# abstract-liu/LORB_SLAM

Measured on AMD Instinct MI355X. Metric: ORB matches/sec + local-BA iterations/sec (50 KF, 10k pts) at 1/2/4/8 MI355X, higher is better.
Workload: dtype f64+u8; 1 GPU; c4_local_mapping_step_chained; windows_per_gpu=1, kf=50, fixed_kf=5, points=10679, observations=75130, new_kf_keypoints=2000, match=2000x~10679 bf crossCheck, parallelism=independent windows x1

## Files before the change

lorb_slam_amd/csrc/lorb_ba.hip:

```cpp
#ifndef LORB_NO_CONTRACT
#pragma clang fp contract(fast)
#endif
#include "lorb_ba_math.h"
#include "lorb_internal.h"
#include "lorb_ba_dev.h"
#include "lorb_ba_plan.h"

#include <algorithm>
#include <cmath>
#include <type_traits>

namespace {

using namespace lorb::ba;
using lorb::residual;
using lorb::residual_jac;
using lorb::residual_jac_s;
using lorb::residual_s;

__device__ __forceinline__ void init_run(const BaDev& d, int W, int ctot, int n_pt, int nf, const LMOpt& o, const int i,
                                         const int stride) {
  if (i < W) {
    WinState s;
    s.radius = o.init_radius; s.decrease_factor = 2.0; s.cost = 0.0; s.x_norm = 0.0; s.gmax = 0.0;
    s.initial_cost = 0.0; s.iter = 0; s.n_success = 0; s.n_invalid = 0;
    s.done = d.win[i].n_obs_all == 0 ? 1 : 0;
    s.relin = 1; s.cur = 0; s.last_successful = 1; s.term = 0; s.chol_fail = 0; s.pad = 0;
    d.st[i] = s;
    if (d.sharded) d.wfail_part[i] = 0.0;
  }
  if (i < ctot) {
    double x[6];
#pragma unroll
    for (int k = 0; k < 6; ++k) { x[k] = d.x_init_pose[6 * i + k]; d.x_pose[0][6 * i + k] = x[k]; }
    d.rot_lin[i] = lorb::rot_jet(x);
  }
  if (i < nf) {
    double x[6];
#pragma unroll
    for (int k = 0; k < 6; ++k) x[k] = d.fixed_pose[6 * i + k];
    d.rot_fix[i] = lorb::rot_jet(x);
    d.rotv_fix[i] = lorb::rot_val(x);
  }
  for (int k = i; k < 3 * n_pt; k += stride) d.x_pt[0][k] = d.x_init_pt[k];
}
__global__ __launch_bounds__(256) void k_ba_init(BaDev d, int W, int ctot, int n_pt, int nf, LMOpt o) {
  init_run(d, W, ctot, n_pt, nf, o, blockIdx.x * blockDim.x + threadIdx.x, gridDim.x * blockDim.x);
}


constexpr int kGW = kGB / 64;
static_assert(kGW >= 1 && kGW <= 16 && kGB % 64 == 0, "point groups of 64..1024 observations, whole waves");
template <bool M1>
__device__ __forceinline__ void block_red3(double& a, double& b, double& c, double (*red)[kGW]) {
  a = wave_sum(a); b = M1 ? wave_max(b) : wave_sum(b); c = wave_sum(c);
  if (kGW == 1) return;
  __syncthreads();
  if ((threadIdx.x & 63) == 0) {
    const int w = threadIdx.x >> 6;
    red[0][w] = a; red[1][w] = b; red[2][w] = c;
  }
  __syncthreads();
  a = red[0][0]; b = red[1][0]; c = red[2][0];
#pragma unroll
  for (int k = 1; k < kGW; ++k) { a += red[0][k]; b = M1 ? fmax(b, red[1][k]) : b + red[1][k]; c += red[2][k]; }
}

__device__ __forceinline__ bool prep_point(const double (&Eu)[6], const double (&bu)[3], const double (&sp)[3],
                                           double rad, const LMOpt& o, double (&Ei)[6], double (&b)[3]) {
  double E[6];
#pragma unroll
  for (int k = 0; k < 3; ++k) b[k] = bu[k] * sp[k];
  E[0] = Eu[0] * sp[0] * sp[0]; E[1] = Eu[1] * sp[0] * sp[1]; E[2] = Eu[2] * sp[0] * sp[2];
  E[3] = Eu[3] * sp[1] * sp[1]; E[4] = Eu[4] * sp[1] * sp[2]; E[5] = Eu[5] * sp[2] * sp[2];
  E[0] += fmin(fmax(E[0], o.min_diag), o.max_diag) / rad;
  E[3] += fmin(fmax(E[3], o.min_diag), o.max_diag) / rad;
  E[5] += fmin(fmax(E[5], o.min_diag), o.max_diag) / rad;
  if (!inv3(E, Ei)) {
#pragma unroll
    for (int k = 0; k < 6; ++k) Ei[k] = 0.0;
    return false;
  }
  return true;
}
__device__ __forceinline__ void prep_fail(const BaDev& d, int win) {
  if (d.sharded) d.wfail_part[win] = 1.0;
  else d.st[win].chol_fail = 1;
}

template <int PH>
__global__ __launch_bounds__(64) void k_ba_win_reduce(BaDev d) {
  const int w = blockIdx.x;
  if (d.st[w].done) return;
  const BaWin& W = d.win[w];
  const int lane = threadIdx.x;
  double a = 0.0, b = 0.0, c = 0.0;
  if (PH == 0) group_partials<0, 1, 2, true>(d.part, W.pblk_base, W.n_pblk, lane, a, c, b);
  else group_partials<3, 4, 5, false>(d.part, W.pblk_base, W.n_pblk, lane, a, b, c);
  a = wave_sum(a); b = wave_sum(b);
  c = PH == 0 ? wave_max(c) : wave_sum(c);
  if (lane == 0) {
    if (PH == 0) { d.wlin_part[2 * w] = a; d.wlin_part[2 * w + 1] = b; d.wmax_part[w] = c; }
    else { d.wstep_part[3 * w] = a; d.wstep_part[3 * w + 1] = b; d.wstep_part[3 * w + 2] = c; }
  }
}

template <bool SH>
__device__ __forceinline__ void lm_begin_run(const BaDev& d, const LMOpt& o, const int w) {
  const WinState* Sp = d.st + w;
  const WinState S = *Sp;
  const BaWin W = d.win[w];
  if (S.done) return;
  (void)lm_head<SH>(d, o, w, threadIdx.x, S, W);
}
template <bool SH>
__global__ __launch_bounds__(64) void k_ba_lm_begin(BaDev d, LMOpt o) {
  lm_begin_run<SH>(d, o, blockIdx.x);
}

__device__ __forceinline__ void lm_record(const BaDev& d, int w, const WinState& S, int outcome, double mcc,
                                          double ncost, double step_norm) {
  if (S.iter < 1 || S.iter > LORB_LM_TRACE_CAP) return;
  lorb_lm_iteration r;
  r.iteration = S.iter; r.outcome = outcome;
  r.cost = S.cost; r.model_cost_change = mcc; r.new_cost = ncost; r.radius = S.radius; r.step_norm = step_norm;
  d.trace[(size_t)w * LORB_LM_TRACE_CAP + S.iter - 1] = r;
}

__device__ int lm_decide(BaDev d, const LMOpt& o, int w, WinState S, bool valid, double mccs,
                         double ncost, double sn2) {
  const double model_cost_change = -mccs;
  valid = valid && isfinite(model_cost_change) && isfinite(sn2) && model_cost_change > 0.0;
  if (!valid) {
    lm_record(d, w, S, LORB_LM_STEP_INVALID, model_cost_change, ncost, sqrt(sn2));
    if (++S.n_invalid >= o.max_invalid) {
      S.done = 1; S.term = LORB_TERM_FAILURE;
    } else {
      S.radius = S.radius / S.decrease_factor;
      S.decrease_factor *= 2.0;
      S.last_successful = 0;
      if (S.iter >= o.max_iter) { S.done = 1; S.term = LORB_TERM_NO_CONVERGENCE; }
    }
    d.st[w] = S;
    return 0;
  }
  S.n_invalid = 0;
  const double new_cost = isfinite(ncost) ? ncost : 1.7976931348623157e308;
  const double step_norm = sqrt(sn2);
  if (step_norm <= o.ptol * (S.x_norm + o.ptol)) {
    lm_record(d, w, S, LORB_LM_STEP_PARAM_TOL, model_cost_change, new_cost, step_norm);
    S.done = 1; S.term = LORB_TERM_PARAMETER_TOL; d.st[w] = S; return 0;
  }
  const double cost_change = S.cost - new_cost;
  if (fabs(cost_change) <= o.ftol * S.cost) {
    lm_record(d, w, S, LORB_LM_STEP_FUNC_TOL, model_cost_change, new_cost, step_norm);
    S.done = 1; S.term = LORB_TERM_FUNCTION_TOL; d.st[w] = S; return 0;
  }
  const double rel = cost_change / model_cost_change;
  lm_record(d, w, S, rel > o.min_rel ? LORB_LM_STEP_ACCEPTED : LORB_LM_STEP_REJECTED, model_cost_change, new_cost,
            step_norm);
  if (rel > o.min_rel) {
    S.cur ^= 1;
    S.relin = 1;
    S.cost = new_cost;
    S.n_success++;
    const double tt = 2.0 * rel - 1.0;
    S.radius = S.radius / fmax(1.0 / 3.0, 1.0 - tt * tt * tt);
    S.radius = fmin(o.max_radius, S.radius);
    S.decrease_factor = 2.0;
  } else {
    S.last_successful = 0;
    S.radius = S.radius / S.decrease_factor;
    S.decrease_factor *= 2.0;
  }
  if (S.iter >= o.max_iter) { S.done = 1; S.term = LORB_TERM_NO_CONVERGENCE; }
  d.st[w] = S;
  return rel > o.min_rel;
}

template <bool SH>
__device__ __forceinline__ void lm_end_run(const BaDev& d, const LMOpt& o, int w, int lane) {
  const WinState* Sp = d.st + w;
  WinState S = *Sp;
  const BaWin W = d.win[w];
  if (S.done) return;
  bool valid = !S.chol_fail;
  double mccs = 0.0, ncost = 0.0, sn2 = 0.0;
  double xc[6] = {0, 0, 0, 0, 0, 0};
  if (valid) {
    const int cur = S.cur;
    const int c0 = W.pose_base + lane;
    const bool has0 = lane < W.n_poses;
    double x0[6], xn0[6];
    bool act0 = false;
    if (has0) {
      act0 = d.cam_active[c0];
#pragma unroll
      for (int k = 0; k < 6; ++k) { x0[k] = d.x_pose[cur][6 * c0 + k]; xn0[k] = d.x_pose[cur ^ 1][6 * c0 + k]; }
    }
    if (!SH) group_partials<3, 4, 5, false>(d.part, W.pblk_base, W.n_pblk, lane, mccs, ncost, sn2);
    if (has0) {
#pragma unroll
      for (int k = 0; k < 6; ++k) {
        if (act0) sn2 += (x0[k] - xn0[k]) * (x0[k] - xn0[k]);
        xc[k] = xn0[k];
      }
    }
    for (int c = c0 + 64; c < W.pose_base + W.n_poses; c += 64) {
      const bool active = d.cam_active[c];
      for (int k = 0; k < 6; ++k) {
        const double x = d.x_pose[cur][6 * c + k];
        const double xn = d.x_pose[cur ^ 1][6 * c + k];
        if (active) sn2 += (x - xn) * (x - xn);
      }
    }
    mccs = wave_sum(mccs); ncost = wave_sum(ncost); sn2 = wave_sum(sn2);
    if (SH) { mccs += d.wstep[3 * w]; ncost += d.wstep[3 * w + 1]; sn2 += d.wstep[3 * w + 2]; }
  }
  S.chol_fail = 0;
  if (SH && lane == 0) d.wfail_part[w] = 0.0;
  int acc = 0;
  if (lane == 0) acc = lm_decide(d, o, w, S, valid, mccs, ncost, sn2);
  acc = __builtin_amdgcn_readfirstlane(acc);
  if (acc) {
    if (lane < W.n_poses) d.rot_lin[W.pose_base + lane] = lorb::rot_jet(xc);
    for (int c = W.pose_base + lane + 64; c < W.pose_base + W.n_poses; c += 64)
      d.rot_lin[c] = lorb::rot_jet(d.x_pose[S.cur ^ 1] + 6 * c);
  }
}
template <bool SH>
__global__ __launch_bounds__(64) void k_ba_lm_end(BaDev d, LMOpt o) {
  lm_end_run<SH>(d, o, blockIdx.x, threadIdx.x);
}


__device__ __forceinline__ void pm_slot_inv(int q, int bwc, int& a, int& dd) {
  const int T = (bwc + 1) * (bwc + 2) / 2;
  if (q < T) {
    a = (int)((sqrt(8.0 * q + 1.0) - 1.0) * 0.5);
    while ((a + 1) * (a + 2) / 2 <= q) ++a;
    while (a * (a + 1) / 2 > q) --a;
    dd = q - a * (a + 1) / 2;
  } else {
    const int r = q - T;
    a = bwc + 1 + r / (bwc + 1);
    dd = r - (r / (bwc + 1)) * (bwc + 1);
  }
}

constexpr int kLsThreads = kGB;
constexpr int kLsWaves = kLsThreads / 64;

template <int NW, bool M1>
__device__ __forceinline__ void block_red3w(double& a, double& b, double& c, double (*red)[NW]) {
  a = wave_sum(a); b = M1 ? wave_max(b) : wave_sum(b); c = wave_sum(c);
  __syncthreads();
  if ((threadIdx.x & 63) == 0) {
    const int w = threadIdx.x >> 6;
    red[0][w] = a; red[1][w] = b; red[2][w] = c;
  }
  __syncthreads();
  a = red[0][0]; b = red[1][0]; c = red[2][0];
#pragma unroll
  for (int k = 1; k < NW; ++k) { a += red[0][k]; b = M1 ? fmax(b, red[1][k]) : b + red[1][k]; c += red[2][k]; }
}

__device__ __forceinline__ void pm_lin(const BaDev& d, const BaWin& W, int cur, int p, int c, int fx, double2 uv,
                                       double (&r)[2], double (&Jp)[6], double (&Jc)[12]) {
  double X[3];
#pragma unroll
  for (int k = 0; k < 3; ++k) X[k] = d.x_pt[cur][3 * p + k];
  if (c >= 0) {
    double tr[3];
#pragma unroll
    for (int k = 0; k < 3; ++k) tr[k] = d.x_pose[cur][6 * c + 3 + k];
    residual_jac_s(d.rot_lin[c], tr, X, W.fx, W.fy, W.cx, W.cy, uv.x, uv.y, r, Jp, Jc);
  } else {
    double tr[3];
#pragma unroll
    for (int k = 0; k < 3; ++k) tr[k] = d.fixed_pose[6 * fx + 3 + k];
    residual_jac_s(d.rot_fix[fx], tr, X, W.fx, W.fy, W.cx, W.cy, uv.x, uv.y, r, Jp, Jc);
  }
}

struct LsSup {
  double* gsp;
  int cmin;
};
template <bool SUP>
__device__ __forceinline__ void ls_group(const BaDev& d, const LMOpt& o, const unsigned bid, const LsSup& su) {
  __shared__ double s_jc[kGB][12];
  __shared__ double s_qj[kGB][12];
  __shared__ double s_rg[kGB][4];
  __shared__ unsigned long long s_mask[2][kGB];
  __shared__ int s_po[kGB];
  __shared__ int s_mm[2][kLsWaves];
  __shared__ double red3[3][kLsWaves];
#ifdef LORB_LS_STAMPS
#define LS_STAMP(k) do { if (threadIdx.x == 0) d.dbg[8 * bid + (k)] = __builtin_amdgcn_s_memtime(); } while (0)
#else
#define LS_STAMP(k) do {} while (0)
#endif
  LS_STAMP(0);
#ifdef LORB_LS_STAMPS
  const unsigned long long ls_rt0 = __builtin_amdgcn_s_memrealtime();
  if (threadIdx.x == 0)
    d.dbg[8 * bid + 6] = ((unsigned long long)__builtin_amdgcn_s_getreg((31 << 11) | 4) << 8) |
                                (__builtin_amdgcn_s_getreg((31 << 11) | 20) & 255);
#endif
  const PBlk g = d.pblk[bid];
  const int t = threadIdx.x, lane = t & 63, wv = t >> 6;
  const bool has = t < g.no;
  const int of = g.o0 + min(t, max(g.no - 1, 0));
  const int p_ = has ? d.obs_pt[of] : 0, c_ = has ? d.obs_cam[of] : -1;
  const int fx_ = has ? d.obs_fix[of] : 0;
  const double2 uv = has ? d.obs_uv[of] : make_double2(0.0, 0.0);
  int po0 = 0, po1 = 0;
  double Xp[2][3] = {{0, 0, 0}, {0, 0, 0}}, spp[3] = {0, 0, 0};
  if (t < g.cnt) {
    const int p = g.p0 + t;
    po0 = d.pt_obs_off[p]; po1 = d.pt_obs_off[p + 1];
#pragma unroll
    for (int k = 0; k < 3; ++k) { Xp[0][k] = d.x_pt[0][3 * p + k]; Xp[1][k] = d.x_pt[1][3 * p + k]; spp[k] = d.scale_pt[3 * p + k]; }
  }
  const WinState& S = d.st[g.win];
  if (S.done) return;
  const BaWin& W = d.win[g.win];
  const int cur = S.cur;
  const double rad = S.radius;
  if (t < kGB) { s_mask[0][t] = 0ull; s_mask[1][t] = 0ull; }
  double r[2] = {0, 0}, Jp[6] = {0, 0, 0, 0, 0, 0}, Jc[12];
#pragma unroll
  for (int k = 0; k < 12; ++k) Jc[k] = 0.0;
  double cost = 0.0;
  if (has) {
    pm_lin(d, W, cur, p_, c_, fx_, uv, r, Jp, Jc);
    cost = 0.5 * (r[0] * r[0] + r[1] * r[1]);
    double* v = s_qj[t];
    v[0] = Jp[0] * Jp[0] + Jp[3] * Jp[3]; v[1] = Jp[0] * Jp[1] + Jp[3] * Jp[4];
    v[2] = Jp[0] * Jp[2] + Jp[3] * Jp[5]; v[3] = Jp[1] * Jp[1] + Jp[4] * Jp[4];
    v[4] = Jp[1] * Jp[2] + Jp[4] * Jp[5]; v[5] = Jp[2] * Jp[2] + Jp[5] * Jp[5];
    v[6] = Jp[0] * r[0] + Jp[3] * r[1]; v[7] = Jp[1] * r[0] + Jp[4] * r[1];
    v[8] = Jp[2] * r[0] + Jp[5] * r[1];
  }
  {
    int mn = has && c_ >= 0 ? c_ : 0x7fffffff, mx = has && c_ >= 0 ? c_ : -1;
#pragma unroll
    for (int s = 32; s > 0; s >>= 1) { mn = min(mn, __shfl_xor(mn, s, 64)); mx = max(mx, __shfl_xor(mx, s, 64)); }
    if (lane == 0) { s_mm[0][wv] = mn; s_mm[1][wv] = mx; }
  }
  __syncthreads();
  LS_STAMP(1);
  int cmin = s_mm[0][0], cmax = s_mm[1][0];
#pragma unroll
  for (int k = 1; k < kLsWaves; ++k) { cmin = min(cmin, s_mm[0][k]); cmax = max(cmax, s_mm[1][k]); }
  const int span = cmax >= 0 ? cmax - cmin + 1 : 0;
  double gm = 0.0, xn2 = 0.0;
  if (t < g.cnt) {
    const int p = g.p0 + t;
    double E[6] = {0, 0, 0, 0, 0, 0}, b[3] = {0, 0, 0};
    for (int e = po0 - g.o0; e < po1 - g.o0; ++e) {
      const double* v = s_qj[e];
#pragma unroll
      for (int k = 0; k < 6; ++k) E[k] += v[k];
#pragma unroll
      for (int k = 0; k < 3; ++k) b[k] += v[6 + k];
    }
#pragma unroll
    for (int k = 0; k < 3; ++k) d.etb[3 * p + k] = b[k];
    double sp[3];
    if (S.iter == 0) {
      sp[0] = 1.0 / (1.0 + sqrt(E[0]));
      sp[1] = 1.0 / (1.0 + sqrt(E[3]));
      sp[2] = 1.0 / (1.0 + sqrt(E[5]));
#pragma unroll
      for (int k = 0; k < 3; ++k) d.scale_pt[3 * p + k] = sp[k];
    } else {
#pragma unroll
      for (int k = 0; k < 3; ++k) sp[k] = spp[k];
    }
    if (po1 > po0) {
#pragma unroll
      for (int k = 0; k < 3; ++k) {
        const double X = cur ? Xp[1][k] : Xp[0][k];
        gm = fmax(gm, fabs(X - (X + -b[k])));
        xn2 += X * X;
      }
    }
    double Ei[6], bs[3];
    if (!prep_point(E, b, sp, rad, o, Ei, bs)) prep_fail(d, g.win);
#pragma unroll
    for (int k = 0; k < 6; ++k) { d.pinv[6 * p + k] = Ei[k]; s_jc[t][k] = Ei[k]; }
#pragma unroll
    for (int k = 0; k < 3; ++k) { s_jc[t][6 + k] = bs[k]; s_jc[t][9 + k] = sp[k]; }
    s_po[t] = po0 - g.o0;
  }
  const int lp = p_ - g.p0;
  const int a_ = c_ - cmin;
  if (has && c_ >= 0) atomicOr(&s_mask[a_ >> 6][lp], 1ull << (a_ & 63));
  __syncthreads();
  LS_STAMP(2);
  double Q[6], Js[6], g0 = 0.0, g1 = 0.0;
  int slot = -1;
  if (has && c_ >= 0) {
    const double* pt = s_jc[lp];
#pragma unroll
    for (int k = 0; k < 6; ++k) Js[k] = Jp[k] * pt[9 + k % 3];
#pragma unroll
    for (int rr = 0; rr < 2; ++rr)
#pragma unroll
      for (int j = 0; j < 3; ++j)
        Q[3 * rr + j] = Js[3 * rr] * s3(pt, 0, j) + Js[3 * rr + 1] * s3(pt, 1, j) + Js[3 * rr + 2] * s3(pt, 2, j);
    g0 = Q[0] * pt[6] + Q[1] * pt[7] + Q[2] * pt[8];
    g1 = Q[3] * pt[6] + Q[4] * pt[7] + Q[5] * pt[8];
    const unsigned long long m0 = s_mask[0][lp];
    slot = s_po[lp] + (a_ < 64 ? __popcll(m0 & ((1ull << a_) - 1ull))
                               : __popcll(m0) + __popcll(s_mask[1][lp] & ((1ull << (a_ - 64)) - 1ull)));
  }
  __syncthreads();
  if (slot >= 0) {
#pragma unroll
    for (int k = 0; k < 12; ++k) s_jc[slot][k] = Jc[k];
#pragma unroll
    for (int k = 0; k < 6; ++k) { s_qj[slot][k] = Q[k]; s_qj[slot][6 + k] = Js[k]; }
    s_rg[slot][0] = r[0]; s_rg[slot][1] = r[1]; s_rg[slot][2] = g0; s_rg[slot][3] = g1;
  }
  __syncthreads();
  LS_STAMP(3);
  const int bwc = W.bwc, nsl = pm_nslots(span, bwc);
  double* gp = SUP ? su.gsp : d.gpart + W.part_base + (size_t)(bid - W.sg_base) * W.part_stride;
  const int aoff = SUP ? cmin - su.cmin : 0;
  if (!SUP && t == 0) d.gspan[bid] = make_int2(span > 0 ? cmin - W.pose_base : 0, span);
  const bool split = nsl <= 64;
  int lr = 0;
  if (split) while (lr < 6 && (nsl << (lr + 1)) <= 64) ++lr;
  const int nrounds = split ? 1 : (nsl + 64 * kLsWaves - 1) / (64 * kLsWaves);
  for (int rd = 0; rd < nrounds; ++rd) {
    const int q = split ? lane >> lr : 64 * (kLsWaves * rd + wv) + lane;
    const int rr = split ? lane & ((1 << lr) - 1) : 0;
    const bool act = q < nsl;
    int a = 0, dd = 0;
    if (act) pm_slot_inv(q, bwc, a, dd);
    const int b = a - dd;
    const bool dg = dd == 0;
    double acc[36], ex[18];
#pragma unroll
    for (int k = 0; k < 36; ++k) acc[k] = 0.0;
#pragma unroll
    for (int k = 0; k < 18; ++k) ex[k] = 0.0;
    const int k0 = split ? (wv << lr) + rr : 0, kst = split ? kLsWaves << lr : 1;
    auto point_loop = [&](auto wide_tag) {
      constexpr bool kWide = decltype(wide_tag)::value;
      const int wa = kWide ? a >> 6 : 0, wb = kWide ? b >> 6 : 0;
      const unsigned long long ba = act ? 1ull << (a & 63) : 0ull, bb = 1ull << (b & 63);
      unsigned long long m = s_mask[0][k0], mh = kWide ? s_mask[1][k0] : 0ull;
      int po = s_po[k0];
      for (int k = k0; k < g.cnt; k += kst) {
        const unsigned long long mc = m, mch = mh;
        const int pc = po;
        if (k + kst < g.cnt) {
          m = s_mask[0][k + kst]; po = s_po[k + kst];
          if (kWide) mh = s_mask[1][k + kst];
        }
        const unsigned long long ma = kWide && wa ? mch : mc, mb = kWide && wb ? mch : mc;
        if ((ma & ba) && (mb & bb)) {
          const int lo = kWide ? __popcll(mc) : 0;
          const int eh = pc + (kWide && wa ? lo : 0) + __popcll(ma & (ba - 1ull));
          const int el = pc + (kWide && wb ? lo : 0) + __popcll(mb & (bb - 1ull));
          const double* Qh = s_qj[eh];
          const double* Jl = s_qj[el] + 6;
          const double* Ch = s_jc[eh];
          const double* Cl = s_jc[el];
          double k00 = -(Qh[0] * Jl[0] + Qh[1] * Jl[1] + Qh[2] * Jl[2]);
          double k01 = -(Qh[0] * Jl[3] + Qh[1] * Jl[4] + Qh[2] * Jl[5]);
          double k10 = -(Qh[3] * Jl[0] + Qh[4] * Jl[1] + Qh[5] * Jl[2]);
          double k11 = -(Qh[3] * Jl[3] + Qh[4] * Jl[4] + Qh[5] * Jl[5]);
          if (dg) { k00 += 1.0; k11 += 1.0; }
          double cl[12], ch[12];
#pragma unroll
          for (int j = 0; j < 12; ++j) { cl[j] = Cl[j]; ch[j] = Ch[j]; }
#pragma unroll
          for (int i = 0; i < 6; ++i) {
            const double z0 = ch[i] * k00 + ch[6 + i] * k10, z1 = ch[i] * k01 + ch[6 + i] * k11;
#pragma unroll
            for (int j = 0; j < 6; ++j) acc[6 * i + j] = fma(z0, cl[j], fma(z1, cl[6 + j], acc[6 * i + j]));
          }
          if (dg) {
            const double* rg = s_rg[eh];
            const double g0r = rg[0], g1r = rg[1], g2r = rg[2], g3r = rg[3];
#pragma unroll
            for (int i = 0; i < 6; ++i) {
              ex[i] = fma(ch[i], ch[i], fma(ch[6 + i], ch[6 + i], ex[i]));
              ex[6 + i] = fma(ch[i], g0r, fma(ch[6 + i], g1r, ex[6 + i]));
              ex[12 + i] = fma(ch[i], g2r, fma(ch[6 + i], g3r, ex[12 + i]));
            }
          }
        }
      }
    };
    if (k0 < g.cnt) {
      if (span > 64) point_loop(std::true_type{});
      else point_loop(std::false_type{});
    }
    for (int m = 1; m < (1 << lr); m <<= 1) {
#pragma unroll
      for (int k = 0; k < 36; ++k) acc[k] += __shfl_xor(acc[k], m, 64);
#pragma unroll
      for (int k = 0; k < 18; ++k) ex[k] += __shfl_xor(ex[k], m, 64);
    }
    const bool own = act && rr == 0;
    if (split) {
      static_assert(64 * 36 <= kGB * 12 && 64 * 18 <= kGB * 12, "reduction buffers");
      __syncthreads();
#pragma unroll
      for (int w = 0; w < kLsWaves; ++w) {
        if (wv == w && own) {
          double* bl = &s_jc[0][0] + 36 * q;
          double* bx = &s_qj[0][0] + 18 * q;
#pragma unroll
          for (int k = 0; k < 36; ++k) { if (w > 0) acc[k] += bl[k]; if (w + 1 < kLsWaves) bl[k] = acc[k]; }
          if (dg) {
#pragma unroll
            for (int k = 0; k < 18; ++k) { if (w > 0) ex[k] += bx[k]; if (w + 1 < kLsWaves) bx[k] = ex[k]; }
          }
        }
        if (w + 1 < kLsWaves) __syncthreads();
      }
    }
    if (own && (!split || wv == kLsWaves - 1)) {
      if (SUP) {
        double* out = gp + 36 * pm_slot(a + aoff, dd, bwc);
#pragma unroll
        for (int k = 0; k < 36; ++k) out[k] = out[k] + acc[k];
        if (dg) {
          double* gc = gp + W.part_cam + 18 * (a + aoff);
#pragma unroll
          for (int k = 0; k < 18; ++k) gc[k] = gc[k] + ex[k];
        }
      } else {
        double* out = gp + 36 * q;
#pragma unroll
        for (int k = 0; k < 36; ++k) out[k] = acc[k];
        if (dg) {
          double* gc = gp + W.part_cam + 18 * a;
#pragma unroll
          for (int k = 0; k < 18; ++k) gc[k] = ex[k];
        }
      }
    }
  }
  LS_STAMP(4);
  block_red3w<kLsWaves, true>(cost, gm, xn2, red3);
  if (t == 0) { double* P = d.part + 8 * bid; P[0] = cost; P[1] = gm; P[2] = xn2; }
  LS_STAMP(5);
#ifdef LORB_LS_STAMPS
  if (t == 0) d.dbg[8 * bid + 7] = (ls_rt0 << 20) | ((__builtin_amdgcn_s_memrealtime() - ls_rt0) & 0xfffff);
#endif
#undef LS_STAMP
}
__device__ __forceinline__ void ls_run(const BaDev& d, const LMOpt& o, const unsigned bid) {
  if ((int)bid >= d.live[0]) return;
  ls_group<false>(d, o, bid, LsSup{nullptr, 0});
}
__global__ __launch_bounds__(kLsThreads) void k_ba_ls(BaDev d, LMOpt o) { ls_run(d, o, blockIdx.x); }

__device__ __forceinline__ void ls_run_sup(const BaDev& d, const LMOpt& o, const unsigned sid) {
  __shared__ int s_r[2][kLsWaves];
  if ((int)sid >= d.live[2]) return;
  const int4 sg = d.sgrp[sid];
  const WinState& S = d.st[sg.x];
  if (S.done) return;
  const BaWin& W = d.win[sg.x];
  const PBlk gf = d.pblk[sg.y], gl = d.pblk[sg.y + sg.z - 1];
  const int t = threadIdx.x, lane = t & 63, wv = t >> 6;
  int mn = 0x7fffffff, mx = -1;
  for (int e = gf.o0 + t; e < gl.o0 + gl.no; e += kLsThreads) {
    const int c = d.obs_cam[e];
    if (c >= 0) { mn = min(mn, c); mx = max(mx, c); }
  }
#pragma unroll
  for (int k = 32; k > 0; k >>= 1) { mn = min(mn, __shfl_xor(mn, k, 64)); mx = max(mx, __shfl_xor(mx, k, 64)); }
  if (lane == 0) { s_r[0][wv] = mn; s_r[1][wv] = mx; }
  __syncthreads();
  int cmin = s_r[0][0], cmax = s_r[1][0];
#pragma unroll
  for (int k = 1; k < kLsWaves; ++k) { cmin = min(cmin, s_r[0][k]); cmax = max(cmax, s_r[1][k]); }
  const int span = cmax >= 0 ? cmax - cmin + 1 : 0;
  double* gsp = d.gpart + W.part_base + (size_t)(sid - W.sg_base) * W.part_stride;
  const int nb = 36 * pm_nslots(span, W.bwc), nc = 18 * span;
  for (int i = t; i < nb + nc; i += kLsThreads) gsp[i < nb ? i : W.part_cam + (i - nb)] = 0.0;
  if (t == 0) d.gspan[sid] = make_int2(span > 0 ? cmin - W.pose_base : 0, span);
  __syncthreads();
  for (int k = 0; k < sg.z; ++k) ls_group<true>(d, o, sg.y + k, LsSup{gsp, cmin});
}
__global__ __launch_bounds__(kLsThreads) __attribute__((amdgpu_waves_per_eu(2))) void k_ba_ls_sup(BaDev d, LMOpt o) {
  ls_run_sup(d, o, blockIdx.x);
}

template <int MODE, int RT>
__device__ __forceinline__ void red_run(const BaDev& d, const LMOpt& o, const unsigned bid) {
  constexpr int kRt = RT, kRw = kRt / 64;
  constexpr int kRc = 1024 / kRt;
  __shared__ int s_cand[kRt * kRc];
  __shared__ int s_a[kRt * kRc];
  __shared__ int s_wc[kRc][kRw];
  __shared__ double s_acc[1024];
  __shared__ double s_tot[54];
  if ((int)bid >= d.live[1]) return;
  const BlockPair bp = d.bp[bid];
  const bool diag = bp.ch == bp.cl;
  if (MODE == 0 && !diag) return;
  const WinState& S = d.st[bp.win];
  const BaWin& W = d.win[bp.win];
  const int t = threadIdx.x, lane = t & 63, wv = t >> 6;
  const int fi = t < 36 ? t / 6 : (t < 42 ? t - 36 : 0), fj = t < 36 ? t % 6 : 0;
  double sci = 1.0, scj = 1.0, udg = 0.0;
  if (MODE != 0) {
    sci = d.scale_pose[6 * bp.ch + fi];
    scj = d.scale_pose[6 * bp.cl + fj];
    if (MODE == 1 && diag) udg = d.U[21 * bp.ch + u21(fi, fi)];
  }
  if (S.done) return;
  const int h = bp.ch - W.pose_base, l = bp.cl - W.pose_base, dd = h - l;
  const int e0 = MODE == 0 ? 36 : 0, ne = MODE == 0 ? 12 : (diag ? 54 : 36);
  const int NS = 1024 / ne;
  const int nsub = kRt / ne, e = t % ne, sub = t / ne;
  constexpr int kSp = RT >= 1024 ? 1 : RT >= 512 ? 3 : 5;
  double acc[kSp];
#pragma unroll
  for (int q = 0; q < kSp; ++q) acc[q] = 0.0;
  const int g0 = W.sg_base, ng = W.n_sg;
  for (int c0 = 0; c0 < ng; c0 += kRt * kRc) {
    int2 gs[kRc];
#pragma unroll
    for (int u = 0; u < kRc; ++u) {
      const int gi = c0 + kRt * u + t;
      gs[u] = gi < ng ? d.gspan[g0 + gi] : make_int2(0, 0);
    }
    unsigned long long bal[kRc];
#pragma unroll
    for (int u = 0; u < kRc; ++u) {
      const bool cand = gs[u].y > 0 && gs[u].x <= l && h < gs[u].x + gs[u].y;
      bal[u] = __ballot(cand);
      if (lane == 0) s_wc[u][wv] = __popcll(bal[u]);
    }
    __syncthreads();
    int pre = 0, nc = 0;
#pragma unroll
    for (int u = 0; u < kRc; ++u)
#pragma unroll
      for (int k = 0; k < kRw; ++k) nc += s_wc[u][k];
#pragma unroll
    for (int u = 0; u < kRc; ++u) {
      int pu = pre;
#pragma unroll
      for (int k = 0; k < kRw; ++k) pu += k < wv ? s_wc[u][k] : 0;
      if ((bal[u] >> lane) & 1ull) {
        const int j = pu + __popcll(bal[u] & ((1ull << lane) - 1ull));
        s_cand[j] = c0 + kRt * u + t;
        s_a[j] = h - gs[u].x;
      }
#pragma unroll
      for (int k = 0; k < kRw; ++k) pre += s_wc[u][k];
    }
    __syncthreads();
    if (sub < nsub) {
      const int ee = e0 + e;
      auto at = [&](int j) -> const double* {
        const double* gp = d.gpart + W.part_base + (size_t)s_cand[j] * W.part_stride;
        const int a = s_a[j];
        return ee < 36 ? gp + 36 * pm_slot(a, dd, W.bwc) + ee : gp + W.part_cam + 18 * a + (ee - 36);
      };
      constexpr int kRu = RT >= 1024 ? 8 : RT >= 512 ? 4 : 2;
      for (int b0 = 0;; b0 += kRu) {
        double v[kSp][kRu];
        bool more = false;
#pragma unroll
        for (int q = 0; q < kSp; ++q) {
          const int s0 = sub + q * nsub;
#pragma unroll
          for (int u = 0; u < kRu; ++u) {
            const int j = s0 + (b0 + u) * NS;
            v[q][u] = s0 < NS && j < nc ? *at(j) : 0.0;
          }
          more |= s0 < NS && s0 + (b0 + kRu) * NS < nc;
        }
#pragma unroll
        for (int q = 0; q < kSp; ++q)
#pragma unroll
          for (int u = 0; u < kRu; ++u) acc[q] += v[q][u];
        if (!more) break;
      }
    }
    __syncthreads();
  }
  if (sub < nsub) {
#pragma unroll
    for (int q = 0; q < kSp; ++q) {
      const int s0 = sub + q * nsub;
      if (s0 < NS) s_acc[e + s0 * ne] = acc[q];
    }
  }
  __syncthreads();
  if (t < ne) {
    double v4[4] = {0.0, 0.0, 0.0, 0.0};
#pragma unroll 4
    for (int s = 0; s < NS; ++s) v4[s & 3] += s_acc[t + s * ne];
    s_tot[t] = (v4[0] + v4[1]) + (v4[2] + v4[3]);
  }
  __syncthreads();
  const int c = bp.ch;
  if (MODE == 0) {
    if (t < 6) d.U_part[21 * c + u21(t, t)] = s_tot[t];
    else if (t < 12) d.V_part[6 * c + t - 6] = s_tot[t];
    return;
  }
  double* A = d.env_part + W.env_base;
  if (t < 36) {
    const int i = fi, j = fj;
    if (!diag || j <= i) {
      double v = s_tot[t] * sci * scj;
      if (MODE == 1 && diag && i == j && d.rank0) {
        const double u = udg * sci * sci;
        v += fmin(fmax(u, o.min_diag), o.max_diag) / S.radius;
      }
      band(A, W.bw, 6 * h + i, 6 * l + j) = v;
    }
  } else if (diag && t < 42) {
    const int i = fi;
    d.rhs_part[W.row_base + 6 * h + i] = (s_tot[42 + i] - s_tot[48 + i]) * sci;
    if (MODE == 2) { d.U_part[21 * c + u21(i, i)] = s_tot[36 + i]; d.V_part[6 * c + i] = s_tot[42 + i]; }
  }
}
template <int MODE, int RT>
__global__ __launch_bounds__(RT) void k_ba_red(BaDev d, LMOpt o) { red_run<MODE, RT>(d, o, blockIdx.x); }

__device__ __forceinline__ void bs2_run(const BaDev& d, const unsigned bid) {
  __shared__ double sh[kGB][3], sst[kGB][3], sxn[kGB][3], ssp[kGB][3];
  __shared__ double red3[3][kGW];
  if ((int)bid >= d.live[0]) return;
  const PBlk g = d.pblk[bid];
  const int t = threadIdx.x;
  const bool has = t < g.no;
  const int of = g.o0 + min(t, max(g.no - 1, 0));
  const int p_ = has ? d.obs_pt[of] : 0, c_ = has ? d.obs_cam[of] : -1;
  const int fx_ = has ? d.obs_fix[of] : 0;
  const double2 uv = has ? d.obs_uv[of] : make_double2(0.0, 0.0);
  double b[3] = {0, 0, 0}, sp[3] = {0, 0, 0}, Xa[3] = {0, 0, 0}, Xb[3] = {0, 0, 0};
  double Ei[6] = {0, 0, 0, 0, 0, 0};
  int po0 = 0, po1 = 0;
  if (t < g.cnt) {
    const int p = g.p0 + t;
    po0 = d.pt_obs_off[p]; po1 = d.pt_obs_off[p + 1];
#pragma unroll
    for (int k = 0; k < 3; ++k) {
      sp[k] = d.scale_pt[3 * p + k];
      b[k] = d.etb[3 * p + k] * sp[k];
      Xa[k] = d.x_pt[0][3 * p + k];
      Xb[k] = d.x_pt[1][3 * p + k];
    }
#pragma unroll
    for (int k = 0; k < 6; ++k) Ei[k] = d.pinv[6 * p + k];
  }
  const WinState& S = d.st[g.win];
  if (S.done || S.chol_fail) return;
  const BaWin& W = d.win[g.win];
  const int cur = S.cur;
  if (t < g.cnt) {
#pragma unroll
    for (int k = 0; k < 3; ++k) ssp[t][k] = sp[k];
  }
  double ys[6] = {0, 0, 0, 0, 0, 0}, tc[3] = {0, 0, 0};
  lorb::RotVal Rc{};
  if (has && c_ >= 0) {
    const double* y = d.ycam + W.row_base + 6 * (c_ - W.pose_base);
#pragma unroll
    for (int i = 0; i < 6; ++i) ys[i] = y[i] * d.scale_pose[6 * c_ + i];
    Rc = d.rot_cand[c_];
#pragma unroll
    for (int k = 0; k < 3; ++k) tc[k] = d.x_pose[cur ^ 1][6 * c_ + 3 + k];
  }
  double r[2] = {0, 0}, Jp[6] = {0, 0, 0, 0, 0, 0}, Jc[12];
#pragma unroll
  for (int k = 0; k < 12; ++k) Jc[k] = 0.0;
  if (has) pm_lin(d, W, cur, p_, c_, fx_, uv, r, Jp, Jc);
  const int lp = p_ - g.p0;
  __syncthreads();
  double ya0 = 0.0, ya1 = 0.0;
  if (has) {
    if (c_ >= 0) {
#pragma unroll
      for (int i = 0; i < 6; ++i) {
        ya0 += Jc[i] * ys[i];
        ya1 += Jc[6 + i] * ys[i];
      }
#pragma unroll
      for (int j = 0; j < 3; ++j) sh[t][j] = (Jp[j] * ssp[lp][j]) * ya0 + (Jp[3 + j] * ssp[lp][j]) * ya1;
    } else {
      sh[t][0] = sh[t][1] = sh[t][2] = 0.0;
    }
  }
  __syncthreads();
  double sn2 = 0.0;
  if (t < g.cnt) {
    const int p = g.p0 + t;
    for (int e = po0 - g.o0; e < po1 - g.o0; ++e) {
#pragma unroll
      for (int j = 0; j < 3; ++j) b[j] -= sh[e][j];
    }
    double X[3], step[3];
#pragma unroll
    for (int k = 0; k < 3; ++k) X[k] = cur ? Xb[k] : Xa[k];
#pragma unroll
    for (int j = 0; j < 3; ++j)
      step[j] = -(s3(Ei, j, 0) * b[0] + s3(Ei, j, 1) * b[1] + s3(Ei, j, 2) * b[2]);
#pragma unroll
    for (int j = 0; j < 3; ++j) {
      const double xn = X[j] + step[j] * sp[j];
      d.x_pt[cur ^ 1][3 * p + j] = xn;
      sxn[t][j] = xn;
      sst[t][j] = step[j] * sp[j];
      if (po1 > po0) sn2 += (X[j] - xn) * (X[j] - xn);
    }
  }
  __syncthreads();
  double mcc = 0.0, ncost = 0.0;
  if (has) {
    const double Xn[3] = {sxn[lp][0], sxn[lp][1], sxn[lp][2]};
    double m0 = 0.0, m1 = 0.0;
#pragma unroll
    for (int j = 0; j < 3; ++j) {
      m0 += Jp[j] * sst[lp][j];
      m1 += Jp[3 + j] * sst[lp][j];
    }
    double rn[2];
    if (c_ >= 0) {
      m0 -= ya0;
      m1 -= ya1;
      residual_s(Rc, tc, Xn, W.fx, W.fy, W.cx, W.cy, uv.x, uv.y, rn);
    } else {
      double tr[3];
#pragma unroll
      for (int k = 0; k < 3; ++k) tr[k] = d.fixed_pose[6 * fx_ + 3 + k];
      residual_s(d.rotv_fix[fx_], tr, Xn, W.fx, W.fy, W.cx, W.cy, uv.x, uv.y, rn);
    }
    mcc = m0 * (r[0] + m0 / 2.0) + m1 * (r[1] + m1 / 2.0);
    ncost = 0.5 * (rn[0] * rn[0] + rn[1] * rn[1]);
  }
  block_red3<false>(mcc, ncost, sn2, red3);
  if (t == 0) {
    double* P = d.part + 8 * bid;
    P[3] = mcc; P[4] = ncost; P[5] = sn2;
  }
}
__global__ __launch_bounds__(kGB) void k_ba_bs2(BaDev d) { bs2_run(d, blockIdx.x); }

__global__ __launch_bounds__(256) void k_ba_init_g(BaGrp g, GrpGrid G, GrpInit a, LMOpt o) {
  unsigned lb;
  const int k = grp_member(G, g.n, blockIdx.x, lb);
  init_run(g.d[k], a.W[k], a.ctot[k], a.n_pt[k], a.nf[k], o, (int)(lb * 256 + threadIdx.x),
           (G.pre[k + 1] - G.pre[k]) * 256);
}
__global__ __launch_bounds__(kLsThreads) void k_ba_ls_g(BaGrp g, GrpGrid G, LMOpt o) {
  unsigned lb;
  const int k = grp_member(G, g.n, blockIdx.x, lb);
  ls_run(g.d[k], o, lb);
}
template <int MODE, int RT>
__global__ __launch_bounds__(RT) void k_ba_red_g(BaGrp g, GrpGrid G, LMOpt o) {
  unsigned lb;
  const int k = grp_member(G, g.n, blockIdx.x, lb);
  red_run<MODE, RT>(g.d[k], o, lb);
}
__global__ __launch_bounds__(64) void k_ba_lm_begin_g(BaGrp g, GrpGrid G, LMOpt o) {
  unsigned lb;
  const int k = grp_member(G, g.n, blockIdx.x, lb);
  lm_begin_run<false>(g.d[k], o, (int)lb);
}
__global__ __launch_bounds__(kGB) void k_ba_bs2_g(BaGrp g, GrpGrid G) {
  unsigned lb;
  const int k = grp_member(G, g.n, blockIdx.x, lb);
  bs2_run(g.d[k], lb);
}
__global__ __launch_bounds__(64) void k_ba_lm_end_g(BaGrp g, GrpGrid G, LMOpt o) {
  unsigned lb;
  const int k = grp_member(G, g.n, blockIdx.x, lb);
  lm_end_run<false>(g.d[k], o, (int)lb, threadIdx.x);
}

constexpr int kPoW = 4, kPoThreads = 64 * kPoW;
constexpr int kPoRegRes = 2 * kPoThreads;
constexpr int kPoArgF = 16;
struct PoOff { int n; int off[kPoArgF + 1]; };
template <class Load>
__device__ __forceinline__ void po_run(int nres, double fx, double fyv, double cx, double cy,
                                       const float* pose_init, const LMOpt& o, Load load,
                                       double* __restrict__ pose_out, lorb_ba_summary* __restrict__ sum) {
  __shared__ double s_nv[2][kPoW][28];
  __shared__ double s_cv[2][kPoW];
  const int t = threadIdx.x, lane = t & 63, wv = t >> 6;
  const int r0 = 0, r1 = nres;
  double xs[6], xn[6], sc[6], JtJ[21], Jtr[6];
#pragma unroll
  for (int k = 0; k < 6; ++k) { xs[k] = (double)pose_init[k]; xn[k] = xs[k]; sc[k] = 1.0; }
  if (r1 == r0) {
    if (t < 6) pose_out[t] = xs[t];
    if (t == 0) { lorb_ba_summary z = {}; *sum = z; }
    return;
  }
  double radius = o.init_radius, df = 2.0;
  int iter = 0, n_success = 0, n_invalid = 0, term = LORB_TERM_NO_CONVERGENCE, last_successful = 1;
  double initial_cost = 0.0, cost = 0.0, gmax = 0.0, xnorm = 0.0;
  bool relin = true;
  int buf = 0;
  constexpr int kPoC = kPoRegRes / kPoThreads;
  double cX[kPoC][3], cuv[kPoC][2];
#pragma unroll
  for (int q = 0; q < kPoC; ++q) {
    load(min(r0 + t + kPoThreads * q, r1 - 1), cX[q], cuv[q]);
  }
  for (;;) {
    if (relin) {
      double v[32];
#pragma unroll
      for (int k = 0; k < 28; ++k) v[k] = 0.0;
      const lorb::RotJet R = lorb::rot_jet(xs);
      auto acc = [&](const double (&X)[3], double u, double w) {
        double rr[2], Jp[6], Jc[12];
        residual_jac_s(R, xs + 3, X, fx, fyv, cx, cy, u, w, rr, Jp, Jc);
        int q = 0;
#pragma unroll
        for (int a = 0; a < 6; ++a) {
          v[21 + a] = fma(Jc[a], rr[0], fma(Jc[6 + a], rr[1], v[21 + a]));
#pragma unroll
          for (int b = a; b < 6; ++b) { v[q] = fma(Jc[a], Jc[b], fma(Jc[6 + a], Jc[6 + b], v[q])); ++q; }
        }
        v[27] += 0.5 * (rr[0] * rr[0] + rr[1] * rr[1]);
      };
// ... 161 lines not shown
                                                             double* __restrict__ pose_out,
                                                             lorb_ba_summary* __restrict__ sums) {
  const int f = blockIdx.x;
  const int r0 = aoff.n ? aoff.off[f] : res_off[f], r1 = aoff.n ? aoff.off[f + 1] : res_off[f + 1];
  const float* P = pts3d + 3 * (size_t)r0;
  const float* U = obs2d + 2 * (size_t)r0;
  po_run(r1 - r0, intr[4 * f], intr[4 * f + 1], intr[4 * f + 2], intr[4 * f + 3], pose_init + 6 * f, o,
         [&](int r, double (&X)[3], double (&uv)[2]) {
#pragma unroll
           for (int k = 0; k < 3; ++k) X[k] = P[3 * r + k];
           uv[0] = U[2 * r]; uv[1] = U[2 * r + 1];
         },
         pose_out + 6 * f, sums + f);
}

struct TailSlots {
  int nk;
  const int* code;
  bool keep;
  const uint8_t* slot_state;
  const float *slot_pos, *pt_pos, *x, *y;
  float* list;
  int* copy_to;
  int* assign_out;
};
__device__ __forceinline__ void tail_run(const TailSlots& s, bool solve, double fx, double fyv, double cx, double cy,
                                         const float* pose_init, const LMOpt& o, int* __restrict__ n_res,
                                         double* __restrict__ pose_out, lorb_ba_summary* __restrict__ sum) {
  __shared__ int s_slot[kPoRegRes];
  __shared__ int wsum[kPoW];
  const int t = threadIdx.x;
  int nres = 0;
  for (int c0 = 0; c0 < s.nk; c0 += kPoThreads) {
    const int j = c0 + t;
    int cd = LORB_ASSIGN_NULL;
    bool has = false;
    if (j < s.nk) {
      cd = s.code[j];
      has = cd >= 0 || (s.keep && cd == LORB_ASSIGN_UNCHANGED && s.slot_state && s.slot_state[j] != LORB_SLOT_EMPTY);
      if (s.copy_to) s.copy_to[j] = cd;
      if (s.assign_out) s.assign_out[j] = cd;
    }
    int tot;
    const int r = nres + lorb::block_excl_scan<kPoThreads>(has ? 1 : 0, wsum, &tot);
    if (has) {
      if (r < kPoRegRes) {
        s_slot[r] = j;
      } else {
        const float* X = cd >= 0 ? s.pt_pos + 3 * (size_t)cd : s.slot_pos + 3 * (size_t)j;
        float* L = s.list + 5 * (size_t)r;
        L[0] = X[0]; L[1] = X[1]; L[2] = X[2]; L[3] = s.x[j]; L[4] = s.y[j];
      }
    }
    nres += tot;
  }
  __syncthreads();
  if (t == 0) *n_res = nres;
  po_run(solve ? nres : 0, fx, fyv, cx, cy, pose_init, o,
         [&](int r, double (&X)[3], double (&uv)[2]) {
           if (r < kPoRegRes) {
             const int j = s_slot[r], cd = s.code[j];
             const float* Xp = cd >= 0 ? s.pt_pos + 3 * (size_t)cd : s.slot_pos + 3 * (size_t)j;
#pragma unroll
             for (int k = 0; k < 3; ++k) X[k] = Xp[k];
             uv[0] = s.x[j]; uv[1] = s.y[j];
           } else {
             const float* L = s.list + 5 * (size_t)r;
#pragma unroll
             for (int k = 0; k < 3; ++k) X[k] = L[k];
             uv[0] = L[3]; uv[1] = L[4];
           }
         },
         pose_out, sum);
}

__global__ __launch_bounds__(kPoThreads) void k_track_tail(lorb::TrackTail a, LMOpt o) {
  const int nm1 = *a.nm1;
  const bool retry = nm1 <= a.min_matches;
  const int nm2 = retry ? *a.nm2 : -1;
  const int pass = !retry ? 1 : (nm2 > a.min_matches ? 2 : 0);
  if (threadIdx.x == 0) { a.rec->pass = pass; a.rec->nmatches_first = nm1; a.rec->nmatches_retry = nm2; }
  const TailSlots s = {a.nk, retry ? a.assign2 : a.assign, !retry, a.slot_state, a.slot_pos, a.last_pos, a.x, a.y,
                       a.list, retry ? a.assign : nullptr, a.assign_out};
  tail_run(s, pass != 0, a.fx, a.fy_eff, a.cx, a.cy, a.pose_init, o, &a.rec->n_residuals, a.rec->pose, &a.rec->summary);
}

__global__ __launch_bounds__(kPoThreads) void k_local_tail(lorb::LocalTail a, LMOpt o) {
  __shared__ int wcnt[kPoW];
  const int nm = *a.nm;
  int c = 0;
  for (int m = threadIdx.x; m < a.np; m += kPoThreads) c += a.in_view[m] != 0;
  int n_in_view;
  lorb::block_excl_scan<kPoThreads>(c, wcnt, &n_in_view);
  const bool ok = nm > a.min_matches;
  if (threadIdx.x == 0) { a.rec->ok = ok; a.rec->nmatches = nm; a.rec->n_in_view = n_in_view; }
  const TailSlots s = {a.nk, a.assign, true, a.slot_state, a.slot_pos, a.pt_pos, a.x, a.y, a.list, nullptr, a.assign_out};
  tail_run(s, ok, a.fx, a.fy_eff, a.cx, a.cy, a.pose_init, o, &a.rec->n_residuals, a.rec->pose, &a.rec->summary);
}

LMOpt to_dev_opt(const lorb_lm_options* o) {
  LMOpt d;
  d.max_iter = o->max_num_iterations; d.max_invalid = o->max_num_consecutive_invalid_steps;
  d.jacobi = o->jacobi_scaling; d.ftol = o->function_tolerance; d.gtol = o->gradient_tolerance;
  d.ptol = o->parameter_tolerance; d.init_radius = o->initial_trust_region_radius;
  d.max_radius = o->max_trust_region_radius; d.min_radius = o->min_trust_region_radius;
  d.min_rel = o->min_relative_decrease; d.min_diag = o->min_lm_diagonal; d.max_diag = o->max_lm_diagonal;
  return d;
}
bool same_opt(const LMOpt& a, const LMOpt& b) {
  return a.max_iter == b.max_iter && a.max_invalid == b.max_invalid && a.jacobi == b.jacobi && a.ftol == b.ftol &&
         a.gtol == b.gtol && a.ptol == b.ptol && a.init_radius == b.init_radius && a.max_radius == b.max_radius &&
         a.min_radius == b.min_radius && a.min_rel == b.min_rel && a.min_diag == b.min_diag && a.max_diag == b.max_diag;
}

bool no_graph() { static const bool v = env_flag("LORB_NO_GRAPH"); return v; }
bool no_fuse() { static const bool v = env_flag("LORB_NO_FUSE"); return v; }

int chol_kind_of(const lorb_ba_plan* P) {
  static const bool force_old = [] { const char* e = getenv("LORB_CHOL"); return e && e[0] == 'o'; }();
  static const bool no_2s = [] { const char* e = getenv("LORB_CHOL"); return e && e[0] == 'w'; }();
  if (!P->Ctot) return -1;
  const bool chol_w = !force_old && P->max_bw <= 48 && sizeof(double) * (size_t)P->max_env_w <= (size_t)kLdsBudget;
  const bool chol_2s = chol_w && !no_2s && P->min_n16 >= 128 && P->min_bw >= 15;
  return chol_2s ? 2 : chol_w ? 1 : 0;
}

size_t x2_count(const lorb_ba_plan* P) {
  return P->devb ? P->x2_off + (size_t)P->env_total : (size_t)P->env_total + P->n_total + P->W;
}

int red_threads(const lorb_ba_plan* P) {
  const double W = std::max(P->W, 1), cams = std::max((double)P->Ctot / W, 1.0);
  const double cand = (double)P->n_pblk / W * ((P->max_bw + 1) / 6.0) / cams;
  if (P->grid_bp <= 256 || cand >= 128.0) return 1024;
  return P->grid_bp <= 1024 ? 512 : 256;
}
template <int MODE>
void launch_red(const lorb_ba_plan* P, hipStream_t s, const BaDev& d, const LMOpt& o) {
  const int rt = red_threads(P);
  if (rt == 1024) hipLaunchKernelGGL((k_ba_red<MODE, 1024>), dim3(P->grid_bp), dim3(1024), 0, s, d, o);
  else if (rt == 512) hipLaunchKernelGGL((k_ba_red<MODE, 512>), dim3(P->grid_bp), dim3(512), 0, s, d, o);
  else hipLaunchKernelGGL((k_ba_red<MODE, 256>), dim3(P->grid_bp), dim3(256), 0, s, d, o);
}

void launch_ls(const lorb_ba_plan* P, hipStream_t s, const BaDev& d, const LMOpt& o) {
  lorb::KernelTimer kt(P->ctx, LORB_K_BA_LINEARIZE);
  if (P->has_super) {
    if (P->grid_sg) hipLaunchKernelGGL(k_ba_ls_sup, dim3(P->grid_sg), dim3(kLsThreads), 0, s, d, o);
  } else if (P->grid_pblk) {
    hipLaunchKernelGGL(k_ba_ls, dim3(P->grid_pblk), dim3(kLsThreads), 0, s, d, o);
  }
}

lorb_ba_plan::GraphKey graph_key(const lorb_ba_plan* P) {
  lorb_ba_plan::GraphKey k;
  k.kind = chol_kind_of(P);
  k.lds = k.kind >= 1 ? P->max_env_w : P->max_env + 1000000 * P->max_bw;
  k.memset_env = sizeof(double) * (size_t)P->max_env > (size_t)kLdsBudget;
  k.env_total = k.memset_env ? P->env_total : 0;
  k.grid_pblk = P->grid_pblk; k.grid_bp = P->grid_bp; k.pt_launch = P->pt_launch;
  k.x2_n = P->comm ? (int)x2_count(P) : 0;
  k.red_wide = red_threads(P);
  k.sup = P->has_super ? 1 : 0;
  k.grid_sg = P->grid_sg;
  return k;
}

int enqueue_linearize(lorb_ba_plan* P, const LMOpt& o) {
  hipStream_t s = P->ctx->stream;
  const BaDev& d = P->dev;
  launch_ls(P, s, d, o);
  if (P->grid_bp) {
    lorb::KernelTimer kt(P->ctx, LORB_K_BA_SCHUR);
    launch_red<0>(P, s, d, o);
  }
  if (P->comm) {
    hipLaunchKernelGGL(k_ba_win_reduce<0>, dim3(P->W), dim3(64), 0, s, d);
    {
      lorb::KernelTimer kt(P->ctx, LORB_K_ALLREDUCE);
      LORB_TRY(lorb::comm_allreduce(P->comm, d.U_part, d.U, (size_t)P->Ctot * 27 + 2 * P->W, LORB_OP_SUM));
      LORB_TRY(lorb::comm_allreduce(P->comm, d.wmax_part, d.wmax, (size_t)P->W, LORB_OP_MAX));
    }
    hipLaunchKernelGGL(k_ba_lm_begin<true>, dim3(P->W), dim3(64), 0, s, d, o);
  } else {
    hipLaunchKernelGGL(k_ba_lm_begin<false>, dim3(P->W), dim3(64), 0, s, d, o);
  }
  return LORB_OK;
}

int enqueue_iteration(lorb_ba_plan* P, const LMOpt& o, bool first) {
  lorb_ctx* ctx = P->ctx;
  hipStream_t s = ctx->stream;
  const BaDev& d = P->dev;
  const bool fused = !first && chol_kind_of(P) == 2 && !no_fuse();
  if (fused) {
    launch_ls(P, s, d, o);
  } else {
    LORB_TRY(enqueue_linearize(P, o));
  }
  const bool chol_in_lds = sizeof(double) * (size_t)P->max_env <= (size_t)kLdsBudget;
  if (P->env_total && !chol_in_lds && !P->comm) LORB_HIP(ctx, hipMemsetAsync(d.env, 0, sizeof(double) * P->env_total, s));
  if (P->grid_bp) {
    lorb::KernelTimer kt(ctx, LORB_K_BA_SCHUR);
    if (fused) launch_red<2>(P, s, d, o);
    else launch_red<1>(P, s, d, o);
  }
  if (P->comm && fused) {
    hipLaunchKernelGGL(k_ba_win_reduce<0>, dim3(P->W), dim3(64), 0, s, d);
    lorb::KernelTimer kt(ctx, LORB_K_ALLREDUCE);
    LORB_TRY(lorb::comm_allreduce(P->comm, d.U_part, d.U, P->fx_n, LORB_OP_SUM));
    LORB_TRY(lorb::comm_allreduce(P->comm, d.wmax_part, d.wmax, (size_t)P->W, LORB_OP_MAX));
  } else if (P->comm) {
    lorb::KernelTimer kt(ctx, LORB_K_ALLREDUCE);
    LORB_TRY(lorb::comm_allreduce(P->comm, P->x2_send, P->x2_recv, x2_count(P), LORB_OP_SUM));
  }
  const int kind = chol_kind_of(P);
  P->chol_kind = kind;
  if (kind >= 0) {
    lorb::KernelTimer kt(ctx, LORB_K_BA_CHOLESKY);
    launch_chol(kind, CholShape{P->W, P->max_env, P->max_env_w, P->max_bw}, s, d, o, fused);
  }
  if (P->grid_pblk) hipLaunchKernelGGL(k_ba_bs2, dim3(P->grid_pblk), dim3(kGB), 0, s, d);
  if (P->comm) {
    hipLaunchKernelGGL(k_ba_win_reduce<1>, dim3(P->W), dim3(64), 0, s, d);
    {
      lorb::KernelTimer kt(ctx, LORB_K_ALLREDUCE);
      LORB_TRY(lorb::comm_allreduce(P->comm, d.wstep_part, d.wstep, 3 * (size_t)P->W, LORB_OP_SUM));
    }
    hipLaunchKernelGGL(k_ba_lm_end<true>, dim3(P->W), dim3(64), 0, s, d, o);
  } else {
    hipLaunchKernelGGL(k_ba_lm_end<false>, dim3(P->W), dim3(64), 0, s, d, o);
  }
  LORB_CHECK_LAUNCH(ctx);
  return LORB_OK;
}

int enqueue_solve(lorb_ba_plan* P, const LMOpt& o) {
  lorb_ctx* ctx = P->ctx;
  {
    const int n = std::max(std::max(std::max(P->W, P->Ctot), P->NF), std::min(3 * P->pt_launch, 256 * 1024));
    hipLaunchKernelGGL(k_ba_init, dim3(lorb::ceil_div(std::max(n, 1), 256)), dim3(256), 0, ctx->stream, P->dev, P->W,
                       P->Ctot, P->pt_launch, P->NF, o);
  }
  LORB_CHECK_LAUNCH(ctx);
  if (o.max_iter <= 0) return enqueue_linearize(P, o);
  for (int it = 0; it < o.max_iter; ++it) LORB_TRY(enqueue_iteration(P, o, it == 0));
  return LORB_OK;
}

int plan_solve(lorb_ba_plan* P, const lorb_lm_options* opt) {
  lorb_ctx* ctx = P->ctx;
  LMOpt o = to_dev_opt(opt);
  const bool timing = ctx->ktime || no_graph() || (P->comm && !P->comm->rccl);
  if (timing) return enqueue_solve(P, o);
  const lorb_ba_plan::GraphKey key = graph_key(P);
  const bool same = key == P->gkey && same_opt(P->graph_opt, o);
  return P->cache.replay_or_capture(ctx, same, [&] { return enqueue_solve(P, o); },
                                    [&] { P->gkey = key; P->graph_opt = o; });
}

int plan_read(lorb_ba_plan* P, double* const* pose_out, double* const* point_out,
              lorb_ba_summary* sums) {
  lorb_ctx* ctx = P->ctx;
  std::vector<WinState> st(P->W);
  std::vector<std::vector<double>> hp(P->W);
  LORB_HIP(ctx, hipMemcpyAsync(st.data(), P->d_state, sizeof(WinState) * P->W, hipMemcpyDeviceToHost, ctx->stream));
  LORB_HIP(ctx, hipStreamSynchronize(ctx->stream));
  for (int w = 0; w < P->W; ++w) {
    const BaWin& bw = P->hwin[w];
    const int cur = st[w].cur;
    if (pose_out && pose_out[w] && bw.n_poses) {
      hp[w].resize(6 * (size_t)bw.n_poses);
      LORB_HIP(ctx, hipMemcpyAsync(hp[w].data(), P->dev.x_pose[cur] + 6 * bw.pose_base, sizeof(double) * 6 * bw.n_poses, hipMemcpyDeviceToHost, ctx->stream));
    }
    if (point_out && point_out[w] && bw.n_points)
      LORB_HIP(ctx, hipMemcpyAsync(point_out[w], P->dev.x_pt[cur] + 3 * bw.point_base, sizeof(double) * 3 * bw.n_points, hipMemcpyDeviceToHost, ctx->stream));
    if (sums) {
      lorb_ba_summary s{};
      s.iterations = st[w].iter; s.successful_steps = st[w].n_success; s.termination = st[w].term;
      s.initial_cost = st[w].initial_cost; s.final_cost = st[w].cost;
      if (bw.n_obs_all == 0) { s.iterations = 0; s.termination = LORB_TERM_FUNCTION_TOL; }
      sums[w] = s;
    }
  }
  LORB_HIP(ctx, hipStreamSynchronize(ctx->stream));
  for (int w = 0; w < P->W; ++w) {
    if (hp[w].empty()) continue;
    const std::vector<int>& map = P->cam_map[w];
    for (int c = 0; c < P->hwin[w].n_poses; ++c)
      for (int q = 0; q < 6; ++q)
        pose_out[w][6 * (size_t)c + q] = hp[w][6 * (size_t)(map.empty() ? c : map[c]) + q];
  }
  return LORB_OK;
}

}

struct lorb_ba_group {
  lorb_ctx* ctx = nullptr;
  std::vector<lorb_ba_plan*> plans;
  GraphCache cache{"group graph"};
  LMOpt graph_opt{};
  std::vector<unsigned> gens;
  std::vector<lorb_ba_plan::GraphKey> keys;
  int n_fused = 0;
};

namespace {

bool group_fused(const lorb_ba_group* G) {
  if (no_fuse() || G->plans.size() > (size_t)kGrpMax) return false;
  for (const lorb_ba_plan* P : G->plans)
    if (P->W == 0 || P->comm || P->has_super || chol_kind_of(P) != 2) return false;
  return true;
}

template <typename F>
GrpGrid grp_grid(const lorb_ba_group* G, F f) {
  GrpGrid g{};
  for (size_t k = 0; k < G->plans.size(); ++k) g.pre[k + 1] = g.pre[k] + f(G->plans[k]);
  for (size_t k = G->plans.size() + 1; k <= (size_t)kGrpMax; ++k) g.pre[k] = g.pre[G->plans.size()];
  return g;
}

template <int MODE>
void launch_red_g(const lorb_ba_group* G, hipStream_t s, const BaGrp& bg, const LMOpt& o) {
  const GrpGrid gg = grp_grid(G, [](const lorb_ba_plan* P) { return P->grid_bp; });
  const int n = (int)G->plans.size(), nb = gg.pre[n];
  if (nb == 0) return;
  bool wide = nb <= 256;
  for (const lorb_ba_plan* P : G->plans) wide = wide || (red_threads(P) == 1024 && P->grid_bp > 256);
  const int rt = wide ? 1024 : nb <= 1024 ? 512 : 256;
  if (rt == 1024) hipLaunchKernelGGL((k_ba_red_g<MODE, 1024>), dim3(nb), dim3(1024), 0, s, bg, gg, o);
  else if (rt == 512) hipLaunchKernelGGL((k_ba_red_g<MODE, 512>), dim3(nb), dim3(512), 0, s, bg, gg, o);
  else hipLaunchKernelGGL((k_ba_red_g<MODE, 256>), dim3(nb), dim3(256), 0, s, bg, gg, o);
}

int enqueue_group_solve(lorb_ba_group* G, const LMOpt& o) {
  lorb_ctx* ctx = G->ctx;
  hipStream_t s = ctx->stream;
  const int n = (int)G->plans.size();
  BaGrp bg{};
  bg.n = n;
  for (int k = 0; k < n; ++k) bg.d[k] = G->plans[k]->dev;
  {
    GrpInit a{};
    for (int k = 0; k < n; ++k) {
      const lorb_ba_plan* P = G->plans[k];
      a.W[k] = P->W; a.ctot[k] = P->Ctot; a.n_pt[k] = P->pt_launch; a.nf[k] = P->NF;
    }
    const GrpGrid gg = grp_grid(G, [](const lorb_ba_plan* P) {
      const int m = std::max(std::max(std::max(P->W, P->Ctot), P->NF), std::min(3 * P->pt_launch, 256 * 1024));
      return lorb::ceil_div(std::max(m, 1), 256);
    });
    hipLaunchKernelGGL(k_ba_init_g, dim3(gg.pre[n]), dim3(256), 0, s, bg, gg, a, o);
  }
  const GrpGrid g_pb = grp_grid(G, [](const lorb_ba_plan* P) { return P->grid_pblk; });
  const GrpGrid g_w = grp_grid(G, [](const lorb_ba_plan* P) { return P->W; });
  size_t lds = 0;
  for (const lorb_ba_plan* P : G->plans) lds = std::max(lds, sizeof(double) * (size_t)P->max_env_w);
  auto linearise = [&]() {
    lorb::KernelTimer kt(ctx, LORB_K_BA_LINEARIZE);
    if (g_pb.pre[n]) hipLaunchKernelGGL(k_ba_ls_g, dim3(g_pb.pre[n]), dim3(kLsThreads), 0, s, bg, g_pb, o);
  };
  if (o.max_iter <= 0) {
    linearise();
    launch_red_g<0>(G, s, bg, o);
    hipLaunchKernelGGL(k_ba_lm_begin_g, dim3(g_w.pre[n]), dim3(64), 0, s, bg, g_w, o);
    LORB_CHECK_LAUNCH(ctx);
    return LORB_OK;
  }
  for (int it = 0; it < o.max_iter; ++it) {
    const bool first = it == 0;
    linearise();
    if (first) {
      {
        lorb::KernelTimer kt(ctx, LORB_K_BA_SCHUR);
        launch_red_g<0>(G, s, bg, o);
      }
      hipLaunchKernelGGL(k_ba_lm_begin_g, dim3(g_w.pre[n]), dim3(64), 0, s, bg, g_w, o);
    }
    for (const lorb_ba_plan* P : G->plans)
      if (P->env_total && sizeof(double) * (size_t)P->max_env > (size_t)kLdsBudget)
        LORB_HIP(ctx, hipMemsetAsync(P->dev.env, 0, sizeof(double) * P->env_total, s));
    {
      lorb::KernelTimer kt(ctx, LORB_K_BA_SCHUR);
      if (first) launch_red_g<1>(G, s, bg, o);
      else launch_red_g<2>(G, s, bg, o);
    }
    {
      lorb::KernelTimer kt(ctx, LORB_K_BA_CHOLESKY);
      launch_chol_2s_g(s, bg, g_w, o, !first, lds);
    }
    if (g_pb.pre[n]) hipLaunchKernelGGL(k_ba_bs2_g, dim3(g_pb.pre[n]), dim3(kGB), 0, s, bg, g_pb);
    hipLaunchKernelGGL(k_ba_lm_end_g, dim3(g_w.pre[n]), dim3(64), 0, s, bg, g_w, o);
  }
  for (lorb_ba_plan* P : G->plans) P->chol_kind = 2;
  LORB_CHECK_LAUNCH(ctx);
  return LORB_OK;
}

int group_solve(lorb_ba_group* G, const lorb_lm_options* opt) {
  lorb_ctx* ctx = G->ctx;
  if (!group_fused(G)) {
    for (lorb_ba_plan* P : G->plans)
      if (P->W > 0) LORB_TRY(plan_solve(P, opt));
    return LORB_OK;
  }
  const LMOpt o = to_dev_opt(opt);
  if (no_graph() || ctx->ktime) {
    LORB_TRY(enqueue_group_solve(G, o));
    G->n_fused++;
    return LORB_OK;
  }
  bool same = same_opt(G->graph_opt, o) && G->gens.size() == G->plans.size();
  for (size_t k = 0; k < G->plans.size() && same; ++k)
    same = G->gens[k] == G->plans[k]->gen && G->keys[k] == graph_key(G->plans[k]);
  LORB_TRY(G->cache.replay_or_capture(ctx, same, [&] { return enqueue_group_solve(G, o); }, [&] {
    G->graph_opt = o;
    G->gens.clear(); G->keys.clear();
    for (const lorb_ba_plan* P : G->plans) { G->gens.push_back(P->gen); G->keys.push_back(graph_key(P)); }
  }));
  G->n_fused++;
  return LORB_OK;
}

}

namespace lorb {
int launch_local_tail(lorb_ctx* ctx, const LocalTail& t, const lorb_lm_options* opt) {
  hipLaunchKernelGGL(k_local_tail, dim3(1), dim3(kPoThreads), 0, ctx->stream, t, to_dev_opt(opt));
  LORB_CHECK_LAUNCH(ctx);
  return LORB_OK;
}
int launch_track_tail(lorb_ctx* ctx, const TrackTail& t, const lorb_lm_options* opt) {
  hipLaunchKernelGGL(k_track_tail, dim3(1), dim3(kPoThreads), 0, ctx->stream, t, to_dev_opt(opt));
  LORB_CHECK_LAUNCH(ctx);
  return LORB_OK;
}
}

extern "C" {

int lorb_ba_plan_solve(lorb_ba_plan* plan, const lorb_lm_options* opt) {
  if (!plan || !opt) return LORB_E_INVALID;
  if (plan->W == 0) return LORB_OK;
  return plan_solve(plan, opt);
}

int lorb_ba_plan_read(lorb_ba_plan* plan, double* const* pose_out, double* const* point_out,
                      lorb_ba_summary* summaries) {
  if (!plan) return LORB_E_INVALID;
  if (plan->W == 0) return LORB_OK;
  return plan_read(plan, pose_out, point_out, summaries);
}

int lorb_ba_plan_trace(lorb_ba_plan* plan, int32_t window, lorb_lm_iteration* out, int32_t cap, int32_t* n_out) {
  if (!plan || !n_out || cap < 0 || (cap > 0 && !out)) return LORB_E_INVALID;
  *n_out = 0;
  if (window < 0 || window >= std::max(plan->W, 0)) return plan->W == 0 ? LORB_OK : LORB_E_INVALID;
  lorb_ctx* ctx = plan->ctx;
  WinState st;
  LORB_HIP(ctx, hipMemcpyAsync(&st, plan->d_state + window, sizeof(WinState), hipMemcpyDeviceToHost, ctx->stream));
  LORB_HIP(ctx, hipStreamSynchronize(ctx->stream));
  const int n = std::min(std::min(st.iter, (int)LORB_LM_TRACE_CAP), (int)cap);
  if (n > 0) {
    LORB_HIP(ctx, hipMemcpyAsync(out, plan->dev.trace + (size_t)window * LORB_LM_TRACE_CAP, sizeof(lorb_lm_iteration) * n,
                                 hipMemcpyDeviceToHost, ctx->stream));
    LORB_HIP(ctx, hipStreamSynchronize(ctx->stream));
  }
  *n_out = std::max(n, 0);
  return LORB_OK;
}

int lorb_ba_plan_debug_stamps(lorb_ba_plan* plan, unsigned long long* out8) {
  if (!plan || !out8) return LORB_E_INVALID;
  const size_t nst = dbg_words(1, (size_t)std::max(plan->n_pblk, plan->W));
  LORB_HIP(plan->ctx, hipMemcpyAsync(out8, plan->dev.dbg, nst * sizeof(unsigned long long), hipMemcpyDeviceToHost, plan->ctx->stream));
  LORB_HIP(plan->ctx, hipStreamSynchronize(plan->ctx->stream));
  return LORB_OK;
}

int lorb_ba_plan_info(lorb_ba_plan* plan, int32_t* info, int32_t n) {
  if (!plan || !info || n < 0) return LORB_E_INVALID;
  int bw = 0;
  for (const BaWin& w : plan->hwin) bw = std::max(bw, w.bw);
  int reordered = 0;
  for (const auto& m : plan->cam_map)
    for (size_t c = 0; c < m.size(); ++c) reordered |= m[c] != (int)c;
  int runs = 0;
  for (const BaWin& w : plan->hwin) runs += w.n_sg;
  const int32_t v[11] = {bw, plan->chol_kind, plan->n_bp, plan->n_pblk, plan->K, plan->Ptot, plan->Ctot, reordered,
                         1, red_threads(plan), plan->has_super ? runs : 0};
  for (int i = 0; i < n && i < 11; ++i) info[i] = v[i];
  return LORB_OK;
}

int lorb_ba_group_create(lorb_ctx* ctx, int32_t n_plans, lorb_ba_plan* const* plans, lorb_ba_group** out) {
  if (!ctx || !out || n_plans < 1 || !plans) return LORB_E_INVALID;
  *out = nullptr;
  for (int k = 0; k < n_plans; ++k) {
    if (!plans[k]) return lorb::set_error(ctx, LORB_E_INVALID, "lorb_ba_group_create: plan %d is null", k);
    if (plans[k]->ctx != ctx)
      return lorb::set_error(ctx, LORB_E_INVALID, "lorb_ba_group_create: plan %d belongs to another context", k);
    for (int j = 0; j < k; ++j)
      if (plans[j] == plans[k]) return lorb::set_error(ctx, LORB_E_INVALID, "lorb_ba_group_create: plan %d appears twice", k);
  }
  lorb_ba_group* G = new (std::nothrow) lorb_ba_group();
  if (!G) return LORB_E_NOMEM;
  G->ctx = ctx;
  G->plans.assign(plans, plans + n_plans);
  *out = G;
  return LORB_OK;
}

int lorb_ba_group_solve(lorb_ba_group* group, const lorb_lm_options* opt) {
  if (!group || !opt) return LORB_E_INVALID;
  return group_solve(group, opt);
}

int lorb_ba_group_info(lorb_ba_group* group, int32_t* info, int32_t n) {
  if (!group || !info || n < 0) return LORB_E_INVALID;
  const int32_t v[3] = {(int32_t)group->plans.size(), group->n_fused, group->cache.captures};
  for (int i = 0; i < n && i < 3; ++i) info[i] = v[i];
  return LORB_OK;
}

int lorb_ba_group_destroy(lorb_ba_group* group) {
  if (!group) return LORB_OK;
  (void)hipStreamSynchronize(group->ctx->stream);
  delete group;
  return LORB_OK;
}

int lorb_ba_local(lorb_ctx* ctx, int32_t n_windows, const lorb_ba_window* windows,
                  const lorb_lm_options* opt, double* const* pose_out, double* const* point_out,
                  lorb_ba_summary* summaries) {
  if (!ctx || !opt) return LORB_E_INVALID;
  lorb_ba_plan* P = nullptr;
  LORB_TRY(lorb_ba_plan_create(ctx, n_windows, windows, &P));
  int rc = lorb_ba_plan_solve(P, opt);
  if (rc == LORB_OK) rc = lorb_ba_plan_read(P, pose_out, point_out, summaries);
  lorb_ba_plan_destroy(P);
  return rc;
}

int lorb_ba_pose_only(lorb_ctx* ctx, const lorb_pose_problem_batch* prob,
                      const lorb_lm_options* opt, double* pose_out, float* Tcw_out,
                      lorb_ba_summary* summaries) {
  if (!ctx || !prob || !opt || !pose_out) return LORB_E_INVALID;
  const int nf = prob->n_frames;
  if (nf <= 0) return LORB_OK;
  const int nr = prob->res_off[nf];
  int max_res = 0;
  for (int f = 0; f < nf; ++f) max_res = std::max(max_res, prob->res_off[f + 1] - prob->res_off[f]);
  lorb::InPack in(ctx);
  const int i_roff = in.add_t(prob->res_off, (size_t)nf + 1), i_intr = in.add_t(prob->intr, (size_t)nf * 4),
            i_pinit = in.add_t(prob->pose_init, (size_t)nf * 6), i_pts = in.add_t(prob->pts3d, (size_t)nr * 3),
            i_obs = in.add_t(prob->obs2d, (size_t)nr * 2);
  LORB_TRY(in.commit(max_res <= kPoRegRes));
  lorb::OutPack out(ctx);
  const int o_pose = out.add(sizeof(double) * 6 * nf), o_sum = out.add(sizeof(lorb_ba_summary) * nf);
  LORB_TRY(out.alloc(true));
  PoOff aoff{};
  if (nf <= kPoArgF) {
    aoff.n = nf;
    for (int f = 0; f <= nf; ++f) aoff.off[f] = prob->res_off[f];
  }
  hipLaunchKernelGGL(k_ba_pose_only, dim3(nf), dim3(kPoThreads), 0, ctx->stream, aoff, in.dev<int32_t>(i_roff), in.dev<float>(i_intr),
                     in.dev<float>(i_pinit), in.dev<float>(i_pts), in.dev<float>(i_obs), to_dev_opt(opt),
                     out.dev<double>(o_pose), out.dev<lorb_ba_summary>(o_sum));
  LORB_CHECK_LAUNCH(ctx);
  LORB_TRY(out.fetch());
  memcpy(pose_out, out.host<double>(o_pose), sizeof(double) * 6 * nf);
  if (summaries) memcpy(summaries, out.host<lorb_ba_summary>(o_sum), sizeof(lorb_ba_summary) * nf);
  if (Tcw_out)
    for (int f = 0; f < nf; ++f) {
      const float R[3] = {(float)pose_out[6 * f], (float)pose_out[6 * f + 1], (float)pose_out[6 * f + 2]};
      const float T[3] = {(float)pose_out[6 * f + 3], (float)pose_out[6 * f + 4], (float)pose_out[6 * f + 5]};
      lorb_pose_to_Tcw(R, T, Tcw_out + 16 * f);
    }
  return LORB_OK;
}

int lorb_ba_pose_only_dev(lorb_ctx* ctx, const lorb_pose_problem_batch* d_prob, const lorb_lm_options* opt,
                          double* d_pose_out, lorb_ba_summary* d_summaries) {
  if (!ctx || !d_prob || !opt) return LORB_E_INVALID;
  const int nf = d_prob->n_frames;
  if (nf <= 0) return LORB_OK;
  if (!d_prob->res_off || !d_prob->intr || !d_prob->pose_init || !d_pose_out || !d_summaries)
    return lorb::set_error(ctx, LORB_E_INVALID, "null array");
  PoOff aoff{};
  hipLaunchKernelGGL(k_ba_pose_only, dim3(nf), dim3(kPoThreads), 0, ctx->stream, aoff, d_prob->res_off, d_prob->intr,
                     d_prob->pose_init, d_prob->pts3d, d_prob->obs2d, to_dev_opt(opt), d_pose_out, d_summaries);
  LORB_CHECK_LAUNCH(ctx);
  return LORB_OK;
}

void lorb_pose_to_Tcw(const float rvec[3], const float tvec[3], float T[16]) {
#pragma clang fp contract(off)
  double rx = rvec[0], ry = rvec[1], rz = rvec[2];
  const double theta = std::sqrt(rx * rx + ry * ry + rz * rz);
  double R[9];
  if (theta < 2.220446049250313e-16) {
    for (int k = 0; k < 9; ++k) R[k] = (k % 4 == 0) ? 1.0 : 0.0;
  } else {
    const double c = std::cos(theta), s = std::sin(theta), c1 = 1. - c;
    const double it = theta ? 1. / theta : 0.;
    rx *= it; ry *= it; rz *= it;
    const double rrt[9] = {rx * rx, rx * ry, rx * rz, rx * ry, ry * ry, ry * rz, rx * rz, ry * rz, rz * rz};
    const double rxm[9] = {0, -rz, ry, rz, 0, -rx, -ry, rx, 0};
    const double I[9] = {1, 0, 0, 0, 1, 0, 0, 0, 1};
    for (int k = 0; k < 9; ++k) R[k] = c * I[k] + c1 * rrt[k] + s * rxm[k];
  }
  for (int r = 0; r < 3; ++r) {
    for (int c = 0; c < 3; ++c) T[4 * r + c] = (float)R[3 * r + c];
    T[4 * r + 3] = tvec[r];
  }
  T[12] = 0.f; T[13] = 0.f; T[14] = 0.f; T[15] = 1.f;
}

}
```

lorb_slam_amd/csrc/lorb_ba_build.hip:

```cpp
#ifndef LORB_NO_CONTRACT
#pragma clang fp contract(fast)
#endif
#include "lorb_ba_math.h"
#include "lorb_internal.h"
#include "lorb_ba_dev.h"
#include "lorb_ba_plan.h"

#include <algorithm>
#include <chrono>
#include <cmath>
#include <map>

struct lorb_ba_devbuild {
  int K_cap = 0, P_cap = 0, C = 0, F = 0, Wd = 0;
  int* key_out = nullptr; int* val_out = nullptr;
  int* scr = nullptr; size_t scr_bytes = 0;
  int* pt_cnt = nullptr;
  int* hdr = nullptr;
  int* cov = nullptr;
  int* cam_cnt = nullptr;
  unsigned long long* bits = nullptr;
  int* perm = nullptr;
  int pblk_cap = 0, part_cap = 0, gspan_cap = 0, sgrp_cap = 0;
  size_t gpart_cap = 0;
// ... 303 lines not shown
  for (int w = 0; w < nw; ++w) {
    const lorb_ba_window& in = win[w];
    if (in.n_poses < 0 || in.n_points < 0 || in.n_obs < 0 || in.n_fixed < 0)
      return lorb::set_error(ctx, LORB_E_INVALID, "window %d: negative sizes", w);
    BaWin bw{};
    bw.pose_base = pose_base; bw.n_poses = in.n_poses;
    bw.point_base = point_base; bw.n_points = in.n_points;
    bw.fx = in.fx; bw.fy = in.fy; bw.cx = in.cx; bw.cy = in.cy;
    bw.obs_base = (int)obs_cam.size(); bw.n_obs = in.n_obs;
    bw.n_obs_all = comm ? g_obs[w] : in.n_obs;
    std::vector<int> cnt(in.n_points + 1, 0);
    for (int k = 0; k < in.n_obs; ++k) {
      const int p = in.obs_point[k], f = in.obs_frame[k];
      if (p < 0 || p >= in.n_points) return lorb::set_error(ctx, LORB_E_INVALID, "window %d obs %d: bad point %d", w, k, p);
      if (f >= in.n_poses || f < -in.n_fixed) return lorb::set_error(ctx, LORB_E_INVALID, "window %d obs %d: bad frame %d", w, k, f);
      cnt[p + 1]++;
    }
    for (int p = 0; p < in.n_points; ++p) cnt[p + 1] += cnt[p];
    std::vector<int> order(in.n_obs), fill(in.n_points, 0);
    for (int k = 0; k < in.n_obs; ++k) { const int p = in.obs_point[k]; order[cnt[p] + fill[p]++] = k; }
    const int ob0 = (int)obs_cam.size();
    for (int p = 0; p < in.n_points; ++p) pt_obs_off.push_back(ob0 + cnt[p + 1]);
    for (int e = 0; e < in.n_obs; ++e) {
      const int k = order[e], f = in.obs_frame[k];
      obs_cam.push_back(f >= 0 ? pose_base + f : -1);
      obs_pt.push_back(point_base + in.obs_point[k]);
      obs_fix.push_back(f >= 0 ? -1 : fix_base + (-1 - f));
      obs_uv.push_back(make_double2(in.obs_uv[2 * k], in.obs_uv[2 * k + 1]));
    }
    for (int i = 0; i < 6 * in.n_fixed; ++i) fixed.push_back(in.fixed_pose[i]);
    for (int i = 0; i < 6 * in.n_poses; ++i) xpose.push_back(in.pose_init[i]);
    for (int i = 0; i < 3 * in.n_points; ++i) xpt.push_back(in.point_init[i]);
    {
      std::vector<int> n_cam(in.n_poses, 0);
      for (int e = 0; e < in.n_obs; ++e) { const int c = obs_cam[ob0 + e]; if (c >= 0) n_cam[c - pose_base]++; }
      for (int c = 0; c < in.n_poses; ++c) cam_active.push_back(comm ? (g_cam_obs[w][c] > 0) : n_cam[c] > 0);
    }
    std::map<std::pair<int, int>, int> bmap;
    for (int c = 0; c < in.n_poses; ++c) bmap[{c, c}];
    std::vector<int> fc(in.n_poses);
    for (int c = 0; c < in.n_poses; ++c) fc[c] = c;
    for (int p = 0; p < in.n_points; ++p) {
      const int e0 = ob0 + cnt[p], e1 = ob0 + cnt[p + 1];
      for (int a = e0; a < e1; ++a) {
        const int ca = obs_cam[a];
        if (ca < 0) continue;
        for (int b = e0; b < e1; ++b) {
          const int cb = obs_cam[b];
          if (cb < 0 || cb > ca) continue;
          if (cb == ca && a != b)
            return lorb::set_error(ctx, LORB_E_INVALID, "window %d: a point observed twice by one camera", w);
          bmap[{ca - pose_base, cb - pose_base}]++;
          fc[ca - pose_base] = std::min(fc[ca - pose_base], cb - pose_base);
        }
      }
    }
    for (auto& kv : bmap) {
      bps.push_back(BlockPair{w, pose_base + kv.first.first, pose_base + kv.first.second, n_pairs, kv.second});
      n_pairs += kv.second;
    }
    const int n = 6 * in.n_poses;
    if (comm)
      for (int c = 0; c < in.n_poses; ++c) fc[c] = std::min(fc[c], g_fc[w][c]);
    const int bwid = band_of(fc);
    bw.env_base = env_base; bw.env_size = n * (bwid + 1); bw.n = n; bw.row_base = row_base; bw.bw = bwid;
    P->max_env = std::max(P->max_env, bw.env_size + 2 * n);
    P->max_bw = std::max(P->max_bw, bwid);
    if (n > 0) P->min_bw = std::min(P->min_bw, bwid);
    {
      const int n16 = (n + 15) & ~15;
      P->max_env_w = std::max(P->max_env_w, chol_lds_words(n16, bwid));
      if (n16 > 0) P->min_n16 = std::min(P->min_n16, n16);
    }
    env_base += bw.env_size; row_base += n;
    bw.pblk_base = (int)pblk.size();
    int span_max = 0;
    for (int p = 0; p < in.n_points;) {
      PBlk g{w, point_base + p, 0, ob0 + cnt[p], 0};
      int gmin = INT32_MAX, gmax = -1;
      while (p < in.n_points && g.cnt < kGB) {
        const int k = cnt[p + 1] - cnt[p];
        int pmin = INT32_MAX, pmax = -1;
        for (int e = ob0 + cnt[p]; e < ob0 + cnt[p + 1]; ++e)
          if (obs_cam[e] >= 0) { pmin = std::min(pmin, obs_cam[e]); pmax = std::max(pmax, obs_cam[e]); }
        if (k > kGB)
          return lorb::set_error(ctx, LORB_E_UNSUPPORTED, "window %d: point %d has %d observations (a point group holds %d)",
                                 w, p, k, kGB);
        if (pmax - pmin >= kPmSpan)
          return lorb::set_error(ctx, LORB_E_UNSUPPORTED, "window %d: point %d is seen by cameras %d apart (at most %d)",
                                 w, p, pmax - pmin, kPmSpan - 1);
        const int nmin = std::min(gmin, pmin), nmax = std::max(gmax, pmax);
        if (g.cnt > 0 && (g.no + k > kGB || (nmax >= 0 && nmax - nmin >= kPmSpan))) break;
        g.cnt++; g.no += k; ++p;
        gmin = nmin; gmax = nmax;
      }
      if (gmax >= 0) span_max = std::max(span_max, gmax - gmin + 1);
      pblk.push_back(g);
      gcam.push_back(make_int2(gmin, gmax));
    }
    bw.n_pblk = (int)pblk.size() - bw.pblk_base;
    {
      const int F = sg_factor(bw.n_pblk);
      bw.sg_base = (int)sgrp.size();
      if (F > 1) span_max = 0;
      for (int g = 0; g < bw.n_pblk; g += F) {
        const int ng = std::min(F, bw.n_pblk - g);
        sgrp.push_back(make_int4(w, bw.pblk_base + g, ng, 0));
        int umin = INT32_MAX, umax = -1;
        for (int k = 0; k < ng; ++k) {
          const int2 c = gcam[bw.pblk_base + g + k];
          if (c.y >= 0) { umin = std::min(umin, c.x); umax = std::max(umax, c.y); }
        }
        if (F > 1 && umax >= 0) span_max = std::max(span_max, umax - umin + 1);
      }
      bw.n_sg = (int)sgrp.size() - bw.sg_base;
      P->has_super = P->has_super || F > 1;
    }
    pm_layout(bw, span_max, part_total);
    P->hwin.push_back(bw);
    pose_base += in.n_poses; point_base += in.n_points; fix_base += in.n_fixed;
  }
  P->Ctot = pose_base; P->Ptot = point_base; P->K = (int)obs_cam.size(); P->NF = fix_base;
  LORB_TRY(part_budget_check(ctx, part_total));
  P->n_pblk = (int)pblk.size(); P->n_bp = (int)bps.size(); P->n_pairs = n_pairs;
  P->env_total = env_base; P->n_total = row_base;
  P->grid_pblk = P->n_pblk; P->grid_bp = P->n_bp; P->pt_launch = P->Ptot;
  P->grid_sg = (int)sgrp.size();
  BaDev& d = P->dev;
  LORB_TRY(dupload(P, P->hwin, &d.win));
  LORB_TRY(dupload(P, std::vector<int>{P->n_pblk, P->n_bp, (int)sgrp.size()}, &P->live)); d.live = P->live;
  LORB_TRY(dupload(P, sgrp.empty() ? std::vector<int4>{make_int4(0, 0, 0, 0)} : sgrp, &d.sgrp));
  LORB_TRY(dupload(P, pblk, &d.pblk));
  LORB_TRY(dupload(P, obs_pt, &d.obs_pt));
  LORB_TRY(dupload(P, bps, &d.bp));
  LORB_TRY(dupload(P, pt_obs_off, &d.pt_obs_off));
  LORB_TRY(dupload(P, obs_cam, &d.obs_cam));
  LORB_TRY(dupload(P, obs_fix, &d.obs_fix));
  LORB_TRY(dupload(P, obs_uv, &d.obs_uv));
  LORB_TRY(dupload(P, fixed, &d.fixed_pose));
  LORB_TRY(dupload(P, xpose, &d.x_init_pose));
  LORB_TRY(dupload(P, xpt, &d.x_init_pt));
  LORB_TRY(dupload(P, xpose, &d.x_pose[0]));
  LORB_TRY(dupload(P, xpose, &d.x_pose[1]));
  LORB_TRY(dupload(P, xpt, &d.x_pt[0]));
  LORB_TRY(dupload(P, xpt, &d.x_pt[1]));
  const size_t C = P->Ctot, Pn = P->Ptot;
  LORB_TRY(dalloc(P, C * 6, &d.scale_pose)); LORB_TRY(dalloc(P, Pn * 3, &d.scale_pt));
  LORB_TRY(dalloc(P, Pn * 3, &d.etb)); LORB_TRY(dalloc(P, Pn * 6, &d.pinv));
  LORB_TRY(dupload(P, cam_active, &d.cam_active));
  double *sol, *solp;
  LORB_TRY(alloc_exchange(P, C, (size_t)nw, (size_t)P->env_total + P->n_total + nw, &sol, &solp));
  d.env = sol; d.rhs = sol + P->env_total; d.wfail = sol + P->env_total + P->n_total;
  d.env_part = solp; d.rhs_part = solp + P->env_total; d.wfail_part = solp + P->env_total + P->n_total;
  LORB_TRY(dalloc(P, (size_t)P->Ctot, &d.rot_lin));
  LORB_TRY(dalloc(P, (size_t)P->Ctot, &d.rot_cand));
  LORB_TRY(dalloc(P, (size_t)std::max(P->NF, 1), &d.rot_fix));
  LORB_TRY(dalloc(P, (size_t)std::max(P->NF, 1), &d.rotv_fix));
  if (P->env_total) LORB_HIP(ctx, hipMemsetAsync(d.env, 0, sizeof(double) * P->env_total, ctx->stream));
  LORB_TRY(dalloc(P, (size_t)P->n_total, &d.ycam)); LORB_TRY(dalloc(P, (size_t)P->n_pblk * 8, &d.part));
  LORB_TRY(dalloc(P, dbg_words((size_t)nw, (size_t)std::max(P->n_pblk, nw)), &d.dbg));
  LORB_TRY(dalloc(P, ((size_t)P->n_total / 16 + nw + 1) * 1024, &d.kco));
  LORB_TRY(dalloc(P, (size_t)nw, &P->d_state)); d.st = P->d_state;
  LORB_TRY(dalloc(P, (size_t)nw * LORB_LM_TRACE_CAP, &d.trace));
  LORB_TRY(dalloc(P, (size_t)std::max(part_total, 1ll), &d.gpart));
  LORB_TRY(dalloc(P, (size_t)std::max(P->grid_sg, 1), &d.gspan));
  LORB_HIP(ctx, hipStreamSynchronize(ctx->stream));
  return LORB_OK;
}


__global__ __launch_bounds__(256) void k_db_keys(lorb_ba_window_dev w, int C, int F, int Wd,
                                                 int* __restrict__ pt_cnt, int* __restrict__ hdr,
                                                 unsigned long long* __restrict__ bits) {
  const int k = blockIdx.x * 256 + threadIdx.x;
  const int n_obs_in = *w.d_n_obs, n_pt_in = *w.d_n_points;
  const int n_obs = min(n_obs_in, w.max_obs), n_pt = min(n_pt_in, w.max_points);
  if (k == 0) {
    hdr[3] = n_pt;
    if (n_obs_in > w.max_obs || n_pt_in > w.max_points || n_obs_in < 0 || n_pt_in < 0) atomicOr(&hdr[2], 8);
  }
  if (k >= n_obs) return;
  const int q = w.d_obs_point[k], f = w.d_obs_frame[k];
  if (f >= -F && f < C) {
    if (q < 0 || q >= n_pt) {
      atomicOr(&hdr[2], 1);
    } else {
      atomicAdd(&pt_cnt[q], 1);
      if (f >= 0) {
        const unsigned long long m = 1ull << (q & 63);
        if (atomicOr(&bits[(size_t)f * Wd + (q >> 6)], m) & m) atomicOr(&hdr[2], 4);
      }
    }
  } else if (f >= C) {
    atomicOr(&hdr[2], 2);
  }
}

constexpr int kDbWords = 4;
constexpr int kDbFuseLds = 64 * 1024;
template <bool FUSE>
__global__ __launch_bounds__(256) void k_db_sorted(lorb_ba_window_dev w, int C, int F, int Wd, int* __restrict__ pt_off,
                                                   int* __restrict__ hdr, unsigned long long* __restrict__ bits,
                                                   int* __restrict__ cov, int* __restrict__ cam_cnt) {
  extern __shared__ unsigned long long s_bits[];
  int* s_cov = reinterpret_cast<int*>(s_bits + C * kDbWords);
  int* s_cam = s_cov + C * C;
  __shared__ int s_cnt, s_err;
  const int t = threadIdx.x, lane = t & 63;
  const int i = blockIdx.x * 256 + t;
  const int n_obs_in = *w.d_n_obs, n_pt_in = *w.d_n_points;
  const int n_obs = max(min(n_obs_in, w.max_obs), 0), n_pt = max(min(n_pt_in, w.max_points), 0);
  const int* __restrict__ op = w.d_obs_point;
  const int* __restrict__ of = w.d_obs_frame;
  for (int k = t; k < C * kDbWords; k += 256) s_bits[k] = 0ull;
  if (FUSE)
    for (int k = t; k < C * C + C; k += 256) s_cov[k] = 0;
  if (t == 0) { s_cnt = 0; s_err = 0; }
  const int i0 = blockIdx.x * 256;
  const int w0 = i0 < n_obs ? max(op[i0], 0) >> 6 : 0;
  int err = 0, cnt = 0;
  if (i == 0) {
    hdr[3] = n_pt;
    hdr[0] = n_obs;
    if (n_obs_in > w.max_obs || n_pt_in > w.max_points || n_obs_in < 0 || n_pt_in < 0) err |= 8;
  }
  const int prev = (i > 0 && i <= n_obs) ? op[i - 1] : -1;
  const int q = i < n_obs ? op[i] : n_pt;
  const int f = i < n_obs ? of[i] : -1;
  const bool bound = i <= n_obs && (i == n_obs || prev != q);
  const unsigned long long bal = __ballot(bound);
  __syncthreads();
  if (i < n_obs) {
    if (f < -F) err |= 16;
    else if (f >= C) err |= 2;
    else if (q < 0 || q >= n_pt) err |= 1;
    else if (f >= 0) {
      const unsigned long long m = 1ull << (q & 63);
      const int wl = (q >> 6) - w0;
      if (wl >= 0 && wl < kDbWords) atomicOr(&s_bits[f * kDbWords + wl], m);
      else __hip_atomic_fetch_or(&bits[(size_t)f * Wd + (q >> 6)], m, __ATOMIC_RELAXED, __HIP_MEMORY_SCOPE_AGENT);
    }
  }
  if (i <= n_obs) {
    if (prev > q) err |= 16;
    else if (prev != q) {
      const int p1 = min(q, n_pt);
      for (int p = max(prev + 1, 0); p <= p1; ++p) pt_off[p] = i;
      if (i < n_obs) {
        const unsigned long long above = lane < 63 ? bal & (~0ull << (lane + 1)) : 0ull;
        int e;
        if (above) {
          e = i - lane + __builtin_ctzll(above);
        } else {
          e = i - lane + 64;
          for (bool more = true; more;) {
            bool eq[8];
#pragma unroll
            for (int u = 0; u < 8; ++u) eq[u] = e + u < n_obs && op[e + u] == q;
            int run = 0;
#pragma unroll
            for (int u = 7; u >= 0; --u) run = eq[u] ? run + 1 : 0;
            e += run;
            more = run == 8;
          }
          e = min(max(e, i + 1), n_obs);
        }
        cnt = e - i;
        constexpr int kR = 16;
        int fr[kR];
#pragma unroll
        for (int k = 0; k < kR; ++k) fr[k] = k < cnt ? of[i + k] : -1 - k;
#pragma unroll
        for (int a = 1; a < kR; ++a)
#pragma unroll
          for (int b = 0; b < a; ++b)
            if (fr[a] >= 0 && fr[a] == fr[b]) err |= 4;
        for (int a = kR; a < cnt; ++a) {
          const int fa = of[i + a];
          if (fa < 0) continue;
          for (int b = 0; b < a; ++b)
            if (of[i + b] == fa) err |= 4;
        }
        if (FUSE && q >= 0 && q < n_pt) {
#pragma unroll
          for (int a = 0; a < kR; ++a) {
            if (fr[a] < 0 || fr[a] >= C) continue;
            atomicAdd(&s_cam[fr[a]], 1);
#pragma unroll
            for (int b = 0; b < a; ++b)
              if (fr[b] >= 0 && fr[b] < C && fr[b] != fr[a])
                atomicAdd(&s_cov[max(fr[a], fr[b]) * C + min(fr[a], fr[b])], 1);
          }
          for (int a = kR; a < cnt; ++a) {
            const int fa = of[i + a];
            if (fa < 0 || fa >= C) continue;
            atomicAdd(&s_cam[fa], 1);
            for (int b = 0; b < a; ++b) {
              const int fb = of[i + b];
              if (fb >= 0 && fb < C && fb != fa) atomicAdd(&s_cov[max(fa, fb) * C + min(fa, fb)], 1);
            }
          }
        }
      }
    }
  }
#pragma unroll
  for (int o = 32; o > 0; o >>= 1) cnt = max(cnt, __shfl_xor(cnt, o, 64));
  if (lane == 0 && cnt) atomicMax(&s_cnt, cnt);
  if (err) atomicOr(&s_err, err);
  __syncthreads();
  for (int k = t; k < C * kDbWords; k += 256) {
    const unsigned long long v = s_bits[k];
    const int wd = w0 + k % kDbWords;
    if (v && wd < Wd)
      __hip_atomic_fetch_or(&bits[(size_t)(k / kDbWords) * Wd + wd], v, __ATOMIC_RELAXED, __HIP_MEMORY_SCOPE_AGENT);
// ... 103 lines not shown
  int sgf = 1, nsg = 0;
  int4* sgrp = nullptr;
};
struct DbCams {
  int perm[kPmSpan], gcam[kPmSpan];
};
__device__ __forceinline__ void group_bounds(const int* __restrict__ off, int P, long long b0, long long b1, int lane,
                                             int& s0, int& s1) {
  const int half = lane >> 5, j = lane & 31;
  const long long bound = half ? b1 : b0;
  int lo = 0, hi = P;
  while (__ballot(hi > lo)) {
    const int n = hi - lo;
    bool pr = false;
    if (n > 0) {
      const int q = lo + (int)(((long long)n * (j + 1)) / 33);
      pr = (long long)off[q] + q >= bound;
    }
    const unsigned long long bal = __ballot(pr);
    const unsigned msk = half ? (unsigned)(bal >> 32) : (unsigned)bal;
    if (n > 0) {
      if (msk) {
        const int f = __builtin_ctz(msk);
        hi = lo + (int)(((long long)n * (f + 1)) / 33);
        if (f > 0) lo = lo + (int)(((long long)n * f) / 33) + 1;
      } else {
        lo = lo + (int)(((long long)n * 32) / 33) + 1;
      }
    }
  }
  s0 = __shfl(lo, 0, 64);
  s1 = __shfl(lo, 32, 64);
}
__global__ __launch_bounds__(256) void k_db_gather(lorb_ba_window_dev w, BaDev d, int K, const int* __restrict__ key,
                                                   const int* __restrict__ val, DbFused f, DbCams cams) {
  const int gt = blockIdx.x * 256 + threadIdx.x, gs = gridDim.x * 256;
  for (int i = gt; i < f.up_words; i += gs) f.up_dst[i] = f.up_src[i];
  const int* __restrict__ perm = cams.perm;
  const int* __restrict__ gcam = cams.gcam;
  {
    const int m = max(max(6 * f.C, 6 * f.F), 3 * f.P);
    for (int i = gt; i < m; i += gs) {
      if (i < 6 * f.C) {
        const int c = i / 6, q = i - 6 * c;
        d.x_init_pose[6 * perm[c] + q] = (double)w.d_pose_init[i];
        if (q == 0) const_cast<int*>(d.cam_active)[perm[c]] = gcam[c] > 0;
      }
      if (i < 6 * f.F) const_cast<double*>(d.fixed_pose)[i] = (double)w.d_fixed_pose[i];
      if (i < 3 * f.P) d.x_init_pt[i] = (double)w.d_point_init[i];
    }
  }
  for (int g = gt >> 6; g < f.G; g += gs >> 6) {
    int s0, s1;
    group_bounds(d.pt_obs_off, f.P, (long long)g * f.S, (long long)(g + 1) * f.S, threadIdx.x & 63, s0, s1);
    if ((threadIdx.x & 63) == 0) {
      PBlk b;
      b.win = 0; b.p0 = s0; b.cnt = s1 - s0; b.o0 = d.pt_obs_off[s0]; b.no = d.pt_obs_off[s1] - d.pt_obs_off[s0];
      const_cast<PBlk*>(d.pblk)[g] = b;
    }
  }
  for (int i = gt; i < f.nsg; i += gs) f.sgrp[i] = make_int4(0, i * f.sgf, min(f.sgf, f.G - i * f.sgf), 0);
  for (int i = gt; i < f.env_n; i += gs) d.env_part[i] = 0.0;
  for (int i = gt; i < f.bits_n; i += gs) f.bits[i] = 0ull;
  for (int i = gt; i < f.cov_n; i += gs) f.cov[i] = 0;
  if (gt == 0) { f.hdr[1] = 0; f.hdr[2] = 0; }
  for (int e = gt; e < K; e += gs) {
    const int k = f.sorted ? e : val[e];
    const int fr = w.d_obs_frame[k];
    const_cast<int*>(d.obs_pt)[e] = f.sorted ? w.d_obs_point[e] : key[e];
    const_cast<int*>(d.obs_cam)[e] = fr >= 0 ? perm[fr] : -1;
    const_cast<int*>(d.obs_fix)[e] = fr >= 0 ? -1 : -1 - fr;
    const_cast<double2*>(d.obs_uv)[e] = make_double2(w.d_obs_uv[2 * k], w.d_obs_uv[2 * k + 1]);
  }
}

__global__ __launch_bounds__(256) void k_db_result(BaDev d, int C, int P, const int* __restrict__ perm,
                                                   float* __restrict__ pose_out, float* __restrict__ pt_out,
                                                   float* __restrict__ ring, int R, int t0) {
  const int i = blockIdx.x * 256 + threadIdx.x;
  const int cur = d.st[0].cur;
  if ((pose_out || ring) && i < 6 * C) {
    const int c = i / 6, q = i - 6 * c;
    const float v = (float)d.x_pose[cur][6 * perm[c] + q];
    if (pose_out) pose_out[i] = v;
    if (ring) {
      const int r = (t0 + c) % R;
      ring[6 * (r < 0 ? r + R : r) + q] = v;
    }
  }
  if (pt_out)
    for (int k = i; k < 3 * P; k += gridDim.x * 256) pt_out[k] = (float)d.x_pt[cur][k];
}

__global__ __launch_bounds__(256) void k_db_result64(BaDev d, int C, int P, const int* __restrict__ perm,
                                                     double* __restrict__ out) {
  const int i = blockIdx.x * 256 + threadIdx.x;
  const WinState& st = d.st[0];
  const int cur = st.cur;
  if (i < 6 * C) {
    const int c = i / 6, q = i - 6 * c;
    out[i] = d.x_pose[cur][6 * perm[c] + q];
  }
  for (int k = i; k < 3 * P; k += gridDim.x * 256) out[6 * C + k] = d.x_pt[cur][k];
  if (i == 0) {
    double* s = out + 6 * C + 3 * P;
    s[0] = st.iter; s[1] = st.n_success; s[2] = st.term; s[3] = st.initial_cost; s[4] = st.cost;
  }
}

template <typename T, typename Cap>
int grow(lorb_ba_plan* P, T** ptr, Cap* cap, size_t need) {
  if (*ptr && (size_t)*cap >= need) return LORB_OK;
  if (*ptr) LORB_TRY(dfree(P, *ptr));
  const size_t n = std::max<size_t>(need + need / 4, 16);
  LORB_TRY(dalloc(P, n, ptr));
  *cap = (Cap)n;
  P->cache.invalidate();
  P->gen++;
  return LORB_OK;
}

int dev_alloc(lorb_ctx* ctx, const lorb_ba_window_dev* w, lorb_ba_plan* P) {
  lorb_ba_devbuild& b = *P->devb;
  b.K_cap = w->max_obs; b.P_cap = w->max_points; b.C = w->n_poses; b.F = w->n_fixed;
  b.Wd = (std::max(b.P_cap, 1) + 63) / 64;
  const size_t K = (size_t)std::max(b.K_cap, 1), Pn = (size_t)std::max(b.P_cap, 1), C = (size_t)std::max(b.C, 1);
  BaDev& d = P->dev;
  if (b.C > kPmSpan)
    return lorb::set_error(ctx, LORB_E_UNSUPPORTED, "device-built plans hold windows of <= %d cameras (%d)", kPmSpan, b.C);
  LORB_TRY(dalloc(P, K, &b.key_out)); LORB_TRY(dalloc(P, K, &b.val_out));
  {
    const size_t ints = ((Pn + 1 + 8 + C * C + C) + 1) & ~(size_t)1;
    b.scr_bytes = sizeof(int) * ints + sizeof(unsigned long long) * C * (size_t)b.Wd;
    unsigned char* m;
    LORB_TRY(dalloc(P, b.scr_bytes, &m));
    b.scr = reinterpret_cast<int*>(m);
    b.pt_cnt = b.scr; b.hdr = b.pt_cnt + Pn + 1; b.cov = b.hdr + 8; b.cam_cnt = b.cov + C * C;
    b.bits = reinterpret_cast<unsigned long long*>(b.scr + ints);
  }
  LORB_TRY(dalloc(P, K, &d.obs_pt)); LORB_TRY(dalloc(P, K, &d.obs_cam)); LORB_TRY(dalloc(P, K, &d.obs_fix));
  LORB_TRY(dalloc(P, K, &d.obs_uv)); LORB_TRY(dalloc(P, C, &d.cam_active));
  LORB_TRY(dalloc(P, Pn + 1, &d.pt_obs_off)); LORB_TRY(dalloc(P, (size_t)std::max(b.F, 1) * 6, &d.fixed_pose));
  LORB_TRY(dalloc(P, C * 6, &d.x_init_pose)); LORB_TRY(dalloc(P, Pn * 3, &d.x_init_pt));
  LORB_TRY(dalloc(P, C * 6, &d.x_pose[0])); LORB_TRY(dalloc(P, C * 6, &d.x_pose[1]));
  LORB_TRY(dalloc(P, Pn * 3, &d.x_pt[0])); LORB_TRY(dalloc(P, Pn * 3, &d.x_pt[1]));
  LORB_TRY(dalloc(P, C * 6, &d.scale_pose)); LORB_TRY(dalloc(P, Pn * 3, &d.scale_pt));
  LORB_TRY(dalloc(P, Pn * 3, &d.etb)); LORB_TRY(dalloc(P, Pn * 6, &d.pinv));
  const size_t n = 6 * C;
  P->x2_off = (n + 1 + 31) & ~(size_t)31;
  double *sol, *solp;
  LORB_TRY(alloc_exchange(P, C, 1, P->x2_off + n * n, &sol, &solp));
  d.rhs = sol; d.wfail = sol + n; d.env = sol + P->x2_off;
  d.rhs_part = solp; d.wfail_part = solp + n; d.env_part = solp + P->x2_off;
  LORB_TRY(dalloc(P, C, &d.rot_lin)); LORB_TRY(dalloc(P, C, &d.rot_cand));
  LORB_TRY(dalloc(P, (size_t)std::max(b.F, 1), &d.rot_fix)); LORB_TRY(dalloc(P, (size_t)std::max(b.F, 1), &d.rotv_fix));
  LORB_TRY(dalloc(P, n, &d.ycam));
  LORB_TRY(dalloc(P, dbg_words(1, K + Pn + 1), &d.dbg));
  LORB_TRY(dalloc(P, ((size_t)n / 16 + 2) * 1024, &d.kco));
  LORB_TRY(dalloc(P, (size_t)1, &P->d_state)); d.st = P->d_state;
  LORB_TRY(dalloc(P, (size_t)LORB_LM_TRACE_CAP, &d.trace));
  P->W = 1;
  P->hwin.assign(1, BaWin{});
  P->pt_launch = b.P_cap;
  return LORB_OK;
}

int up_alloc(lorb_ba_plan* P, int bp_need) {
  lorb_ba_devbuild& b = *P->devb;
  if (b.up_dev && b.up_bp_cap >= bp_need) return LORB_OK;
  lorb_ctx* ctx = P->ctx;
  const int cap = std::max(bp_need + bp_need / 4, 16);
  auto al = [](size_t x) { return (x + 255) & ~(size_t)255; };
  const size_t C = (size_t)std::max(b.C, 1);
  b.off_live = al(sizeof(BaWin));
  b.off_perm = b.off_live + 256;
  b.off_gcam = b.off_perm + al(4 * C);
  b.off_bp = b.off_gcam + al(4 * C);
  b.up_bytes = b.off_bp + sizeof(BlockPair) * (size_t)cap;
  if (b.up_dev) {
    LORB_TRY(dfree(P, b.up_dev));
    (void)hipHostFree(b.up_host);
    b.up_host = nullptr;
  }
  LORB_TRY(dalloc(P, b.up_bytes, &b.up_dev));
  LORB_HIP(ctx, hipHostMalloc(reinterpret_cast<void**>(&b.up_host), b.up_bytes));
  LORB_HIP(ctx, hipHostGetDevicePointer((void**)&b.up_host_dev, b.up_host, 0));
  b.up_bp_cap = cap;
  BaDev& d = P->dev;
  d.win = reinterpret_cast<const BaWin*>(b.up_dev);
  d.live = reinterpret_cast<const int*>(b.up_dev + b.off_live);
  b.perm = reinterpret_cast<int*>(b.up_dev + b.off_perm);
  d.bp = reinterpret_cast<const BlockPair*>(b.up_dev + b.off_bp);
  P->grid_bp = cap;
  P->cache.invalidate();
  P->gen++;
  return LORB_OK;
}

int db_phase1_issue(lorb_ctx* ctx, const lorb_ba_window_dev* w, lorb_ba_plan* P, bool sorted) {
  lorb_ba_devbuild& b = *P->devb;
  hipStream_t s = ctx->stream;
  BaDev& d = P->dev;
  const int C = b.C, F = b.F, Kc = w->max_obs;
  const size_t nrb = 8 + (size_t)C + (size_t)C * C;
  const int nb_obs = lorb::ceil_div(std::max(Kc, 1), 256), nb_pt = lorb::ceil_div(std::max(b.P_cap, 1), 256);
  if (b.pinned_n < nrb) {
    if (b.pinned) (void)hipHostFree(b.pinned);
    b.pinned = nullptr; b.pinned_n = 0;
    LORB_HIP(ctx, hipHostMalloc(reinterpret_cast<void**>(&b.pinned), sizeof(int) * nrb));
    b.pinned_n = nrb;
  }
  if (!b.rb_ev) LORB_HIP(ctx, hipEventCreateWithFlags(&b.rb_ev, hipEventDisableTiming));
  if (b.dirty) LORB_HIP(ctx, hipMemsetAsync(b.scr, 0, b.scr_bytes, s));
  b.dirty = true;
  const bool fuse = sorted && C > 0 && sizeof(int) * ((size_t)C * C + C) <= (size_t)kDbFuseLds;
  if (sorted) {
    const size_t lds = sizeof(unsigned long long) * kDbWords * std::max(C, 1) +
                       (fuse ? sizeof(int) * ((size_t)C * C + C) : 0);
    hipLaunchKernelGGL(fuse ? k_db_sorted<true> : k_db_sorted<false>, dim3(lorb::ceil_div(Kc + 1, 256)), dim3(256), lds, s,
                       *w, C, F, b.Wd, const_cast<int*>(d.pt_obs_off), b.hdr, b.bits, b.cov, b.cam_cnt);
  } else {
    hipLaunchKernelGGL(k_db_keys, dim3(nb_obs), dim3(256), 0, s, *w, C, F, b.Wd, b.pt_cnt, b.hdr, b.bits);
    hipLaunchKernelGGL(k_db_scan1, dim3(1), dim3(1024), 0, s, b.pt_cnt, const_cast<int*>(d.pt_obs_off), b.P_cap + 1,
                       w->d_n_points, b.hdr);
    if (Kc > 0) {
      hipLaunchKernelGGL(k_db_scatter, dim3(nb_obs), dim3(256), 0, s, *w, C, F, d.pt_obs_off, b.pt_cnt, b.val_out);
      hipLaunchKernelGGL(k_db_segsort, dim3(nb_pt), dim3(256), 0, s, *w, d.pt_obs_off, b.val_out, b.key_out);
    }
  }
  if (C > 0 && !fuse)
    hipLaunchKernelGGL(k_db_cov, dim3(lorb::ceil_div(C * (C + 1) / 2, 4)), dim3(256), 0, s, C, b.Wd, b.bits, b.cov,
                       b.cam_cnt);
  LORB_CHECK_LAUNCH(ctx);
  LORB_HIP(ctx, hipMemcpyAsync(b.pinned, b.hdr, sizeof(int) * nrb, hipMemcpyDeviceToHost, s));
  LORB_HIP(ctx, hipEventRecord(b.rb_ev, s));
  b.rb_sorted = sorted;
  b.rb_fuse = fuse;
  b.rb_pending = true;
  return LORB_OK;
}

int db_phase1_wait(lorb_ctx* ctx, const lorb_ba_window_dev* w, lorb_ba_plan* P) {
  lorb_ba_devbuild& b = *P->devb;
  for (;;) {
    b.rb_pending = false;
    LORB_HIP(ctx, lorb::spin_wait(b.rb_ev));
    if (!(b.rb_sorted && (b.pinned[2] & 16))) return LORB_OK;
    b.sorted_hint = false;
    LORB_TRY(db_phase1_issue(ctx, w, P, false));
  }
}

int dev_build_issue(lorb_ctx* ctx, const lorb_ba_window_dev* w, lorb_ba_plan* P, int* lerr_out) {
  lorb_ba_devbuild& b = *P->devb;
  const bool shape_ok = w->n_poses == b.C && w->n_fixed == b.F && w->max_obs <= b.K_cap && w->max_points <= b.P_cap;
  *lerr_out = shape_ok ? 0 : 32;
  if (!shape_ok && !P->comm)
    return lorb::set_error(ctx, LORB_E_INVALID, "window shape differs from the plan's (cameras %d/%d, fixed %d/%d)",
                           w->n_poses, b.C, w->n_fixed, b.F);
  if (!shape_ok) return LORB_OK;
  const int rc = db_phase1_issue(ctx, w, P, b.sorted_hint);
  if (rc != LORB_OK && P->comm) { *lerr_out |= 64; return LORB_OK; }
  return rc;
}

struct HostPhase {
  using Clock = std::chrono::steady_clock;
  lorb_ba_plan* P;
  const bool on;
  const Clock::time_point t0 = Clock::now();
  Clock::time_point last = t0;
  void mark(int k) {
    if (!on) return;
    const auto now = Clock::now();
    P->hp_sec[k] += std::chrono::duration<double, std::micro>(now - last).count();
    if (k == 5) { P->hp_us += std::chrono::duration<double, std::micro>(now - t0).count(); P->hp_n++; }
    last = now;
  }
};

struct DbBuild {
  int K, maxk, Pn, K_all;
  const int *cov, *cam_cnt;
  const int *gcov, *gcam;
  std::vector<int> g_int;
  std::vector<BlockPair> bps;
  int n_pairs = 0, bw = 0;
  int S, G, SF, NSG;
  long long part_total;
};

int db_land(lorb_ctx* ctx, const lorb_ba_window_dev* w, lorb_ba_plan* P, int lerr, int phase_rc, DbBuild& r) {
  lorb_ba_devbuild& b = *P->devb;
  const bool shape_ok = !(lerr & 32), fuse = b.rb_fuse;
  const int C = b.C;
  const size_t nrb = 8 + (size_t)C + (size_t)C * C;
  if (phase_rc != LORB_OK) {
    if (!P->comm) return phase_rc;
    lerr |= 64;
  }
  b.h_copy.resize(nrb);
  if (lerr) std::fill(b.h_copy.begin(), b.h_copy.end(), 0);
  else std::memcpy(b.h_copy.data(), b.pinned, sizeof(int) * nrb);
  int* H = b.h_copy.data();
  if (fuse)
    for (int i = 0; i < C; ++i)
      for (int j = i + 1; j < C; ++j) H[8 + (size_t)i * C + j] = H[8 + (size_t)j * C + i];
  r.K = r.K_all = H[0]; r.maxk = H[1]; r.Pn = H[3];
  r.cov = r.gcov = H + 8;
  r.cam_cnt = r.gcam = r.cov + (size_t)C * C;
  const int err = H[2], Pn = r.Pn;
  int gerr = err, gmaxk = r.maxk;
// ... 298 lines not shown
```

lorb_slam_amd/csrc/lorb_ba_chol.hip:

```cpp
#ifndef LORB_NO_CONTRACT
#pragma clang fp contract(fast)
#endif
#include "lorb_ba_math.h"
#include "lorb_internal.h"
#include "lorb_ba_dev.h"

namespace {

using namespace lorb::ba;

typedef double v4d __attribute__((ext_vector_type(4)));

__device__ __forceinline__ void wave_sync_lds() {
  __builtin_amdgcn_s_waitcnt(0xc07f);
  __builtin_amdgcn_wave_barrier();
}

constexpr int NB = 16;

__device__ __forceinline__ void chol_trail_tile(double* A, int bw, int kb, int ke, int rlast,
                                                int I, int J, int lane) {
  if (16 * (I - J) - 15 > bw) return;
  const int ci = lane & 15, ck = lane >> 4;
  const int i0 = ke + 16 * I, j0 = ke + 16 * J;
  v4d acc;
#pragma unroll
  for (int r = 0; r < 4; ++r) {
    const int i = i0 + ck + 4 * r, j = j0 + ci;
    const bool ok = i <= rlast && j <= i && i - j <= bw;
    const double v = band(A, bw, ok ? i : ke, ok ? j : ke);
    acc[r] = ok ? v : 0.0;
  }
#pragma unroll
  for (int kk = 0; kk < NB / 4; ++kk) {
    const int k = kb + 4 * kk + ck;
    const int ia = i0 + ci, jb = j0 + ci;
    const bool oka = ia <= rlast && ia - k <= bw, okb = jb <= rlast && jb - k <= bw;
    const double a = band(A, bw, oka ? ia : k, k), b = band(A, bw, okb ? jb : k, k);
    acc = __builtin_amdgcn_mfma_f64_16x16x4f64(oka ? -a : 0.0, okb ? b : 0.0, acc, 0, 0, 0);
  }
#pragma unroll
  for (int r = 0; r < 4; ++r) {
    const int i = i0 + ck + 4 * r, j = j0 + ci;
    if (i <= rlast && j <= i && i - j <= bw) band(A, bw, i, j) = acc[r];
  }
}

template <bool IN_LDS, int RPL>
__global__ __launch_bounds__(256) void k_ba_chol(BaDev d) {
  extern __shared__ __attribute__((aligned(16))) double smem[];
  __shared__ int s_fail;
  __shared__ __attribute__((aligned(16))) double s_col[80];
  __shared__ double s_l[NB][NB + 1], s_zk[NB], s_y[NB];
  const int w = blockIdx.x;
  if (d.st[w].done) return;
  if (d.sharded && d.wfail[w] > 0.0) {
    if (threadIdx.x == 0) d.st[w].chol_fail = 1;
    return;
  }
  const BaWin W = d.win[w];
  const int n = W.n, bw = W.bw;
  const int t = threadIdx.x, lane = t & 63, wv = t >> 6;
  double *A, *z, *invd;
  if (IN_LDS) {
    A = smem;
    z = smem + (size_t)n * (bw + 1);
    invd = z + n;
    const double* src = d.env + W.env_base;
    for (int k = t; k < n * (bw + 1); k += 256) A[k] = src[k];
    for (int k = t; k < n; k += 256) z[k] = d.rhs[W.row_base + k];
  } else {
    A = d.env + W.env_base;
    z = d.rhs + W.row_base;
    invd = d.ycam + W.row_base;
  }
  if (t == 0) s_fail = 0;
  __syncthreads();
  int pkb = -1, pke = 0, prl = 0;
  for (int kb = 0; kb < n; kb += NB) {
    const int ke = min(kb + NB, n);
    const int rlast = min(n - 1, ke - 1 + bw);
    if (wv != 0 && pkb >= 0) {
      const int m = ((prl - pke + 1 + 15) >> 4) - 1;
      for (int tt = wv - 1; tt < m * (m + 1) / 2; tt += 3) {
        int I = 0;
        while ((I + 1) * (I + 2) / 2 <= tt) ++I;
        chol_trail_tile(A, bw, pkb, pke, prl, I + 1, tt - I * (I + 1) / 2 + 1, lane);
      }
    }
    if (wv == 0) {
      double P[RPL][NB], zr[RPL];
#pragma unroll
      for (int r = 0; r < RPL; ++r) {
        const int row = kb + lane + 64 * r;
        const bool vr = row <= rlast;
#pragma unroll
        for (int q = 0; q < NB; ++q) {
          const int col = kb + q;
          P[r][q] = (vr && col < ke && col <= row && row - col <= bw) ? band(A, bw, row, col) : 0.0;
        }
        zr[r] = vr ? z[row] : 0.0;
      }
      bool bad = false;
      if (ke - kb == NB) {
        double yq = 0.0;
#pragma unroll
        for (int q = 0; q < NB; ++q) {
          const double akk = readlane_d(P[0][q], q);
          bad |= !(akk > 0.0);
          const double y = rsqrt_refined(akk);
#pragma unroll
          for (int r = 0; r < RPL; ++r) P[r][q] *= y;
          yq = lane == q ? y : yq;
          const double zk = readlane_d(zr[0], q) * y;
          zr[0] = lane > q ? fma(-P[0][q], zk, zr[0]) : (lane == q ? zk : zr[0]);
#pragma unroll
          for (int r = 1; r < RPL; ++r) zr[r] = fma(-P[r][q], zk, zr[r]);
#pragma unroll
          for (int q2 = q + 1; q2 < NB; ++q2) {
            const double l = readlane_d(P[0][q], q2);
#pragma unroll
            for (int r = 0; r < RPL; ++r) P[r][q2] = fma(-P[r][q], l, P[r][q2]);
          }
        }
        if (lane < NB) invd[kb + lane] = yq;
      } else {
#pragma unroll
      for (int q = 0; q < NB; ++q) {
        const int k = kb + q;
        if (k < ke && !bad) {
          const double akk = readlane_d(P[0][q], q);
          if (!(akk > 0.0)) {
            bad = true;
          } else {
            const double y = rsqrt_refined(akk);
#pragma unroll
            for (int r = 0; r < RPL; ++r) {
              const int row = kb + lane + 64 * r;
              if (row > k) P[r][q] *= y;
            }
            if (lane == q) { P[0][q] = akk * y; zr[0] *= y; invd[k] = y; s_col[64] = zr[0]; }
            s_col[lane] = P[0][q];
            wave_sync_lds();
            const double zk = s_col[64];
            double l[NB];
#pragma unroll
            for (int q2 = q + 1; q2 < NB; ++q2) l[q2] = s_col[q2];
#pragma unroll
            for (int r = 0; r < RPL; ++r) {
              const int row = kb + lane + 64 * r;
              if (row > k) zr[r] -= P[r][q] * zk;
            }
#pragma unroll
            for (int q2 = q + 1; q2 < NB; ++q2) {
#pragma unroll
              for (int r = 0; r < RPL; ++r) {
                const int row = kb + lane + 64 * r;
                if (row >= kb + q2) P[r][q2] -= P[r][q] * l[q2];
              }
            }
            wave_sync_lds();
          }
        }
      }
      }
#pragma unroll
      for (int r = 0; r < RPL; ++r) {
        const int row = kb + lane + 64 * r;
        if (row <= rlast) {
#pragma unroll
          for (int q = 0; q < NB; ++q) {
            const int col = kb + q;
            if (col < ke && col <= row && row - col <= bw) band(A, bw, row, col) = P[r][q];
          }
          z[row] = zr[r];
        }
      }
      if (!bad && kb + 64 * RPL <= rlast) {
        const int nq = ke - kb;
        if (lane < NB) {
#pragma unroll
          for (int q = 0; q < NB; ++q) s_l[lane][q] = P[0][q];
          s_zk[lane] = zr[0];
          s_y[lane] = lane < nq ? invd[kb + lane] : 0.0;
        }
        wave_sync_lds();
        for (int r0 = kb + 64 * RPL; r0 <= rlast; r0 += 64) {
          const int row = r0 + lane;
          const bool vr = row <= rlast;
          double X[NB], zx = vr ? z[row] : 0.0;
#pragma unroll
          for (int q = 0; q < NB; ++q) X[q] = (vr && q < nq && row - (kb + q) <= bw) ? band(A, bw, row, kb + q) : 0.0;
#pragma unroll
          for (int q = 0; q < NB; ++q) {
            if (q < nq) {
              X[q] *= s_y[q];
              zx = fma(-X[q], s_zk[q], zx);
#pragma unroll
              for (int q2 = q + 1; q2 < NB; ++q2) X[q2] = fma(-X[q], s_l[q2][q], X[q2]);
            }
          }
          if (vr) {
#pragma unroll
            for (int q = 0; q < NB; ++q)
              if (q < nq && row - (kb + q) <= bw) band(A, bw, row, kb + q) = X[q];
            z[row] = zx;
          }
        }
        wave_sync_lds();
      }
      if (bad && lane == 0) s_fail = 1;
    }
    __syncthreads();
    if (s_fail) break;
    {
      const int nt = (rlast - ke + 1 + 15) >> 4;
      for (int I = wv; I < nt; I += 4) chol_trail_tile(A, bw, kb, ke, rlast, I, 0, lane);
      pkb = kb; pke = ke; prl = rlast;
    }
    __syncthreads();
  }
  if (s_fail) {
    if (t == 0) d.st[w].chol_fail = 1;
    return;
  }
  if (wv == 0) {
    for (int bb = ((n - 1) / 64) * 64; bb >= 0; bb -= 64) {
      const int row = bb + lane;
      const int be = min(n - 1, bb + 63);
      double zr = row < n ? z[row] : 0.0;
      constexpr int BC = 8;
      for (int k0 = be; k0 >= bb; k0 -= BC) {
        double lk[BC], iv[BC];
#pragma unroll
        for (int u = 0; u < BC; ++u) {
          const int k = max(k0 - u, bb);
          const bool ok = k0 - u >= bb && row < k && k - row <= bw;
          lk[u] = band(A, bw, k, ok ? row : k);
          lk[u] = ok ? lk[u] : 0.0;
          iv[u] = invd[k];
        }
#pragma unroll
        for (int u = 0; u < BC; ++u) {
          const int k = k0 - u;
          if (k >= bb) {
            const double yk = readlane_d(zr, k - bb) * iv[u];
            zr = lane == k - bb ? yk : fma(-lk[u], yk, zr);
          }
        }
      }
      if (row < n) z[row] = zr;
      wave_sync_lds();
      for (int i = max(0, bb - bw) + lane; i < bb; i += 64) {
        double acc = 0.0;
        const int kend = min(be, i + bw);
        for (int k = bb; k <= kend; k += BC) {
          double a[BC], zk[BC];
#pragma unroll
          for (int u = 0; u < BC; ++u) {
            const int kk = min(k + u, kend);
            a[u] = band(A, bw, kk, i);
            zk[u] = z[kk];
          }
#pragma unroll
          for (int u = 0; u < BC; ++u) acc = fma(k + u <= kend ? a[u] : 0.0, zk[u], acc);
        }
        z[i] -= acc;
      }
      wave_sync_lds();
    }
  }
  __syncthreads();
  for (int k = t; k < n; k += 256) d.ycam[W.row_base + k] = z[k];
  {
    const int cur = d.st[w].cur;
    for (int ci = t; ci < W.n_poses; ci += 256) {
      const int c = W.pose_base + ci;
      double xn[6];
#pragma unroll
      for (int k = 0; k < 6; ++k) {
        xn[k] = d.x_pose[cur][6 * c + k] + (-z[6 * ci + k]) * d.scale_pose[6 * c + k];
        d.x_pose[cur ^ 1][6 * c + k] = xn[k];
      }
      d.rot_cand[c] = lorb::rot_val(xn);
    }
  }
}

__device__ __forceinline__ constexpr int tri4(int I, int J) { return I * (I + 1) / 2 + J; }

__global__ __launch_bounds__(256) void k_ba_chol_w(BaDev d) {
  extern __shared__ __attribute__((aligned(16))) double smem[];
  const int w = blockIdx.x;
  if (d.st[w].done) return;
  if (d.sharded && d.wfail[w] > 0.0) {
    if (threadIdx.x == 0) d.st[w].chol_fail = 1;
    return;
  }
  const BaWin W = d.win[w];
  const int n = W.n, bw = W.bw;
  const int n16 = (n + 15) & ~15;
  const int t = threadIdx.x, lane = t & 63, ci = lane & 15, ck = lane >> 4;
  double* A = smem;
  double* z = A + (size_t)n16 * (bw + 1);
  double* invd = z + n16;
  double* xch = invd + n16;
  const int dummy = (int)(xch + 64 * 17 + lane - A);
  {
    const double* __restrict__ S = d.env + W.env_base;
    const int ne = n * (bw + 1);
    for (int k = t; k < ne; k += 256) A[k] = S[k];
    for (int k = ne + t; k < n16 * (bw + 1); k += 256) A[k] = (k % (bw + 1)) == bw ? 1.0 : 0.0;
    for (int k = t; k < n16; k += 256) z[k] = k < n ? d.rhs[W.row_base + k] : 0.0;
  }
  __syncthreads();
  if (t >= 64) return;
  auto sget = [&](int i, int j) -> double {
    const bool ok = j <= i && i - j <= bw && i < n16;
    const double v = A[ok ? i * (bw + 1) + (j - i + bw) : 0];
    return ok ? v : 0.0;
  };
  v4d T[10], Tn[4];
#pragma unroll
  for (int I = 0; I < 4; ++I)
#pragma unroll
    for (int J = 0; J <= I; ++J)
#pragma unroll
      for (int r = 0; r < 4; ++r) T[tri4(I, J)][r] = sget(16 * I + ck + 4 * r, 16 * J + ci);
  double zr = z[lane];
  bool bad = false;
  for (int kb = 0; kb < n16; kb += 16) {
#pragma unroll
    for (int J = 0; J < 4; ++J)
#pragma unroll
      for (int r = 0; r < 4; ++r) Tn[J][r] = sget(kb + 64 + ck + 4 * r, kb + 16 + 16 * J + ci);
    const double zin = kb + 16 + lane < n16 ? z[kb + 16 + lane] : 0.0;
#pragma unroll
    for (int I = 0; I < 4; ++I)
#pragma unroll
      for (int r = 0; r < 4; ++r) xch[(16 * I + ck + 4 * r) * 17 + ci] = T[tri4(I, 0)][r];
    wave_sync_lds();
    double P[NB];
#pragma unroll
    for (int q = 0; q < NB; ++q) P[q] = xch[lane * 17 + q];
    wave_sync_lds();
    double yq = 0.0;
#pragma unroll
    for (int q = 0; q < NB; ++q) {
      const double akk = readlane_d(P[q], q);
      bad |= !(akk > 0.0);
      const double y = rsqrt_refined(akk);
      P[q] *= y;
      yq = lane == q ? y : yq;
      const double zk = readlane_d(zr, q) * y;
      zr = lane > q ? fma(-P[q], zk, zr) : (lane == q ? zk : zr);
#pragma unroll
      for (int q2 = q + 1; q2 < NB; ++q2) {
        const double l = readlane_d(P[q], q2);
        P[q2] = fma(-P[q], l, P[q2]);
      }
    }
    {
      const int row = kb + lane;
#pragma unroll
      for (int q = 0; q < NB; ++q) {
        const int col = kb + q;
        const bool ok = row < n16 && col <= row && row - col <= bw;
        A[ok ? row * (bw + 1) + (col - row + bw) : dummy] = P[q];
        xch[lane * 17 + q] = P[q];
      }
      if (lane < NB) { z[row] = zr; invd[row] = yq; }
    }
    wave_sync_lds();
    double opA[4][4];
#pragma unroll
    for (int I = 1; I < 4; ++I)
#pragma unroll
      for (int kk = 0; kk < 4; ++kk) opA[I][kk] = xch[(16 * I + ci) * 17 + 4 * kk + ck];
#pragma unroll
    for (int J = 1; J < 4; ++J)
#pragma unroll
      for (int I = J; I < 4; ++I)
#pragma unroll
        for (int kk = 0; kk < 4; ++kk)
          T[tri4(I, J)] = __builtin_amdgcn_mfma_f64_16x16x4f64(-opA[I][kk], opA[J][kk], T[tri4(I, J)], 0, 0, 0);
    {
      const double zs = __shfl_down(zr, 16, 64);
      zr = lane < 48 ? zs : zin;
    }
    T[tri4(0, 0)] = T[tri4(1, 1)];
    T[tri4(1, 0)] = T[tri4(2, 1)]; T[tri4(1, 1)] = T[tri4(2, 2)];
    T[tri4(2, 0)] = T[tri4(3, 1)]; T[tri4(2, 1)] = T[tri4(3, 2)]; T[tri4(2, 2)] = T[tri4(3, 3)];
#pragma unroll
    for (int J = 0; J < 4; ++J) T[tri4(3, J)] = Tn[J];
  }
  if (bad) {
    if (lane == 0) d.st[w].chol_fail = 1;
    return;
  }
  wave_sync_lds();
  {
    const int jc = lane & 15, g = lane >> 4;
    for (int c0 = n16 - 16; c0 >= 0; c0 -= 16) {
      const int j = c0 + jc;
      double lk[NB];
#pragma unroll
      for (int k = 0; k < NB; ++k) {
        const bool ok = k > jc && k - jc <= bw;
        const double v = A[ok ? (c0 + k) * (bw + 1) + (j - (c0 + k) + bw) : 0];
        lk[k] = ok ? v : 0.0;
      }
      const int iend = min(n16 - 1, j + bw);
      double av[16], zv[16];
#pragma unroll
      for (int u = 0; u < 16; ++u) {
        const int i = c0 + 16 + g + 4 * u;
        const bool ok = i <= iend;
        av[u] = A[ok ? i * (bw + 1) + (j - i + bw) : 0];
        zv[u] = z[ok ? i : 0];
        av[u] = ok ? av[u] : 0.0;
      }
      double a4[4] = {0.0, 0.0, 0.0, 0.0};
#pragma unroll
      for (int u = 0; u < 16; ++u) a4[u & 3] = fma(av[u], zv[u], a4[u & 3]);
      double acc = (a4[0] + a4[1]) + (a4[2] + a4[3]);
      {
        double a, b;
        xrow_pair<false>(acc, a, b); acc = a + b;
        xrow_pair<true>(acc, a, b); acc = a + b;
      }
      double zb = z[j] - acc;
      const double iv = invd[j];
#pragma unroll
      for (int k = NB - 1; k >= 0; --k) {
        const double yk = readlane_d(zb, k) * readlane_d(iv, k);
        zb = jc == k ? yk : fma(-lk[k], yk, zb);
      }
      if (g == 0) z[j] = zb;
      wave_sync_lds();
    }
  }
  for (int k = lane; k < n; k += 64) d.ycam[W.row_base + k] = z[k];
  const int cur = d.st[w].cur;
  for (int ci2 = lane; ci2 < W.n_poses; ci2 += 64) {
    const int c = W.pose_base + ci2;
    double xn[6];
#pragma unroll
    for (int k = 0; k < 6; ++k) {
      xn[k] = d.x_pose[cur][6 * c + k] + (-z[6 * ci2 + k]) * d.scale_pose[6 * c + k];
      d.x_pose[cur ^ 1][6 * c + k] = xn[k];
    }
    d.rot_cand[c] = lorb::rot_val(xn);
  }
}

__device__ __forceinline__ void wait_bit(unsigned long long* mask, int b) {
  while (!((__hip_atomic_load(mask, __ATOMIC_ACQUIRE, __HIP_MEMORY_SCOPE_WORKGROUP) >> b) & 1ull))
    __builtin_amdgcn_s_sleep(1);
}
template <bool SLEEP>
__device__ __forceinline__ void wait_ge(int* c, int v) {
  while (__hip_atomic_load(c, __ATOMIC_ACQUIRE, __HIP_MEMORY_SCOPE_WORKGROUP) < v)
    if (SLEEP) __builtin_amdgcn_s_sleep(1);
}

constexpr int kCS = 65;
struct BandSide {
  double* A;
  double* z;
  double* xch;
  int rows, bw, lane;
  int base, si, sj;
  unsigned long long* mask = nullptr;
  int* pdone = nullptr;
  int nbk = 0, dir = 0;
  int zslot = 0;
  double* kco = nullptr;
  unsigned long long* trace = nullptr;
  int tslot = 0;
  int bslot = 320;
  unsigned long long t0 = 0;
  __device__ __forceinline__ void tr(int k) const {
#ifdef LORB_CHOL_TRACE
    if (trace && lane == 0) trace[tslot + k] = __builtin_amdgcn_s_memtime() - t0;
#endif
  }

  __device__ __forceinline__ int idx(int i, int j) const { return base + si * i + sj * j; }

  __device__ __forceinline__ double get(int i, int j) const {
    const bool ok = j <= i && i - j <= bw && i < rows;
    const double v = A[ok ? idx(i, j) : base];
    return ok ? v : 0.0;
  }
  __device__ __forceinline__ void init_tiles(v4d (&T)[10]) const {
#pragma unroll
    for (int I = 1; I < 4; ++I)
#pragma unroll
      for (int J = 1; J <= I; ++J)
#pragma unroll
        for (int r = 0; r < 4; ++r) T[tri4(I, J)][r] = get(16 * I + (lane >> 4) + 4 * r, 16 * J + (lane & 15));
  }
  __device__ __forceinline__ void init_panel(double (&P)[NB], double& zr) const {
#pragma unroll
    for (int q = 0; q < NB; ++q) P[q] = get(lane, q);
    zr = lane < rows ? z[lane] : 0.0;
  }
  __device__ __forceinline__ void chain(double (&P)[NB], double& zr, bool& bad, int kb0, int kend, bool pre,
                                        int* lrd, int* prd, int& pwant, const double* pb) const {
    const int dstep = 16 * (si + sj);
    unsigned l_ok = 0;
#pragma unroll
    for (int q = 0; q < NB; ++q) l_ok |= (unsigned)(q <= lane && lane - q <= bw) << q;
    int l_base = idx(kb0 + lane, kb0);
    double* colbuf = xch;
    double* dummy = xch + 16 * kCS + lane;
    for (int kb = kb0; kb < kend; kb += 16) {
      int lane = this->lane, lok = (int)l_ok;
      asm volatile("" : "+v"(lane), "+v"(lok));
      if (!(pre && kb == kb0)) {
        wait_ge<false>(prd, ++pwant);
#pragma unroll
        for (int q = 0; q < NB; ++q) P[q] = pb[lane * 17 + q];
      }
      tr(0);
      const double zin = kb + 16 + lane < rows ? z[kb + 16 + lane] : 0.0;
      double yq = 0.0;
      double mp[NB];
#pragma unroll
      for (int q2 = 0; q2 < NB; ++q2) mp[q2] = 0.0;
      double akk = readlane_d(P[0], 0);
#pragma unroll
      for (int q = 0; q < NB; ++q) {
        bad |= !(akk > 0.0);
        double y = __builtin_amdgcn_rsq(akk);
        __builtin_amdgcn_sched_barrier(0);
        if (q >= 1) {
#pragma unroll
          for (int q2 = q + 1; q2 < NB; ++q2) P[q2] = fma(-P[q - 1], mp[q2], P[q2]);
        }
        {
          const double e = fma(-akk * y, y, 1.0);
          y = fma(0.5 * y, e, y);
        }
        P[q] *= y;
        yq = lane == q ? y : yq;
        const double zk = readlane_d(zr, q) * y;
        zr = lane > q ? fma(-P[q], zk, zr) : (lane == q ? zk : zr);
        colbuf[q * kCS + lane] = P[q];
        if (q + 1 < NB) {
          const double l1 = readlane_d(P[q], q + 1);
          P[q + 1] = fma(-P[q], l1, P[q + 1]);
          akk = readlane_d(P[q + 1], q + 1);
#pragma unroll
          for (int q2 = q + 2; q2 < NB; ++q2) mp[q2] = colbuf[q * kCS + q2];
        }
      }
      tr(1);
      const bool rowvalid = kb + lane < rows;
      if (lane == 0) __hip_atomic_fetch_add(lrd, 1, __ATOMIC_RELEASE, __HIP_MEMORY_SCOPE_WORKGROUP);
#pragma unroll
      for (int q = 0; q < NB; ++q) {
        const bool ok = rowvalid && (((unsigned)lok >> q) & 1u);
        *(ok ? A + l_base + q * sj : dummy) = q == lane ? yq : P[q];
      }
      l_base += dstep;
      if (lane < NB) z[kb + lane] = zr;
      if (lane == 0 && pdone) __hip_atomic_fetch_add(pdone, 1, __ATOMIC_RELEASE, __HIP_MEMORY_SCOPE_WORKGROUP);
      const double zs = __shfl_down(zr, 16, 64);
      zr = lane < 48 ? zs : zin;
      tr(2);
      const_cast<BandSide*>(this)->tslot += 3;
    }
  }
  __device__ __forceinline__ void update(v4d (&T)[10], int kb0, int kend, int* lrd, int* prd, int& lwant,
                                         double* pb) const {
    const int ci = lane & 15, ck = lane >> 4;
    const int dstep = 16 * (si + sj);
    int tn_addr = idx(kb0 + 64 + ck, kb0 + 16 + ci);
    unsigned tn_ok = 0;
#pragma unroll
    for (int J = 0; J < 4; ++J)
#pragma unroll
      for (int r = 0; r < 4; ++r) {
        const int i = 64 + ck + 4 * r, j = 16 + 16 * J + ci;
        tn_ok |= (unsigned)(j <= i && i - j <= bw) << (4 * J + r);
      }
    for (int kb = kb0; kb < kend; kb += 16) {
      int tok = (int)tn_ok;
      asm volatile("" : "+v"(tok));
      if (mask) {
        const int b = dir > 0 ? kb / 16 + 4 : nbk - 5 - kb / 16;
        if (b >= 0 && b < nbk) wait_bit(mask, b);
      }
      v4d Tn[4];
#pragma unroll
      for (int J = 0; J < 4; ++J)
#pragma unroll
        for (int r = 0; r < 4; ++r) {
          const bool ok = (((unsigned)tok >> (4 * J + r)) & 1u) && kb + 64 + ck + 4 * r < rows;
          const double v = A[ok ? tn_addr + 4 * r * si + 16 * J * sj : base];
          Tn[J][r] = ok ? v : 0.0;
        }
      tn_addr += dstep;
      const bool nxt = kb + 16 < kend;
      tr(0);
// ... 244 lines not shown
__device__ __forceinline__ void stage_band(const double2* __restrict__ S2, double* Ab, int j0, int j1, int tid,
                                           int nthr, int n, int bw, int nsrc) {
  const int B1 = bw + 1;
  for (int jb = j0 + tid; jb < j1; jb += nthr * U) {
    double2 v[U];
#pragma unroll
    for (int u = 0; u < U; ++u) {
      const int j = jb + nthr * u;
      v[u] = S2[(j < j1 && j < nsrc) ? j : 0];
    }
#pragma unroll
    for (int u = 0; u < U; ++u) {
      const int j = jb + nthr * u;
      if (j < j1) {
        int i = (2 * j) / B1, off = (2 * j) % B1;
        double e[2] = {v[u].x, v[u].y};
#pragma unroll
        for (int h = 0; h < 2; ++h) {
          const bool in = i < n && i - (bw - off) >= 0;
          e[h] = in ? e[h] : ((i >= n && off == bw) ? 1.0 : 0.0);
          if (++off == B1) { off = 0; ++i; }
        }
        reinterpret_cast<double2*>(Ab)[j] = double2{e[0], e[1]};
      }
    }
  }
}


template <int U>
__device__ __forceinline__ void stage_band2(const double2* __restrict__ S2, double* Ab, int a0, int a1, int b0, int b1,
                                            int tid, int nthr, int n, int bw, int nsrc) {
  const int B1 = bw + 1, la = a1 - a0, tot = la + (b1 - b0);
  for (int vb = tid; vb < tot; vb += nthr * U) {
    double2 v[U];
    int jj[U];
#pragma unroll
    for (int u = 0; u < U; ++u) {
      const int vv = vb + nthr * u;
      jj[u] = vv < la ? a0 + vv : b0 + (vv - la);
      v[u] = S2[(vv < tot && jj[u] < nsrc) ? jj[u] : 0];
    }
#pragma unroll
    for (int u = 0; u < U; ++u) {
      const int j = jj[u];
      if (vb + nthr * u < tot) {
        int i = (2 * j) / B1, off = (2 * j) % B1;
        double e[2] = {v[u].x, v[u].y};
#pragma unroll
        for (int h = 0; h < 2; ++h) {
          const bool in = i < n && i - (bw - off) >= 0;
          e[h] = in ? e[h] : ((i >= n && off == bw) ? 1.0 : 0.0);
          if (++off == B1) { off = 0; ++i; }
        }
        reinterpret_cast<double2*>(Ab)[j] = double2{e[0], e[1]};
      }
    }
  }
}

__device__ __forceinline__ void stage_fix(const BaDev& d, const LMOpt& o, double* Ab, const BaWin& W, double radius,
                                          int r0, int r1, int tid, int nthr) {
  r1 = min(r1, W.n);
  const int B1 = W.bw + 1;
  for (int q = tid; q < (r1 - r0) * 6; q += nthr) {
    const int i = r0 + q / 6, i6 = i % 6, j6 = q % 6;
    if (j6 != i6) continue;
    const int c = W.pose_base + i / 6;
    const double* sc = d.scale_pose + 6 * c;
    double v = d.U[21 * c + u21(i6, j6)] * sc[i6] * sc[j6];
    v = 0.0 + fmin(fmax(v, o.min_diag), o.max_diag) / radius;
    double& e = Ab[i * B1 + (j6 - i6 + W.bw)];
    e = e + v;
  }
}

__device__ __forceinline__ double stage_fix_val(const BaDev& d, const LMOpt& o, const BaWin& W, double radius,
                                                int r0, int r1, int q, int& at) {
  r1 = min(r1, W.n);
  at = -1;
  if (q >= (r1 - r0) * 6) return 0.0;
  const int i = r0 + q / 6, i6 = i % 6, j6 = q % 6;
  if (j6 != i6) return 0.0;
  const int c = W.pose_base + i / 6;
  const double* sc = d.scale_pose + 6 * c;
  double v = d.U[21 * c + u21(i6, j6)] * sc[i6] * sc[j6];
  v = 0.0 + fmin(fmax(v, o.min_diag), o.max_diag) / radius;
  at = i * (W.bw + 1) + (j6 - i6 + W.bw);
  return v;
}

struct StageBlk {
  static __device__ __forceinline__ double pinned_load(const double* p) {
    return __hip_atomic_load(p, __ATOMIC_RELAXED, __HIP_MEMORY_SCOPE_WAVEFRONT);
  }
  double2 v[7];
  double fu[2], fs[2];
  int fa[2];
  template <bool FIX>
  __device__ __forceinline__ void load(const BaDev& d, const BaWin& W, const double2* __restrict__ S2, int b, int cpb,
                                       int nch, int nsrc, int lane) {
    const int j0 = b * cpb, j1 = min(j0 + cpb, nch);
    const double* Sd = reinterpret_cast<const double*>(S2);
#pragma unroll
    for (int u = 0; u < 7; ++u) {
      const int j = j0 + lane + 64 * u;
      const int js = (j < j1 && j < nsrc) ? j : 0;
      v[u].x = pinned_load(Sd + 2 * js);
      v[u].y = pinned_load(Sd + 2 * js + 1);
    }
    if (FIX) {
      const int rows = min(16 * b + 16, W.n) - 16 * b;
#pragma unroll
      for (int h = 0; h < 2; ++h) {
        const int q = lane + 64 * h;
        const int i = 16 * b + q / 6, i6 = i % 6, j6 = q % 6;
        const bool on = q < rows * 6 && j6 == i6;
        const int c = W.pose_base + (on ? i / 6 : 0);
        fu[h] = pinned_load(&d.U[21 * c + (on ? u21(i6, i6) : 0)]);
        fs[h] = pinned_load(&d.scale_pose[6 * c + (on ? i6 : 0)]);
        fa[h] = on ? i * (W.bw + 1) + W.bw : -1;
      }
    }
  }
  template <bool FIX>
  __device__ __forceinline__ void store(const LMOpt& o, double radius, double* Ab, int b, int cpb, int nch,
                                        int lane) const {
    const int j0 = b * cpb, j1 = min(j0 + cpb, nch);
#pragma unroll
    for (int u = 0; u < 7; ++u) {
      const int j = j0 + lane + 64 * u;
      if (j < j1) reinterpret_cast<double2*>(Ab)[j] = v[u];
    }
    if (FIX) {
      wave_sync_lds();
#pragma unroll
      for (int h = 0; h < 2; ++h) {
        double t = fu[h] * fs[h] * fs[h];
        t = 0.0 + fmin(fmax(t, o.min_diag), o.max_diag) / radius;
        if (fa[h] >= 0) Ab[fa[h]] = Ab[fa[h]] + t;
      }
    }
  }
};

constexpr int kChol2sThreads = 512;

template <bool HEAD>
__device__ __forceinline__ void chol_2s_run(const BaDev& d, const LMOpt& o, const int w) {
  extern __shared__ __attribute__((aligned(16))) double smem[];
  __shared__ int s_bad;
  __shared__ int s_head_done;

  const BaWin W = d.win[w];
  const WinState S0 = d.st[w];
  const int done = S0.done;
  const double wfail = d.sharded ? d.wfail[w] : 0.0;
  if (done) return;
  if (wfail > 0.0) {
    if (HEAD) {
      if (threadIdx.x < 64) {
        const WinState S = lm_head<true>(d, o, w, threadIdx.x, S0, W);
        if (threadIdx.x == 0 && !S.done) d.st[w].chol_fail = 1;
      }
    } else if (threadIdx.x == 0) {
      d.st[w].chol_fail = 1;
    }
    return;
  }
#ifdef LORB_CHOL_TRACE
  if (threadIdx.x == 0) d.dbg[512 * w + 250] = __builtin_amdgcn_s_memtime();
#endif
  constexpr int NT = kChol2sThreads;
  const int n = W.n, bw = W.bw, B1 = bw + 1;
  const int n16 = (n + 15) & ~15;
  const int m = 16 * ((n16 - 48) / 32);
  const int nB = n16 - m - 48;
  const int rt = m + 48, rb = nB + 48;
  const int t = threadIdx.x, lane = t & 63, wv = t >> 6;
  double* Ab = smem;
  double* zt = Ab + n16 * B1;
  double* zb = zt + rt;
  double* xt = zb + rb;
  double* xb = xt + 64 * 18;
  double* zX = xb + 64 * 18;
  double* pbt = zX + 48;
  double* pbb = pbt + 64 * 17;
  double* zero = pbb + 64 * 17;
  __shared__ unsigned long long s_mask;
  __shared__ int s_pdone[2];
  __shared__ int s_linv[2];
  __shared__ int s_lrd[2], s_prd[2];
  __shared__ int s_hand[3];
  __shared__ int s_kdone[2];
  const double2* __restrict__ S2 = reinterpret_cast<const double2*>(d.env + W.env_base);
  const int nch = n16 * B1 / 2, nsrc = n * B1 / 2;
  const int nbk = n16 / 16, ib = 4;
  const bool prog = nbk <= 64 && nbk > 2 * ib;
  const int cpb = 8 * B1;
  static_assert(16 * 4 * 6 <= kChol2sThreads, "one stage_fix item per thread");
  int fa0 = -1, fa1 = -1;
  double fv0 = 0.0, fv1 = 0.0;
  if (HEAD && prog) {
    fv0 = stage_fix_val(d, o, W, S0.radius, 0, 16 * ib, t, fa0);
    fv1 = stage_fix_val(d, o, W, S0.radius, 16 * (nbk - ib), n16, t, fa1);
  }
  const int cur = S0.cur, ep = t - (NT - 128);
  double rz;
  {
    const int row = t < rt ? t : n16 - 1 - (t - rt);
    rz = (t < rt + rb && row < n) ? d.rhs[W.row_base + row] : 0.0;
  }
  if (prog) {
    stage_band2<7>(S2, Ab, 0, ib * cpb, (nbk - ib) * cpb, nch, t, NT, n, bw, nsrc);
  } else {
    stage_band<14>(S2, Ab, 0, nch, t, NT, n, bw, nsrc);
  }
  if (t < rt) zt[t] = rz;
  else if (t < rt + rb) zb[t - rt] = rz;
  for (int k = t + NT; k < rt + rb; k += NT) {
    const int row = k < rt ? k : n16 - 1 - (k - rt);
    double v = row < n ? d.rhs[W.row_base + row] : 0.0;
    if (k < rt) zt[k] = v; else zb[k - rt] = v;
  }
  if (t == 0) {
    *zero = 0.0;
    s_bad = 0;
    s_head_done = 0;
    s_pdone[0] = 0; s_pdone[1] = 0;
    s_linv[0] = 0; s_linv[1] = 0;
    s_lrd[0] = 0; s_lrd[1] = 0; s_prd[0] = 0; s_prd[1] = 0;
    s_hand[0] = 0; s_hand[1] = 0; s_hand[2] = 0;
    s_kdone[0] = 0; s_kdone[1] = 0;
    unsigned long long msk = 0;
    for (int b = 0; b < nbk; ++b) msk |= (unsigned long long)(!prog || b < ib || b >= nbk - ib) << (b & 63);
    s_mask = msk;
  }
  __syncthreads();
  if (HEAD) {
    if (prog) {
      if (fa0 >= 0) Ab[fa0] = Ab[fa0] + fv0;
      if (fa1 >= 0) Ab[fa1] = Ab[fa1] + fv1;
    } else {
      stage_fix(d, o, Ab, W, S0.radius, 0, n16, t, NT);
    }
    __syncthreads();
  }
  BandSide top{Ab, zt, xt, rt, bw, lane, bw, bw, 1};
  BandSide bot{Ab, zb, xb, rb, bw, lane, (n16 - 1) * B1 + bw, -1, -bw};
  top.pdone = &s_pdone[0]; bot.pdone = &s_pdone[1];
  top.zslot = (int)(zero - Ab); bot.zslot = top.zslot;
  top.kco = d.kco + (size_t)((W.row_base >> 4) + w) * 1024;
  bot.kco = top.kco + (size_t)(m >> 4) * 1024;
  top.nbk = bot.nbk = nbk; top.dir = 1; bot.dir = -1;
  if (prog) { top.mask = &s_mask; bot.mask = &s_mask; }
#ifdef LORB_CHOL_TRACE
  const unsigned long long tr0 = __builtin_amdgcn_s_memtime();
  unsigned long long* trb = d.dbg + 512 * w;
  top.trace = trb; bot.trace = trb; top.t0 = tr0; bot.t0 = tr0;
  if (t == 0) trb[252] = tr0;
  top.tslot = wv == 0 ? 0 : 64; bot.tslot = wv == 1 ? 128 : 160;
  top.bslot = 320; bot.bslot = 400;
#define TR1(k) do { if (lane == 0) trb[200 + (k)] = __builtin_amdgcn_s_memtime() - tr0; } while (0)
#else
#define TR1(k) do {} while (0)
#endif
  const int side = wv & 1;
  const BandSide& me = side == 0 ? top : bot;
  double* pb = side == 0 ? pbt : pbb;
  int* lrd = &s_lrd[side];
  int* prd = &s_prd[side];
  int lwant = 0, pwant = 0;
  bool bad = false;
  double zr = 0.0;
  double P[NB];
  v4d T[10];
  if (wv >= 6) {
    if (prog) {
      const int lo = ib, hi = nbk - ib, mid = (lo + hi) / 2;
      const int nk = side == 0 ? mid - lo : hi - mid;
      auto blk = [&](int k) { return side == 0 ? lo + k : hi - 1 - k; };
      auto put = [&](const StageBlk& R, int b) {
        R.template store<HEAD>(o, S0.radius, Ab, b, cpb, nch, lane);
        if (lane == 0) __hip_atomic_fetch_or(&s_mask, 1ull << b, __ATOMIC_RELEASE, __HIP_MEMORY_SCOPE_WORKGROUP);
      };
      for (int k = 0; k < nk; ++k) {
        StageBlk R;
        R.template load<HEAD>(d, W, S2, blk(k), cpb, nch, nsrc, lane);
        put(R, blk(k));
      }
    }
    TR1(8 + side);
  }
  if (HEAD && wv == 4) {
    const WinState S = d.sharded ? lm_head<true>(d, o, w, lane, S0, W) : lm_head<false>(d, o, w, lane, S0, W);
    if (lane == 0) s_head_done = S.done;
  }
  if (wv == 4 || wv == 5) {
    int* pd = &s_pdone[side];
    const int nblk = (side == 0 ? m : nB) / 16;
    for (int p = 0; p < nblk; ++p) {
      while (__hip_atomic_load(pd, __ATOMIC_ACQUIRE, __HIP_MEMORY_SCOPE_WORKGROUP) <= p) __builtin_amdgcn_s_sleep(1);
      TR1(56 + 32 * side + 2 * p);
      me.linv(16 * p);
      if (lane == 0) __hip_atomic_fetch_add(&s_linv[side], 1, __ATOMIC_RELEASE, __HIP_MEMORY_SCOPE_WORKGROUP);
      TR1(57 + 32 * side + 2 * p);
    }
    TR1(10 + side);
  } else if (wv < 2) {
    me.init_panel(P, zr);
    me.chain(P, zr, bad, 0, side == 0 ? m : nB, true, lrd, prd, pwant, pb);
  } else if (wv < 4) {
    me.init_tiles(T);
    me.update(T, 0, side == 0 ? m : nB, lrd, prd, lwant, pb);
  }
  auto build_ops = [&](int ks, int par) {
    const BandSide& kside = ks == 0 ? top : bot;
    const int nkb = (ks == 0 ? m : nB) / 16;
    wait_ge<true>(&s_linv[ks], nkb);
    TR1(16 + 2 * ks);
    for (int b = nkb - 1 - par; b >= 0; b -= 2) kside.bsk_block(16 * b);
    __builtin_amdgcn_s_waitcnt(0x0f70);
    if (lane == 0) __hip_atomic_fetch_add(&s_kdone[ks], 1, __ATOMIC_RELEASE, __HIP_MEMORY_SCOPE_WORKGROUP);
    TR1(17 + 2 * ks);
  };
  if (wv == 5 || wv == 7) build_ops(0, wv == 7);
  double* X = xt;
  if (wv == 3) {
    wait_ge<true>(&s_hand[0], 1);
#pragma unroll
    for (int I = 0; I < 3; ++I)
#pragma unroll
      for (int J = 0; J <= I; ++J)
#pragma unroll
        for (int r = 0; r < 4; ++r) {
          const int rho = 16 * I + (lane >> 4) + 4 * r, kap = 16 * J + (lane & 15);
          X[(47 - kap) * 48 + (47 - rho)] = T[tri4(I, J)][r];
          (void)kap; (void)rho;
        }
    if (lane == 0) __hip_atomic_fetch_add(&s_hand[1], 1, __ATOMIC_RELEASE, __HIP_MEMORY_SCOPE_WORKGROUP);
    TR1(2);
  }
  if (wv == 1) {
    if (lane < 48) zX[47 - lane] = zr;
    if (bad) s_bad = 1;
    if (lane == 0) __hip_atomic_fetch_add(&s_hand[2], 1, __ATOMIC_RELEASE, __HIP_MEMORY_SCOPE_WORKGROUP);
  }
  if (wv == 1 || wv == 3) build_ops(1, wv == 3);
  if (wv == 2) {
    TR1(0);
    if (lane == 0) __hip_atomic_fetch_add(&s_hand[0], 1, __ATOMIC_RELEASE, __HIP_MEMORY_SCOPE_WORKGROUP);
    wait_ge<true>(&s_hand[1], 1);
    TR1(1);
  }
  if (wv == 0) wait_ge<true>(&s_hand[2], 1);
  if (wv == 2) {
#pragma unroll
    for (int I = 0; I < 3; ++I)
#pragma unroll
      for (int J = 0; J <= I; ++J)
#pragma unroll
        for (int r = 0; r < 4; ++r) {
          const int rho = 16 * I + (lane >> 4) + 4 * r, kap = 16 * J + (lane & 15);
          T[tri4(I, J)][r] += X[rho * 48 + kap] - top.get(m + rho, m + kap);
        }
#pragma unroll
    for (int J = 0; J < 4; ++J) T[tri4(3, J)] = v4d{0.0, 0.0, 0.0, 0.0};
    TR1(14);
    BandSide topM = top;
    topM.mask = nullptr; topM.pdone = nullptr;
    {
      const int ci = lane & 15, ck = lane >> 4;
#pragma unroll
      for (int I = 0; I < 4; ++I)
#pragma unroll
        for (int r = 0; r < 4; ++r) pbt[(16 * I + ck + 4 * r) * 17 + ci] = T[tri4(I, 0)][r];
      if (lane == 0) __hip_atomic_fetch_add(&s_prd[0], 1, __ATOMIC_RELEASE, __HIP_MEMORY_SCOPE_WORKGROUP);
    }
    TR1(15);
    topM.update(T, m, m + 48, &s_lrd[0], &s_prd[0], lwant, pbt);
  } else if (wv == 0) {
    zr = lane < 48 ? zr + zX[lane] - zt[m + lane] : 0.0;
    BandSide topM = top;
    topM.mask = nullptr; topM.pdone = nullptr;
    TR1(3);
    topM.chain(P, zr, bad, m, m + 48, false, &s_lrd[0], &s_prd[0], pwant, pbt);
    TR1(4);
    if (bad) s_bad = 1;
  }
  double cf[16];
  BandSide::BsWin S{0.0};
  if (wv == 0) {
    wait_ge<true>(&s_kdone[0], 2);
    top.bsk_load(m - 16, cf);
    S = BandSide::BsWin{top.bs_init(m + 32, 0)};
    TR1(5);
    top.bs_run<false>(S, m + 32, m);
    TR1(6);
    if (lane < 48) zb[nB + 47 - lane] = zt[m + lane];
    if (lane == 0) __hip_atomic_fetch_add(&s_hand[0], 1, __ATOMIC_RELEASE, __HIP_MEMORY_SCOPE_WORKGROUP);
  } else if (wv == 1) {
    wait_ge<true>(&s_kdone[1], 2);
    bot.bsk_load(nB - 16, cf);
    double lb[48];
    const int brow = bot.bs_row(nB - 16);
#pragma unroll
    for (int k = 0; k < 48; ++k) {
      const bool ok = brow >= 0 && nB + k - brow <= bw;
      const double v = Ab[ok ? bot.idx(nB + k, brow) : bot.base];
      lb[k] = ok ? v : 0.0;
    }
#pragma unroll
    for (int k = 0; k < 48; ++k) asm volatile("" : "+v"(lb[k]));
    wait_ge<true>(&s_hand[0], 2);
    TR1(20);
    double b4[4] = {0.0, 0.0, 0.0, 0.0};
    const double2* zm2 = reinterpret_cast<const double2*>(zb + nB);
#pragma unroll
    for (int k2 = 0; k2 < 24; ++k2) {
      const double2 v = zm2[k2];
      b4[(2 * k2) & 3] = fma(lb[2 * k2], v.x, b4[(2 * k2) & 3]);
      b4[(2 * k2 + 1) & 3] = fma(lb[2 * k2 + 1], v.y, b4[(2 * k2 + 1) & 3]);
    }
    const double bzw = (brow >= 0 ? zb[brow] : 0.0) - ((b4[0] + b4[1]) + (b4[2] + b4[3]));
    S = BandSide::BsWin{bzw};
    TR1(21);
  }
  if (wv < 2) {
    const BandSide g = wv == 0 ? top : bot;
    g.bs_run_k(S, (wv == 0 ? m : nB) - 16, 0, cf);
    TR1(wv == 0 ? 7 : 12);
  }
  __syncthreads();
  TR1(13);
#undef TR1
  if (s_bad) {
    if (t == 0) d.st[w].chol_fail = 1;
    return;
  }
  if (HEAD && s_head_done) return;
  for (int k = t; k < n; k += NT) d.ycam[W.row_base + k] = k < rt ? zt[k] : zb[n16 - 1 - k];
  for (int ci2 = ep; ep >= 0 && ci2 < W.n_poses; ci2 += 128) {
    const int c = W.pose_base + ci2;
    double xn[6];
#pragma unroll
    for (int k = 0; k < 6; ++k) {
      const int row = 6 * ci2 + k;
      const double y = row < rt ? zt[row] : zb[n16 - 1 - row];
      const double xp = d.x_pose[cur][6 * c + k];
      const double sp = d.scale_pose[6 * c + k];
      xn[k] = xp + (-y) * sp;
      d.x_pose[cur ^ 1][6 * c + k] = xn[k];
    }
    d.rot_cand[c] = lorb::rot_val(xn);
  }
#ifdef LORB_CHOL_TRACE
  if (t == 0) d.dbg[512 * w + 251] = __builtin_amdgcn_s_memtime();
#endif
}
template <bool HEAD>
__global__ __launch_bounds__(kChol2sThreads) void k_ba_chol_2s(BaDev d, LMOpt o) { chol_2s_run<HEAD>(d, o, blockIdx.x); }

template <bool HEAD>
__global__ __launch_bounds__(kChol2sThreads) void k_ba_chol_2s_g(BaGrp g, GrpGrid G, LMOpt o) {
  unsigned lb;
  const int k = grp_member(G, g.n, blockIdx.x, lb);
  chol_2s_run<HEAD>(g.d[k], o, (int)lb);
}

}

namespace lorb {
namespace ba {

void launch_chol(int kind, const CholShape& sh, hipStream_t s, const BaDev& d, const LMOpt& o, bool head) {
  if (kind == 2) {
    if (head)
      hipLaunchKernelGGL(k_ba_chol_2s<true>, dim3(sh.W), dim3(kChol2sThreads), sizeof(double) * (size_t)sh.max_env_w, s, d, o);
    else
      hipLaunchKernelGGL(k_ba_chol_2s<false>, dim3(sh.W), dim3(kChol2sThreads), sizeof(double) * (size_t)sh.max_env_w, s, d, o);
  } else if (kind == 1) {
    hipLaunchKernelGGL(k_ba_chol_w, dim3(sh.W), dim3(256), sizeof(double) * (size_t)sh.max_env_w, s, d);
  } else if (kind == 0) {
    const size_t lds = sizeof(double) * (size_t)sh.max_env;
    const bool in_lds = lds <= (size_t)kLdsBudget;
    const int rows = NB + sh.max_bw;
    const int rpl = rows <= 64 ? 1 : rows <= 128 ? 2 : rows <= 256 ? 4 : 8;
#define LORB_CHOL(L, R) hipLaunchKernelGGL((k_ba_chol<L, R>), dim3(sh.W), dim3(256), L ? lds : 0, s, d)
    if (in_lds) { if (rpl == 1) LORB_CHOL(true, 1); else if (rpl == 2) LORB_CHOL(true, 2); else if (rpl == 4) LORB_CHOL(true, 4); else LORB_CHOL(true, 8); }
    else { if (rpl == 1) LORB_CHOL(false, 1); else if (rpl == 2) LORB_CHOL(false, 2); else if (rpl == 4) LORB_CHOL(false, 4); else LORB_CHOL(false, 8); }
#undef LORB_CHOL
  }
}

void launch_chol_2s_g(hipStream_t s, const BaGrp& g, const GrpGrid& G, const LMOpt& o, bool head, size_t lds) {
  if (head) hipLaunchKernelGGL(k_ba_chol_2s_g<true>, dim3(G.pre[g.n]), dim3(kChol2sThreads), lds, s, g, G, o);
  else hipLaunchKernelGGL(k_ba_chol_2s_g<false>, dim3(G.pre[g.n]), dim3(kChol2sThreads), lds, s, g, G, o);
}

}
}
```

lorb_slam_amd/csrc/lorb_ba_dev.h:

```cpp
#pragma once
#include "lorb_ba_math.h"
#include "lorb_internal.h"

namespace lorb {
namespace ba {

constexpr int kGB = 256;

struct BaWin {
  int pose_base, n_poses, point_base, n_points;
  int pblk_base, n_pblk;
  int env_base, env_size, n, row_base, bw;
  int obs_base, n_obs;
  int n_obs_all;
  int part_stride, part_cam, bwc, pad_;
  int sg_base, n_sg;
  long long part_base;
  double fx, fy, cx, cy;
};
struct PBlk { int win, p0, cnt, o0, no; };
struct BlockPair { int win, ch, cl, off, cnt; };
struct WinState {
  double radius, decrease_factor, cost, x_norm, gmax, initial_cost;
  int iter, n_success, n_invalid, done, relin, cur, last_successful, term, chol_fail, pad;
// ... 19 lines not shown
  const auto h = W32 ? __builtin_amdgcn_permlane32_swap(hi, hi, false, false)
                     : __builtin_amdgcn_permlane16_swap(hi, hi, false, false);
  a = __longlong_as_double(((unsigned long long)h[0] << 32) | l[0]);
  b = __longlong_as_double(((unsigned long long)h[1] << 32) | l[1]);
}
__device__ __forceinline__ double wave_sum(double v) {
  double a, b;
  xrow_pair<true>(v, a, b); v = a + b;
  xrow_pair<false>(v, a, b); v = a + b;
  v += dpp_d<0x128>(v);
  v += dpp_d<0x124>(v);
  v += dpp_d<0x4E>(v);
  v += dpp_d<0xB1>(v);
  return v;
}
__device__ __forceinline__ double wave_max(double v) {
  double a, b;
  xrow_pair<true>(v, a, b); v = fmax(a, b);
  xrow_pair<false>(v, a, b); v = fmax(a, b);
  v = fmax(v, dpp_d<0x128>(v));
  v = fmax(v, dpp_d<0x124>(v));
  v = fmax(v, dpp_d<0x4E>(v));
  v = fmax(v, dpp_d<0xB1>(v));
  return v;
}
__device__ __forceinline__ double readlane_d(double v, int l);
__device__ __forceinline__ void swap_pair(double x, double y, bool w32, double& r0, double& r1) {
  const unsigned long long ux = __double_as_longlong(x), uy = __double_as_longlong(y);
  const unsigned xl = (unsigned)ux, xh = (unsigned)(ux >> 32), yl = (unsigned)uy, yh = (unsigned)(uy >> 32);
  const auto l = w32 ? __builtin_amdgcn_permlane32_swap(xl, yl, false, false)
                     : __builtin_amdgcn_permlane16_swap(xl, yl, false, false);
  const auto h = w32 ? __builtin_amdgcn_permlane32_swap(xh, yh, false, false)
                     : __builtin_amdgcn_permlane16_swap(xh, yh, false, false);
  r0 = __longlong_as_double(((unsigned long long)h[0] << 32) | l[0]);
  r1 = __longlong_as_double(((unsigned long long)h[1] << 32) | l[1]);
}
template <int CTRL, int BIT, int H>
__device__ __forceinline__ void rs_dpp_step(double (&v)[32], int lane) {
  const bool up = (lane >> BIT) & 1;
#pragma unroll
  for (int k = 0; k < H; ++k) {
    const double keep = up ? v[k + H] : v[k], send = up ? v[k] : v[k + H];
    v[k] = keep + dpp_d<CTRL>(send);
  }
}
template <int N>
__device__ __forceinline__ void wave_sum_all(double (&v)[32]) {
  static_assert(N <= 32, "at most 32 values");
  const int lane = threadIdx.x & 63;
#pragma unroll
  for (int k = N; k < 32; ++k) v[k] = 0.0;
#pragma unroll
  for (int k = 0; k < 16; ++k) {
    double a, b;
    swap_pair(v[k], v[k + 16], true, a, b);
    v[k] = a + b;
  }
#pragma unroll
  for (int k = 0; k < 8; ++k) {
    double a, b;
    swap_pair(v[k], v[k + 8], false, a, b);
    v[k] = a + b;
  }
  rs_dpp_step<0x128, 3, 4>(v, lane);
  rs_dpp_step<0x141, 2, 2>(v, lane);
  rs_dpp_step<0x4E, 1, 1>(v, lane);
  v[0] += dpp_d<0xB1>(v[0]);
  const double r = v[0];
#pragma unroll
  for (int k = 0; k < N; ++k) v[k] = readlane_d(r, 2 * k);
}
template <int N>
__device__ __forceinline__ void block_sum(double (&v)[N], double* sh ) {
  const int t = threadIdx.x;
#pragma unroll
  for (int k = 0; k < N; ++k) sh[k * 256 + t] = v[k];
  __syncthreads();
  for (int s = 128; s > 0; s >>= 1) {
    if (t < s) {
#pragma unroll
      for (int k = 0; k < N; ++k) sh[k * 256 + t] += sh[k * 256 + t + s];
    }
    __syncthreads();
  }
#pragma unroll
  for (int k = 0; k < N; ++k) v[k] = sh[k * 256];
  __syncthreads();
}

__device__ __forceinline__ bool inv3(const double a[6], double inv[6]) {
  const double l00 = a[0];
  if (!(l00 > 0.0)) return false;
  const double L00 = sqrt(l00);
  const double L10 = a[1] / L00, L20 = a[2] / L00;
  const double d1 = a[3] - L10 * L10;
  if (!(d1 > 0.0)) return false;
  const double L11 = sqrt(d1);
  const double L21 = (a[4] - L20 * L10) / L11;
  const double d2 = a[5] - L20 * L20 - L21 * L21;
  if (!(d2 > 0.0)) return false;
  const double L22 = sqrt(d2);
  const double i00 = 1.0 / L00, i11 = 1.0 / L11, i22 = 1.0 / L22;
  const double i10 = -L10 * i00 * i11;
  const double i21 = -L21 * i11 * i22;
  const double i20 = -(L20 * i00 + L21 * i10) * i22;
  inv[0] = i00 * i00 + i10 * i10 + i20 * i20;
  inv[1] = i10 * i11 + i20 * i21;
  inv[2] = i20 * i22;
  inv[3] = i11 * i11 + i21 * i21;
  inv[4] = i21 * i22;
  inv[5] = i22 * i22;
  return true;
}
__device__ __forceinline__ double s3(const double m[6], int a, int b) {
  if (a > b) { const int t = a; a = b; b = t; }
  return m[a * 3 - (a * (a - 1)) / 2 + (b - a)];
}

struct BaDev {
  lorb::RotJet* rot_lin;
  lorb::RotVal* rot_cand;
  lorb::RotJet* rot_fix;
  lorb::RotVal* rotv_fix;
  const BaWin* win;
  const PBlk* pblk;
  const int* obs_pt;
  const BlockPair* bp;
  const int* pt_obs_off;
  const int* obs_cam;
  const int* obs_fix;
  const double2* obs_uv;
  const double* fixed_pose;
  double* x_init_pose;
  double* x_init_pt;
  double* x_pose[2];
  double* x_pt[2];
  double* scale_pose;
  double* scale_pt;
  double* etb;
  double* pinv;
  double* U;
  double* V;
  double* env;
  double* rhs;
  double *U_part, *V_part, *wlin, *wlin_part, *wmax, *wmax_part;
  double *env_part, *rhs_part, *wfail, *wfail_part, *wstep, *wstep_part;
  const int* cam_active;
  int sharded, rank0;
  double* ycam;
  double* part;
  unsigned long long* dbg;
  double* kco;
  WinState* st;
  double* gpart;
  int2* gspan;
  const int4* sgrp;
  lorb_lm_iteration* trace;
  const int* live;
};

__device__ __forceinline__ int u21(int a, int b) {
  if (a > b) { const int t = a; a = b; b = t; }
  return a * 6 - (a * (a - 1)) / 2 + (b - a);
}

__device__ __forceinline__ double readlane_d(double v, int l) {
  const unsigned long long u = __double_as_longlong(v);
  const int lo = __builtin_amdgcn_readlane((int)(u & 0xffffffffu), l);
  const int hi = __builtin_amdgcn_readlane((int)(u >> 32), l);
  return __longlong_as_double(((unsigned long long)(unsigned)hi << 32) | (unsigned)lo);
}

__device__ __forceinline__ double& band(double* A, int bw, int i, int j) {
  return A[(size_t)i * (bw + 1) + (j - i + bw)];
}
__host__ __device__ __forceinline__ int pm_slot(int a, int dd, int bwc) {
  return a <= bwc ? a * (a + 1) / 2 + dd : (bwc + 1) * (bwc + 2) / 2 + (a - bwc - 1) * (bwc + 1) + dd;
}
__host__ __device__ __forceinline__ int pm_nslots(int span, int bwc) {
  return span <= 0 ? 0 : pm_slot(span - 1, span - 1 < bwc ? span - 1 : bwc, bwc) + 1;
}

#ifndef LORB_RSQ_STEPS
#define LORB_RSQ_STEPS 2
#endif
__device__ __forceinline__ double rsqrt_refined(double a) {
  double y = __builtin_amdgcn_rsq(a);
#pragma unroll
  for (int s = 0; s < LORB_RSQ_STEPS; ++s) {
    const double e = fma(-a * y, y, 1.0);
    y = fma(0.5 * y, e, y);
  }
  return y;
}

template <int F0, int F1, int F2, bool M1>
__device__ __forceinline__ void group_partials(const double* __restrict__ part, int base, int n, int lane,
                                               double& a, double& b, double& c) {
  constexpr int kPU = 8;
  for (int b0 = lane; b0 < n; b0 += 64 * kPU) {
    double v0[kPU], v1[kPU], v2[kPU];
#pragma unroll
    for (int u = 0; u < kPU; ++u) {
      const int g = b0 + 64 * u;
      const double* P = part + 8 * (base + (g < n ? g : 0));
      v0[u] = P[F0]; v1[u] = P[F1]; v2[u] = P[F2];
    }
#pragma unroll
    for (int u = 0; u < kPU; ++u)
      if (b0 + 64 * u < n) {
        a += v0[u];
        b = M1 ? fmax(b, v1[u]) : b + v1[u];
        c += v2[u];
      }
  }
}

template <bool SH>
__device__ __forceinline__ WinState lm_head(const BaDev& d, const LMOpt& o, int w, int lane, WinState S, const BaWin& W) {
  if (S.relin) {
    double cost = 0.0, gm = 0.0, xn2 = 0.0;
    if (!SH) group_partials<0, 1, 2, true>(d.part, W.pblk_base, W.n_pblk, lane, cost, gm, xn2);
    const int cur = S.cur;
    for (int c = W.pose_base + lane; c < W.pose_base + W.n_poses; c += 64) {
      if (S.iter == 0) {
        const int dg[6] = {0, 6, 11, 15, 18, 20};
        for (int k = 0; k < 6; ++k) d.scale_pose[6 * c + k] = 1.0 / (1.0 + sqrt(d.U[21 * c + dg[k]]));
      }
      if (!d.cam_active[c]) continue;
      for (int k = 0; k < 6; ++k) {
        const double x = d.x_pose[cur][6 * c + k];
        gm = fmax(gm, fabs(x - (x + -d.V[6 * c + k])));
        xn2 += x * x;
      }
    }
    cost = wave_sum(cost); gm = wave_max(gm); xn2 = wave_sum(xn2);
    if (SH) { cost += d.wlin[2 * w]; xn2 += d.wlin[2 * w + 1]; gm = fmax(gm, d.wmax[w]); }
    S.cost = cost;
    S.gmax = gm;
    S.x_norm = sqrt(xn2);
    if (S.iter == 0) S.initial_cost = cost;
    S.last_successful = 1;
    S.relin = 0;
  }
  if (lane == 0) {
    if (S.iter >= o.max_iter) { S.done = 1; S.term = LORB_TERM_NO_CONVERGENCE; }
    else if (S.last_successful && S.gmax <= o.gtol) { S.done = 1; S.term = LORB_TERM_GRADIENT_TOL; }
    else if (S.radius <= o.min_radius) { S.done = 1; S.term = LORB_TERM_MIN_RADIUS; }
    else S.iter++;
    d.st[w] = S;
  }
  return S;
}

__host__ __device__ constexpr int chol2s_words(int n16, int bw) {
  return n16 * (bw + 1) + (n16 + 48) + 2 * 64 * 18 + 48 + 2 * 64 * 17 + 2;
}
constexpr int chol_lds_words(int n16, int bw) {
  const int w1 = n16 * (bw + 1) + 2 * n16 + 64 * 18, w2 = (n16 + 48) * (bw + 2) + 2 * 64 * 18 + 48;
  const int w3 = chol2s_words(n16, bw);
  return w1 > w2 ? (w1 > w3 ? w1 : w3) : (w2 > w3 ? w2 : w3);
}

constexpr int kGrpMax = 4;
struct BaGrp {
  BaDev d[kGrpMax];
  int n;
};
struct GrpGrid {
  int pre[kGrpMax + 1];
};
struct GrpInit {
  int W[kGrpMax], ctot[kGrpMax], n_pt[kGrpMax], nf[kGrpMax];
};
__device__ __forceinline__ int grp_member(const GrpGrid& G, int n, unsigned b, unsigned& lb) {
  int k = 0;
#pragma unroll
  for (int i = 1; i < kGrpMax; ++i) k += (i < n && (int)b >= G.pre[i]) ? 1 : 0;
  lb = b - (unsigned)G.pre[k];
  return k;
}


constexpr int kLdsBudget = 160 * 1024 - 2048;
struct CholShape { int W, max_env, max_env_w, max_bw; };
void launch_chol(int kind, const CholShape& sh, hipStream_t s, const BaDev& d, const LMOpt& o, bool head);
void launch_chol_2s_g(hipStream_t s, const BaGrp& g, const GrpGrid& G, const LMOpt& o, bool head, size_t lds);

}
}
```

lorb_slam_amd/csrc/lorb_ba_plan.h:

```cpp
#pragma once
#include "lorb_ba_dev.h"

#include <algorithm>
#include <cstring>
#include <vector>

namespace lorb::ba {

inline bool env_flag(const char* name) { const char* e = getenv(name); return e && e[0] == '1'; }

inline size_t dbg_words(size_t windows, size_t stamp_slots) {
#ifdef LORB_CHOL_TRACE
  return windows * 512;
#elif defined(LORB_LS_STAMPS)
  return stamp_slots * 8;
#else
  return windows * 8;
#endif
}

struct GraphCache {
  const char* what;
  hipGraph_t graph = nullptr;
  hipGraphExec_t exec = nullptr;
  bool valid = false;
  int captures = 0;
  explicit GraphCache(const char* what_) : what(what_) {}
  GraphCache(const GraphCache&) = delete;
  GraphCache& operator=(const GraphCache&) = delete;
  ~GraphCache() { destroy(); }
  void invalidate() { valid = false; }
  template <typename F, typename R>
  int replay_or_capture(lorb_ctx* ctx, bool same, F enqueue, R remember) {
    if (!valid || !same) {
      destroy();
      LORB_HIP(ctx, hipStreamBeginCapture(ctx->stream, hipStreamCaptureModeThreadLocal));
      const int rc = enqueue();
      hipGraph_t g = nullptr;
      const hipError_t e = hipStreamEndCapture(ctx->stream, &g);
      if (rc != LORB_OK) { if (g) (void)hipGraphDestroy(g); return rc; }
      if (e != hipSuccess) return lorb::set_error(ctx, LORB_E_DEVICE, "%s capture failed: %s", what, hipGetErrorString(e));
      graph = g;
      LORB_HIP(ctx, hipGraphInstantiate(&exec, graph, nullptr, nullptr, 0));
      remember();
      valid = true;
      captures++;
    }
    LORB_HIP(ctx, hipGraphLaunch(exec, ctx->stream));
    return LORB_OK;
  }

 private:
  void destroy() {
    if (exec) { (void)hipGraphExecDestroy(exec); exec = nullptr; }
    if (graph) { (void)hipGraphDestroy(graph); graph = nullptr; }
    valid = false;
  }
};

}

struct lorb_ba_devbuild;

struct lorb_ba_plan {
  lorb_ctx* ctx = nullptr;
  int W = 0, Ctot = 0, Ptot = 0, K = 0, NF = 0, n_pblk = 0, n_bp = 0, n_pairs = 0;
  int env_total = 0, n_total = 0, max_env = 0, max_bw = 0, max_env_w = 0, min_n16 = 1 << 30;
  int min_bw = 1 << 30;
  double hp_us = 0.0, hp_sec[6] = {};
  int hp_n = 0;
  std::vector<lorb::ba::BaWin> hwin;
  std::vector<void*> allocs;
  lorb::ba::BaDev dev{};
  lorb::ba::WinState* d_state = nullptr;
  lorb::ba::GraphCache cache{"graph"};
  lorb::ba::LMOpt graph_opt{};
  unsigned gen = 0;
  struct GraphKey {
    int kind = -1, lds = 0, memset_env = 0, env_total = 0, grid_pblk = 0, grid_bp = 0, pt_launch = 0, x2_n = 0;
    int red_wide = 0, sup = 0, grid_sg = 0;
    bool operator==(const GraphKey& o) const { return memcmp(this, &o, sizeof(GraphKey)) == 0; }
  } gkey;
  int grid_pblk = 0, grid_bp = 0;
  int grid_sg = 0;
  bool has_super = false;
  int pt_launch = 0;
  int* live = nullptr;
  lorb_comm* comm = nullptr;
  double *x2_send = nullptr, *x2_recv = nullptr;
  size_t fx_n = 0;
  size_t x2_off = 0;
  std::vector<std::vector<int>> cam_map;
  int chol_kind = -1;
  lorb_ba_devbuild* devb = nullptr;
  ~lorb_ba_plan();
};
```

Measured before the change: 11310 BA iterations/s.

## Fold LM end-of-iteration decision into the next linearize kernel

Removes the separate k_ba_lm_end launch per iteration by having every linearize block evaluate the LM accept/reject decision redundantly, with a staged state copy (st2) and an ls_fail flag consumed by the fused Cholesky head. Rotation Jacobians for the candidate pose are now computed inside the solver kernels into a double-buffered rot_lin, so an accepted step needs no recomputation pass. The cost is redundant per-block reduction work and extra state buffers, and it is limited to single-node fused Cholesky plans with at most a bounded number of point blocks. It also records the kernel-node count of the captured graph.

After: 11580 BA iterations/s (median of 6 runs). 2.4% higher.

```diff
diff --git a/lorb_slam_amd/csrc/lorb_ba.hip b/lorb_slam_amd/csrc/lorb_ba.hip
--- a/lorb_slam_amd/csrc/lorb_ba.hip
+++ b/lorb_slam_amd/csrc/lorb_ba.hip
@@ -27,6 +27,7 @@
     s.done = d.win[i].n_obs_all == 0 ? 1 : 0;
     s.relin = 1; s.cur = 0; s.last_successful = 1; s.term = 0; s.chol_fail = 0; s.pad = 0;
     d.st[i] = s;
+    d.ls_fail[i] = 0;
     if (d.sharded) d.wfail_part[i] = 0.0;
   }
   if (i < ctot) {
@@ -83,8 +84,9 @@
   }
   return true;
 }
-__device__ __forceinline__ void prep_fail(const BaDev& d, int win) {
-  if (d.sharded) d.wfail_part[win] = 1.0;
+__device__ __forceinline__ void prep_fail(const BaDev& d, int win, int fold) {
+  if (fold) d.ls_fail[win] = 1;
+  else if (d.sharded) d.wfail_part[win] = 1.0;
   else d.st[win].chol_fail = 1;
 }
 
@@ -118,21 +120,33 @@
   lm_begin_run<SH>(d, o, blockIdx.x);
 }
 
-__device__ __forceinline__ void lm_record(const BaDev& d, int w, const WinState& S, int outcome, double mcc,
-                                          double ncost, double step_norm) {
-  if (S.iter < 1 || S.iter > LORB_LM_TRACE_CAP) return;
+__device__ __forceinline__ lorb_lm_iteration lm_rec(const WinState& S, int outcome, double mcc, double ncost,
+                                                    double step_norm) {
   lorb_lm_iteration r;
   r.iteration = S.iter; r.outcome = outcome;
   r.cost = S.cost; r.model_cost_change = mcc; r.new_cost = ncost; r.radius = S.radius; r.step_norm = step_norm;
-  d.trace[(size_t)w * LORB_LM_TRACE_CAP + S.iter - 1] = r;
-}
-
-__device__ int lm_decide(BaDev d, const LMOpt& o, int w, WinState S, bool valid, double mccs,
-                         double ncost, double sn2) {
+  return r;
+}
+__device__ __forceinline__ void lm_record(const BaDev& d, int w, const lorb_lm_iteration& r) {
+  if (r.iteration < 1 || r.iteration > LORB_LM_TRACE_CAP) return;
+  d.trace[(size_t)w * LORB_LM_TRACE_CAP + r.iteration - 1] = r;
+}
+
+__device__ __forceinline__ WinState state_copy(const WinState& s) {
+  WinState r;
+  r.radius = s.radius; r.decrease_factor = s.decrease_factor; r.cost = s.cost; r.x_norm = s.x_norm; r.gmax = s.gmax;
+  r.initial_cost = s.initial_cost; r.iter = s.iter; r.n_success = s.n_success; r.n_invalid = s.n_invalid;
+  r.done = s.done; r.relin = s.relin; r.cur = s.cur; r.last_successful = s.last_successful; r.term = s.term;
+  r.chol_fail = s.chol_fail; r.pad = s.pad;
+  return r;
+}
+
+__device__ __forceinline__ int lm_decide(const LMOpt& o, WinState& S, bool valid, double mccs, double ncost,
+                                         double sn2, lorb_lm_iteration& rec) {
   const double model_cost_change = -mccs;
   valid = valid && isfinite(model_cost_change) && isfinite(sn2) && model_cost_change > 0.0;
   if (!valid) {
-    lm_record(d, w, S, LORB_LM_STEP_INVALID, model_cost_change, ncost, sqrt(sn2));
+    rec = lm_rec(S, LORB_LM_STEP_INVALID, model_cost_change, ncost, sqrt(sn2));
     if (++S.n_invalid >= o.max_invalid) {
       S.done = 1; S.term = LORB_TERM_FAILURE;
     } else {
@@ -141,24 +155,23 @@
       S.last_successful = 0;
       if (S.iter >= o.max_iter) { S.done = 1; S.term = LORB_TERM_NO_CONVERGENCE; }
     }
-    d.st[w] = S;
     return 0;
   }
   S.n_invalid = 0;
   const double new_cost = isfinite(ncost) ? ncost : 1.7976931348623157e308;
   const double step_norm = sqrt(sn2);
   if (step_norm <= o.ptol * (S.x_norm + o.ptol)) {
-    lm_record(d, w, S, LORB_LM_STEP_PARAM_TOL, model_cost_change, new_cost, step_norm);
-    S.done = 1; S.term = LORB_TERM_PARAMETER_TOL; d.st[w] = S; return 0;
+    rec = lm_rec(S, LORB_LM_STEP_PARAM_TOL, model_cost_change, new_cost, step_norm);
+    S.done = 1; S.term = LORB_TERM_PARAMETER_TOL; return 0;
   }
   const double cost_change = S.cost - new_cost;
   if (fabs(cost_change) <= o.ftol * S.cost) {
-    lm_record(d, w, S, LORB_LM_STEP_FUNC_TOL, model_cost_change, new_cost, step_norm);
-    S.done = 1; S.term = LORB_TERM_FUNCTION_TOL; d.st[w] = S; return 0;
+    rec = lm_rec(S, LORB_LM_STEP_FUNC_TOL, model_cost_change, new_cost, step_norm);
+    S.done = 1; S.term = LORB_TERM_FUNCTION_TOL; return 0;
   }
   const double rel = cost_change / model_cost_change;
-  lm_record(d, w, S, rel > o.min_rel ? LORB_LM_STEP_ACCEPTED : LORB_LM_STEP_REJECTED, model_cost_change, new_cost,
-            step_norm);
+  rec = lm_rec(S, rel > o.min_rel ? LORB_LM_STEP_ACCEPTED : LORB_LM_STEP_REJECTED, model_cost_change, new_cost,
+               step_norm);
   if (rel > o.min_rel) {
     S.cur ^= 1;
     S.relin = 1;
@@ -174,58 +187,60 @@
     S.decrease_factor *= 2.0;
   }
   if (S.iter >= o.max_iter) { S.done = 1; S.term = LORB_TERM_NO_CONVERGENCE; }
-  d.st[w] = S;
   return rel > o.min_rel;
 }
 
+template <bool SH>
+__device__ __forceinline__ void lm_end_eval(const BaDev& d, const LMOpt& o, int w, int lane, WinState& S,
+                                            const BaWin& W, lorb_lm_iteration& rec) {
+  bool valid = !S.chol_fail;
+  double mccs = 0.0, ncost = 0.0, sn2 = 0.0;
+  if (valid) {
+    const int cur = S.cur;
+    const int c0 = W.pose_base + lane;
+    const bool has0 = lane < W.n_poses;
+    const double* xp = cur ? d.x_pose[1] : d.x_pose[0];
+    const double* xpn = cur ? d.x_pose[0] : d.x_pose[1];
+    double x0[6], xn0[6];
+    bool act0 = false;
+    if (has0) {
+      act0 = d.cam_active[c0];
+#pragma unroll
+      for (int k = 0; k < 6; ++k) { x0[k] = xp[6 * c0 + k]; xn0[k] = xpn[6 * c0 + k]; }
+    }
+    if (!SH) group_partials<3, 4, 5, false>(d.part, W.pblk_base, W.n_pblk, lane, mccs, ncost, sn2);
+    if (has0) {
+#pragma unroll
+      for (int k = 0; k < 6; ++k) {
+        if (act0) sn2 += (x0[k] - xn0[k]) * (x0[k] - xn0[k]);
+      }
+    }
+    for (int c = c0 + 64; c < W.pose_base + W.n_poses; c += 64) {
+      const bool active = d.cam_active[c];
+      for (int k = 0; k < 6; ++k) {
+        const double x = xp[6 * c + k];
+        const double xn = xpn[6 * c + k];
+        if (active) sn2 += (x - xn) * (x - xn);
+      }
+    }
+    mccs = wave_sum(mccs); ncost = wave_sum(ncost); sn2 = wave_sum(sn2);
+    if (SH) { mccs += d.wstep[3 * w]; ncost += d.wstep[3 * w + 1]; sn2 += d.wstep[3 * w + 2]; }
+  }
+  S.chol_fail = 0;
+  if (lane == 0) (void)lm_decide(o, S, valid, mccs, ncost, sn2, rec);
+}
 template <bool SH>
 __device__ __forceinline__ void lm_end_run(const BaDev& d, const LMOpt& o, int w, int lane) {
   const WinState* Sp = d.st + w;
   WinState S = *Sp;
   const BaWin W = d.win[w];
   if (S.done) return;
-  bool valid = !S.chol_fail;
-  double mccs = 0.0, ncost = 0.0, sn2 = 0.0;
-  double xc[6] = {0, 0, 0, 0, 0, 0};
-  if (valid) {
-    const int cur = S.cur;
-    const int c0 = W.pose_base + lane;
-    const bool has0 = lane < W.n_poses;
-    double x0[6], xn0[6];
-    bool act0 = false;
-    if (has0) {
-      act0 = d.cam_active[c0];
-#pragma unroll
-      for (int k = 0; k < 6; ++k) { x0[k] = d.x_pose[cur][6 * c0 + k]; xn0[k] = d.x_pose[cur ^ 1][6 * c0 + k]; }
-    }
-    if (!SH) group_partials<3, 4, 5, false>(d.part, W.pblk_base, W.n_pblk, lane, mccs, ncost, sn2);
-    if (has0) {
-#pragma unroll
-      for (int k = 0; k < 6; ++k) {
-        if (act0) sn2 += (x0[k] - xn0[k]) * (x0[k] - xn0[k]);
-        xc[k] = xn0[k];
-      }
-    }
-    for (int c = c0 + 64; c < W.pose_base + W.n_poses; c += 64) {
-      const bool active = d.cam_active[c];
-      for (int k = 0; k < 6; ++k) {
-        const double x = d.x_pose[cur][6 * c + k];
-        const double xn = d.x_pose[cur ^ 1][6 * c + k];
-        if (active) sn2 += (x - xn) * (x - xn);
-      }
-    }
-    mccs = wave_sum(mccs); ncost = wave_sum(ncost); sn2 = wave_sum(sn2);
-    if (SH) { mccs += d.wstep[3 * w]; ncost += d.wstep[3 * w + 1]; sn2 += d.wstep[3 * w + 2]; }
-  }
-  S.chol_fail = 0;
-  if (SH && lane == 0) d.wfail_part[w] = 0.0;
-  int acc = 0;
-  if (lane == 0) acc = lm_decide(d, o, w, S, valid, mccs, ncost, sn2);
-  acc = __builtin_amdgcn_readfirstlane(acc);
-  if (acc) {
-    if (lane < W.n_poses) d.rot_lin[W.pose_base + lane] = lorb::rot_jet(xc);
-    for (int c = W.pose_base + lane + 64; c < W.pose_base + W.n_poses; c += 64)
-      d.rot_lin[c] = lorb::rot_jet(d.x_pose[S.cur ^ 1] + 6 * c);
+  lorb_lm_iteration rec;
+  lm_end_eval<SH>(d, o, w, lane, S, W, rec);
+  if (lane == 0) {
+    if (SH) d.wfail_part[w] = 0.0;
+    d.st[w] = S;
+    lm_record(d, w, rec);
   }
 }
 template <bool SH>
@@ -265,7 +280,12 @@
   for (int k = 1; k < NW; ++k) { a += red[0][k]; b = M1 ? fmax(b, red[1][k]) : b + red[1][k]; c += red[2][k]; }
 }
 
-__device__ __forceinline__ void pm_lin(const BaDev& d, const BaWin& W, int cur, int p, int c, int fx, double2 uv,
+__device__ __forceinline__ int rot_idx(const BaDev& d, int cur, int c) {
+  int cr = rot_off(d, cur) + c;
+  asm volatile("" : "+v"(cr));
+  return cr;
+}
+__device__ __forceinline__ void pm_lin(const BaDev& d, const BaWin& W, int cur, int cr, int p, int c, int fx, double2 uv,
                                        double (&r)[2], double (&Jp)[6], double (&Jc)[12]) {
   double X[3];
 #pragma unroll
@@ -274,7 +294,7 @@
     double tr[3];
 #pragma unroll
     for (int k = 0; k < 3; ++k) tr[k] = d.x_pose[cur][6 * c + 3 + k];
-    residual_jac_s(d.rot_lin[c], tr, X, W.fx, W.fy, W.cx, W.cy, uv.x, uv.y, r, Jp, Jc);
+    residual_jac_s(d.rot_lin[cr], tr, X, W.fx, W.fy, W.cx, W.cy, uv.x, uv.y, r, Jp, Jc);
   } else {
     double tr[3];
 #pragma unroll
@@ -287,8 +307,14 @@
   double* gsp;
   int cmin;
 };
+__device__ __forceinline__ double uniform_d(double v) {
+  const unsigned long long u = __double_as_longlong(v);
+  const unsigned lo = __builtin_amdgcn_readfirstlane((int)(u & 0xffffffffu)), hi = __builtin_amdgcn_readfirstlane((int)(u >> 32));
+  return __longlong_as_double(((unsigned long long)hi << 32) | lo);
+}
 template <bool SUP>
 __device__ __forceinline__ void ls_group(const BaDev& d, const LMOpt& o, const unsigned bid, const LsSup& su) {
+  const int fold = SUP ? 0 : d.fold;
   __shared__ double s_jc[kGB][12];
   __shared__ double s_qj[kGB][12];
   __shared__ double s_rg[kGB][4];
@@ -308,6 +334,13 @@
     d.dbg[8 * bid + 6] = ((unsigned long long)__builtin_amdgcn_s_getreg((31 << 11) | 4) << 8) |
                                 (__builtin_amdgcn_s_getreg((31 << 11) | 20) & 255);
 #endif
+  WinState S0{};
+  BaWin W0{};
+  if (fold == 2) {
+    S0 = state_copy(d.st[0]);
+    W0.pose_base = d.win[0].pose_base; W0.n_poses = d.win[0].n_poses;
+    W0.pblk_base = d.win[0].pblk_base; W0.n_pblk = d.win[0].n_pblk;
+  }
   const PBlk g = d.pblk[bid];
   const int t = threadIdx.x, lane = t & 63, wv = t >> 6;
   const bool has = t < g.no;
@@ -323,18 +356,43 @@
 #pragma unroll
     for (int k = 0; k < 3; ++k) { Xp[0][k] = d.x_pt[0][3 * p + k]; Xp[1][k] = d.x_pt[1][3 * p + k]; spp[k] = d.scale_pt[3 * p + k]; }
   }
-  const WinState& S = d.st[g.win];
-  if (S.done) return;
-  const BaWin& W = d.win[g.win];
-  const int cur = S.cur;
-  const double rad = S.radius;
+  __shared__ WinState s_dec;
+  int win = 0;
+  if (fold != 2) {
+    win = g.win;
+    S0 = state_copy(d.st[win]);
+    if (fold) {
+      W0.pose_base = d.win[win].pose_base; W0.n_poses = d.win[win].n_poses;
+      W0.pblk_base = d.win[win].pblk_base; W0.n_pblk = d.win[win].n_pblk;
+    }
+  }
+  if (S0.done) return;
+  const BaWin& W = d.win[win];
+  int cur = S0.cur, iter = S0.iter;
+  double rad = S0.radius;
+  if (fold) {
+    if (wv == 0) {
+      WinState Sn = S0;
+      lorb_lm_iteration rec;
+      lm_end_eval<false>(d, o, win, lane, Sn, W0, rec);
+      if (lane == 0) {
+        s_dec = Sn;
+        if ((int)bid == W0.pblk_base) { d.st2[win] = Sn; lm_record(d, win, rec); }
+      }
+    }
+    __syncthreads();
+    if (__builtin_amdgcn_readfirstlane(s_dec.done)) return;
+    cur = __builtin_amdgcn_readfirstlane(s_dec.cur);
+    iter = __builtin_amdgcn_readfirstlane(s_dec.iter);
+    rad = uniform_d(s_dec.radius);
+  }
   if (t < kGB) { s_mask[0][t] = 0ull; s_mask[1][t] = 0ull; }
   double r[2] = {0, 0}, Jp[6] = {0, 0, 0, 0, 0, 0}, Jc[12];
 #pragma unroll
   for (int k = 0; k < 12; ++k) Jc[k] = 0.0;
   double cost = 0.0;
   if (has) {
-    pm_lin(d, W, cur, p_, c_, fx_, uv, r, Jp, Jc);
+    pm_lin(d, W, cur, rot_idx(d, cur, c_), p_, c_, fx_, uv, r, Jp, Jc);
     cost = 0.5 * (r[0] * r[0] + r[1] * r[1]);
     double* v = s_qj[t];
     v[0] = Jp[0] * Jp[0] + Jp[3] * Jp[3]; v[1] = Jp[0] * Jp[1] + Jp[3] * Jp[4];
@@ -369,7 +427,7 @@
 #pragma unroll
     for (int k = 0; k < 3; ++k) d.etb[3 * p + k] = b[k];
     double sp[3];
-    if (S.iter == 0) {
+    if (iter == 0) {
       sp[0] = 1.0 / (1.0 + sqrt(E[0]));
       sp[1] = 1.0 / (1.0 + sqrt(E[3]));
       sp[2] = 1.0 / (1.0 + sqrt(E[5]));
@@ -388,7 +446,7 @@
       }
     }
     double Ei[6], bs[3];
-    if (!prep_point(E, b, sp, rad, o, Ei, bs)) prep_fail(d, g.win);
+    if (!prep_point(E, b, sp, rad, o, Ei, bs)) prep_fail(d, win, fold);
 #pragma unroll
     for (int k = 0; k < 6; ++k) { d.pinv[6 * p + k] = Ei[k]; s_jc[t][k] = Ei[k]; }
 #pragma unroll
@@ -610,7 +668,7 @@
   const BlockPair bp = d.bp[bid];
   const bool diag = bp.ch == bp.cl;
   if (MODE == 0 && !diag) return;
-  const WinState& S = d.st[bp.win];
+  const WinState& S = (d.fold ? d.st2 : d.st)[bp.win];
   const BaWin& W = d.win[bp.win];
   const int t = threadIdx.x, lane = t & 63, wv = t >> 6;
   const int fi = t < 36 ? t / 6 : (t < 42 ? t - 36 : 0), fj = t < 36 ? t % 6 : 0;
@@ -620,7 +678,7 @@
     scj = d.scale_pose[6 * bp.cl + fj];
     if (MODE == 1 && diag) udg = d.U[21 * bp.ch + u21(fi, fi)];
   }
-  if (S.done) return;
+  if (S.done | d.st[bp.win].done) return;
   const int h = bp.ch - W.pose_base, l = bp.cl - W.pose_base, dd = h - l;
   const int e0 = MODE == 0 ? 36 : 0, ne = MODE == 0 ? 12 : (diag ? 54 : 36);
   const int NS = 1024 / ne;
@@ -783,7 +841,7 @@
   double r[2] = {0, 0}, Jp[6] = {0, 0, 0, 0, 0, 0}, Jc[12];
 #pragma unroll
   for (int k = 0; k < 12; ++k) Jc[k] = 0.0;
-  if (has) pm_lin(d, W, cur, p_, c_, fx_, uv, r, Jp, Jc);
+  if (has) pm_lin(d, W, cur, rot_idx(d, cur, c_), p_, c_, fx_, uv, r, Jp, Jc);
   const int lp = p_ - g.p0;
   __syncthreads();
   double ya0 = 0.0, ya1 = 0.0;
@@ -1251,6 +1309,14 @@
   }
 }
 
+constexpr int kFoldMaxGroups = 512;
+bool fold_of(const lorb_ba_plan* P) {
+  if (env_flag("LORB_NO_FOLD") || no_fuse() || P->comm || P->has_super || chol_kind_of(P) != 2) return false;
+  for (const BaWin& w : P->hwin)
+    if (w.n_poses > 0 && w.n_pblk == 0) return false;
+  return P->grid_pblk > 0 && P->grid_pblk <= kFoldMaxGroups;
+}
+
 lorb_ba_plan::GraphKey graph_key(const lorb_ba_plan* P) {
   lorb_ba_plan::GraphKey k;
   k.kind = chol_kind_of(P);
@@ -1262,6 +1328,7 @@
   k.red_wide = red_threads(P);
   k.sup = P->has_super ? 1 : 0;
   k.grid_sg = P->grid_sg;
+  k.fold = P->fold ? 1 : 0;
   return k;
 }
 
@@ -1287,11 +1354,13 @@
   return LORB_OK;
 }
 
-int enqueue_iteration(lorb_ba_plan* P, const LMOpt& o, bool first) {
+int enqueue_iteration(lorb_ba_plan* P, const LMOpt& o, bool first, bool last) {
   lorb_ctx* ctx = P->ctx;
   hipStream_t s = ctx->stream;
-  const BaDev& d = P->dev;
   const bool fused = !first && chol_kind_of(P) == 2 && !no_fuse();
+  const bool fold_in = P->fold && fused, fold_out = P->fold && !last;
+  BaDev d = P->dev;
+  d.fold = fold_in ? (P->W == 1 ? 2 : 1) : 0;
   if (fused) {
     launch_ls(P, s, d, o);
   } else {
@@ -1327,7 +1396,7 @@
       LORB_TRY(lorb::comm_allreduce(P->comm, d.wstep_part, d.wstep, 3 * (size_t)P->W, LORB_OP_SUM));
     }
     hipLaunchKernelGGL(k_ba_lm_end<true>, dim3(P->W), dim3(64), 0, s, d, o);
-  } else {
+  } else if (!fold_out) {
     hipLaunchKernelGGL(k_ba_lm_end<false>, dim3(P->W), dim3(64), 0, s, d, o);
   }
   LORB_CHECK_LAUNCH(ctx);
@@ -1343,13 +1412,14 @@
   }
   LORB_CHECK_LAUNCH(ctx);
   if (o.max_iter <= 0) return enqueue_linearize(P, o);
-  for (int it = 0; it < o.max_iter; ++it) LORB_TRY(enqueue_iteration(P, o, it == 0));
+  for (int it = 0; it < o.max_iter; ++it) LORB_TRY(enqueue_iteration(P, o, it == 0, it + 1 == o.max_iter));
   return LORB_OK;
 }
 
 int plan_solve(lorb_ba_plan* P, const lorb_lm_options* opt) {
   lorb_ctx* ctx = P->ctx;
   LMOpt o = to_dev_opt(opt);
+  P->fold = fold_of(P);
   const bool timing = ctx->ktime || no_graph() || (P->comm && !P->comm->rccl);
   if (timing) return enqueue_solve(P, o);
   const lorb_ba_plan::GraphKey key = graph_key(P);
@@ -1458,12 +1528,17 @@
   const GrpGrid g_w = grp_grid(G, [](const lorb_ba_plan* P) { return P->W; });
   size_t lds = 0;
   for (const lorb_ba_plan* P : G->plans) lds = std::max(lds, sizeof(double) * (size_t)P->max_env_w);
-  auto linearise = [&]() {
+  const bool fold = G->plans[0]->fold;
+  bool one_win = true;
+  for (const lorb_ba_plan* P : G->plans) one_win = one_win && P->W == 1;
+  BaGrp bgf = bg;
+  for (int k = 0; k < n; ++k) bgf.d[k].fold = one_win ? 2 : 1;
+  auto linearise = [&](bool fold_in) {
     lorb::KernelTimer kt(ctx, LORB_K_BA_LINEARIZE);
-    if (g_pb.pre[n]) hipLaunchKernelGGL(k_ba_ls_g, dim3(g_pb.pre[n]), dim3(kLsThreads), 0, s, bg, g_pb, o);
+    if (g_pb.pre[n]) hipLaunchKernelGGL(k_ba_ls_g, dim3(g_pb.pre[n]), dim3(kLsThreads), 0, s, fold_in ? bgf : bg, g_pb, o);
   };
   if (o.max_iter <= 0) {
-    linearise();
+    linearise(false);
     launch_red_g<0>(G, s, bg, o);
     hipLaunchKernelGGL(k_ba_lm_begin_g, dim3(g_w.pre[n]), dim3(64), 0, s, bg, g_w, o);
     LORB_CHECK_LAUNCH(ctx);
@@ -1471,7 +1546,9 @@
   }
   for (int it = 0; it < o.max_iter; ++it) {
     const bool first = it == 0;
-    linearise();
+    const bool fold_in = fold && !first, fold_out = fold && it + 1 < o.max_iter;
+    const BaGrp& bi = fold_in ? bgf : bg;
+    linearise(fold_in);
     if (first) {
       {
         lorb::KernelTimer kt(ctx, LORB_K_BA_SCHUR);
@@ -1485,14 +1562,14 @@
     {
       lorb::KernelTimer kt(ctx, LORB_K_BA_SCHUR);
       if (first) launch_red_g<1>(G, s, bg, o);
-      else launch_red_g<2>(G, s, bg, o);
+      else launch_red_g<2>(G, s, bi, o);
     }
     {
       lorb::KernelTimer kt(ctx, LORB_K_BA_CHOLESKY);
-      launch_chol_2s_g(s, bg, g_w, o, !first, lds);
+      launch_chol_2s_g(s, bi, g_w, o, !first, lds);
     }
     if (g_pb.pre[n]) hipLaunchKernelGGL(k_ba_bs2_g, dim3(g_pb.pre[n]), dim3(kGB), 0, s, bg, g_pb);
-    hipLaunchKernelGGL(k_ba_lm_end_g, dim3(g_w.pre[n]), dim3(64), 0, s, bg, g_w, o);
+    if (!fold_out) hipLaunchKernelGGL(k_ba_lm_end_g, dim3(g_w.pre[n]), dim3(64), 0, s, bg, g_w, o);
   }
   for (lorb_ba_plan* P : G->plans) P->chol_kind = 2;
   LORB_CHECK_LAUNCH(ctx);
@@ -1507,6 +1584,11 @@
     return LORB_OK;
   }
   const LMOpt o = to_dev_opt(opt);
+  bool fold = true;
+  int groups = 0;
+  for (const lorb_ba_plan* P : G->plans) { fold = fold && fold_of(P); groups += P->grid_pblk; }
+  fold = fold && groups <= kFoldMaxGroups;
+  for (lorb_ba_plan* P : G->plans) P->fold = fold;
   if (no_graph() || ctx->ktime) {
     LORB_TRY(enqueue_group_solve(G, o));
     G->n_fused++;
@@ -1589,9 +1671,9 @@
     for (size_t c = 0; c < m.size(); ++c) reordered |= m[c] != (int)c;
   int runs = 0;
   for (const BaWin& w : plan->hwin) runs += w.n_sg;
-  const int32_t v[11] = {bw, plan->chol_kind, plan->n_bp, plan->n_pblk, plan->K, plan->Ptot, plan->Ctot, reordered,
-                         1, red_threads(plan), plan->has_super ? runs : 0};
-  for (int i = 0; i < n && i < 11; ++i) info[i] = v[i];
+  const int32_t v[12] = {bw, plan->chol_kind, plan->n_bp, plan->n_pblk, plan->K, plan->Ptot, plan->Ctot, reordered,
+                         1, red_threads(plan), plan->has_super ? runs : 0, plan->cache.kernel_nodes};
+  for (int i = 0; i < n && i < 12; ++i) info[i] = v[i];
   return LORB_OK;
 }
 
@@ -1620,8 +1702,8 @@
 
 int lorb_ba_group_info(lorb_ba_group* group, int32_t* info, int32_t n) {
   if (!group || !info || n < 0) return LORB_E_INVALID;
-  const int32_t v[3] = {(int32_t)group->plans.size(), group->n_fused, group->cache.captures};
-  for (int i = 0; i < n && i < 3; ++i) info[i] = v[i];
+  const int32_t v[4] = {(int32_t)group->plans.size(), group->n_fused, group->cache.captures, group->cache.kernel_nodes};
+  for (int i = 0; i < n && i < 4; ++i) info[i] = v[i];
   return LORB_OK;
 }
 
diff --git a/lorb_slam_amd/csrc/lorb_ba_build.hip b/lorb_slam_amd/csrc/lorb_ba_build.hip
--- a/lorb_slam_amd/csrc/lorb_ba_build.hip
+++ b/lorb_slam_amd/csrc/lorb_ba_build.hip
@@ -479,7 +479,7 @@
   LORB_TRY(alloc_exchange(P, C, (size_t)nw, (size_t)P->env_total + P->n_total + nw, &sol, &solp));
   d.env = sol; d.rhs = sol + P->env_total; d.wfail = sol + P->env_total + P->n_total;
   d.env_part = solp; d.rhs_part = solp + P->env_total; d.wfail_part = solp + P->env_total + P->n_total;
-  LORB_TRY(dalloc(P, (size_t)P->Ctot, &d.rot_lin));
+  LORB_TRY(dalloc(P, 2 * (size_t)P->Ctot, &d.rot_lin)); d.rot_stride = P->Ctot;
   LORB_TRY(dalloc(P, (size_t)P->Ctot, &d.rot_cand));
   LORB_TRY(dalloc(P, (size_t)std::max(P->NF, 1), &d.rot_fix));
   LORB_TRY(dalloc(P, (size_t)std::max(P->NF, 1), &d.rotv_fix));
@@ -488,6 +488,7 @@
   LORB_TRY(dalloc(P, dbg_words((size_t)nw, (size_t)std::max(P->n_pblk, nw)), &d.dbg));
   LORB_TRY(dalloc(P, ((size_t)P->n_total / 16 + nw + 1) * 1024, &d.kco));
   LORB_TRY(dalloc(P, (size_t)nw, &P->d_state)); d.st = P->d_state;
+  LORB_TRY(dalloc(P, (size_t)nw, &d.st2)); LORB_TRY(dalloc(P, (size_t)nw, &d.ls_fail));
   LORB_TRY(dalloc(P, (size_t)nw * LORB_LM_TRACE_CAP, &d.trace));
   LORB_TRY(dalloc(P, (size_t)std::max(part_total, 1ll), &d.gpart));
   LORB_TRY(dalloc(P, (size_t)std::max(P->grid_sg, 1), &d.gspan));
@@ -897,12 +898,13 @@
   LORB_TRY(alloc_exchange(P, C, 1, P->x2_off + n * n, &sol, &solp));
   d.rhs = sol; d.wfail = sol + n; d.env = sol + P->x2_off;
   d.rhs_part = solp; d.wfail_part = solp + n; d.env_part = solp + P->x2_off;
-  LORB_TRY(dalloc(P, C, &d.rot_lin)); LORB_TRY(dalloc(P, C, &d.rot_cand));
+  LORB_TRY(dalloc(P, 2 * C, &d.rot_lin)); d.rot_stride = (int)C; LORB_TRY(dalloc(P, C, &d.rot_cand));
   LORB_TRY(dalloc(P, (size_t)std::max(b.F, 1), &d.rot_fix)); LORB_TRY(dalloc(P, (size_t)std::max(b.F, 1), &d.rotv_fix));
   LORB_TRY(dalloc(P, n, &d.ycam));
   LORB_TRY(dalloc(P, dbg_words(1, K + Pn + 1), &d.dbg));
   LORB_TRY(dalloc(P, ((size_t)n / 16 + 2) * 1024, &d.kco));
   LORB_TRY(dalloc(P, (size_t)1, &P->d_state)); d.st = P->d_state;
+  LORB_TRY(dalloc(P, (size_t)1, &d.st2)); LORB_TRY(dalloc(P, (size_t)1, &d.ls_fail));
   LORB_TRY(dalloc(P, (size_t)LORB_LM_TRACE_CAP, &d.trace));
   P->W = 1;
   P->hwin.assign(1, BaWin{});
diff --git a/lorb_slam_amd/csrc/lorb_ba_chol.hip b/lorb_slam_amd/csrc/lorb_ba_chol.hip
--- a/lorb_slam_amd/csrc/lorb_ba_chol.hip
+++ b/lorb_slam_amd/csrc/lorb_ba_chol.hip
@@ -8,6 +8,13 @@
 namespace {
 
 using namespace lorb::ba;
+
+__device__ __forceinline__ void rot_lin_of(const BaDev& d, int k, int c) {
+  double x[6];
+#pragma unroll
+  for (int q = 0; q < 6; ++q) x[q] = d.x_pose[k][6 * c + q];
+  d.rot_lin[rot_off(d, k) + c] = lorb::rot_jet(x);
+}
 
 typedef double v4d __attribute__((ext_vector_type(4)));
 
@@ -284,6 +291,7 @@
       }
       d.rot_cand[c] = lorb::rot_val(xn);
     }
+    for (int ci = t; ci < W.n_poses; ci += 256) rot_lin_of(d, cur ^ 1, W.pose_base + ci);
   }
 }
 
@@ -452,6 +460,7 @@
     }
     d.rot_cand[c] = lorb::rot_val(xn);
   }
+  for (int ci2 = lane; ci2 < W.n_poses; ci2 += 64) rot_lin_of(d, cur ^ 1, W.pose_base + ci2);
 }
 
 __device__ __forceinline__ void wait_bit(unsigned long long* mask, int b) {
@@ -1002,10 +1011,20 @@
   __shared__ int s_bad;
   __shared__ int s_head_done;
 
+  const bool fold = HEAD && d.fold;
   const BaWin W = d.win[w];
-  const WinState S0 = d.st[w];
+  const int ls_fail = fold ? d.ls_fail[w] : 0;
+  const WinState S0 = [&] {
+    WinState S = (fold ? d.st2 : d.st)[w];
+    if (fold) S.chol_fail = ls_fail;
+    return S;
+  }();
   const int done = S0.done;
   const double wfail = d.sharded ? d.wfail[w] : 0.0;
+  if (fold) {
+    if (d.st[w].done) return;
+    if (done && threadIdx.x == 0) d.st[w] = S0;
+  }
   if (done) return;
   if (wfail > 0.0) {
     if (HEAD) {
@@ -1145,6 +1164,7 @@
   if (HEAD && wv == 4) {
     const WinState S = d.sharded ? lm_head<true>(d, o, w, lane, S0, W) : lm_head<false>(d, o, w, lane, S0, W);
     if (lane == 0) s_head_done = S.done;
+    if (fold && lane == 0) d.ls_fail[w] = 0;
   }
   if (wv == 4 || wv == 5) {
     int* pd = &s_pdone[side];
@@ -1303,6 +1323,20 @@
       d.x_pose[cur ^ 1][6 * c + k] = xn[k];
     }
     d.rot_cand[c] = lorb::rot_val(xn);
+  }
+  const int el = t - (NT - 256);
+  for (int ci2 = el; el >= 0 && el < 128 && ci2 < W.n_poses; ci2 += 128) {
+    const int c = W.pose_base + ci2;
+    double xn[3];
+#pragma unroll
+    for (int k = 0; k < 3; ++k) {
+      const int row = 6 * ci2 + k;
+      const double y = row < rt ? zt[row] : zb[n16 - 1 - row];
+      const double xp = d.x_pose[cur][6 * c + k];
+      const double sp = d.scale_pose[6 * c + k];
+      xn[k] = xp + (-y) * sp;
+    }
+    d.rot_lin[rot_off(d, cur ^ 1) + c] = lorb::rot_jet(xn);
   }
 #ifdef LORB_CHOL_TRACE
   if (t == 0) d.dbg[512 * w + 251] = __builtin_amdgcn_s_memtime();
diff --git a/lorb_slam_amd/csrc/lorb_ba_dev.h b/lorb_slam_amd/csrc/lorb_ba_dev.h
--- a/lorb_slam_amd/csrc/lorb_ba_dev.h
+++ b/lorb_slam_amd/csrc/lorb_ba_dev.h
@@ -195,6 +195,10 @@
   unsigned long long* dbg;
   double* kco;
   WinState* st;
+  WinState* st2;
+  int* ls_fail;
+  int fold;
+  int rot_stride;
   double* gpart;
   int2* gspan;
   const int4* sgrp;
@@ -206,6 +210,8 @@
   if (a > b) { const int t = a; a = b; b = t; }
   return a * 6 - (a * (a - 1)) / 2 + (b - a);
 }
+
+__device__ __forceinline__ int rot_off(const BaDev& d, int k) { return k ? d.rot_stride : 0; }
 
 __device__ __forceinline__ double readlane_d(double v, int l) {
   const unsigned long long u = __double_as_longlong(v);
diff --git a/lorb_slam_amd/csrc/lorb_ba_plan.h b/lorb_slam_amd/csrc/lorb_ba_plan.h
--- a/lorb_slam_amd/csrc/lorb_ba_plan.h
+++ b/lorb_slam_amd/csrc/lorb_ba_plan.h
@@ -25,6 +25,7 @@
   hipGraphExec_t exec = nullptr;
   bool valid = false;
   int captures = 0;
+  int kernel_nodes = 0;
   explicit GraphCache(const char* what_) : what(what_) {}
   GraphCache(const GraphCache&) = delete;
   GraphCache& operator=(const GraphCache&) = delete;
@@ -42,6 +43,18 @@
       if (e != hipSuccess) return lorb::set_error(ctx, LORB_E_DEVICE, "%s capture failed: %s", what, hipGetErrorString(e));
       graph = g;
       LORB_HIP(ctx, hipGraphInstantiate(&exec, graph, nullptr, nullptr, 0));
+      {
+        size_t nn = 0;
+        LORB_HIP(ctx, hipGraphGetNodes(graph, nullptr, &nn));
+        std::vector<hipGraphNode_t> nodes(nn);
+        if (nn) LORB_HIP(ctx, hipGraphGetNodes(graph, nodes.data(), &nn));
+        kernel_nodes = 0;
+        for (size_t i = 0; i < nn; ++i) {
+          hipGraphNodeType ty;
+          LORB_HIP(ctx, hipGraphNodeGetType(nodes[i], &ty));
+          kernel_nodes += ty == hipGraphNodeTypeKernel;
+        }
+      }
       remember();
       valid = true;
       captures++;
@@ -79,11 +92,13 @@
   struct GraphKey {
     int kind = -1, lds = 0, memset_env = 0, env_total = 0, grid_pblk = 0, grid_bp = 0, pt_launch = 0, x2_n = 0;
     int red_wide = 0, sup = 0, grid_sg = 0;
+    int fold = 0;
     bool operator==(const GraphKey& o) const { return memcmp(this, &o, sizeof(GraphKey)) == 0; }
   } gkey;
   int grid_pblk = 0, grid_bp = 0;
   int grid_sg = 0;
   bool has_super = false;
+  bool fold = false;
   int pt_launch = 0;
   int* live = nullptr;
   lorb_comm* comm = nullptr;
```
